# VinAIResearch/GeoFormer

Measured on AMD Instinct MI355X. Metric: scenes/sec forward (ScanNetV2 ~150k pts), higher is better.
Workload: dtype f32

## Files before the change

### geoformer_amd/csrc/decoder_attn.hip

```cpp
#include <stdlib.h>

#include "common.h"

#define DA_WAVES 16
#define DA_D 64

__device__ __forceinline__ float da_row_max(float v) {
    v = fmaxf(v, __int_as_float(__builtin_amdgcn_update_dpp(0, __float_as_int(v), 0xB1, 0xF, 0xF, true)));
    v = fmaxf(v, __int_as_float(__builtin_amdgcn_update_dpp(0, __float_as_int(v), 0x4E, 0xF, 0xF, true)));
    v = fmaxf(v, __int_as_float(__builtin_amdgcn_update_dpp(0, __float_as_int(v), 0x141, 0xF, 0xF, true)));
    v = fmaxf(v, __int_as_float(__builtin_amdgcn_update_dpp(0, __float_as_int(v), 0x140, 0xF, 0xF, true)));
    return v;
}
__device__ __forceinline__ float da_row_sum(float v) {
    v += __int_as_float(__builtin_amdgcn_update_dpp(0, __float_as_int(v), 0xB1, 0xF, 0xF, true));
    v += __int_as_float(__builtin_amdgcn_update_dpp(0, __float_as_int(v), 0x4E, 0xF, 0xF, true));
    v += __int_as_float(__builtin_amdgcn_update_dpp(0, __float_as_int(v), 0x141, 0xF, 0xF, true));
    v += __int_as_float(__builtin_amdgcn_update_dpp(0, __float_as_int(v), 0x140, 0xF, 0xF, true));
    return v;
}

template <int WAVES>
__global__ __launch_bounds__(WAVES * 64) void k_decoder_cross_attn(
    const float* __restrict__ geo_ctx, const float* __restrict__ max_geo, const float* __restrict__ qloc,
    const float* __restrict__ cloc, const float* __restrict__ lo, const float* __restrict__ hi,
    const float* __restrict__ gaussB, const float* __restrict__ Q1, const float* __restrict__ K1,
    const float* __restrict__ Kv, const float4* __restrict__ Wpack, int nq, int nc, float* __restrict__ out,
    float* __restrict__ stat_m, float* __restrict__ stat_l) {
    __shared__ float4 sW[3 * 16 * 64];
    __shared__ float4 sQ1[16];
    __shared__ float4 sB[3][2][4];
    __shared__ float sRed[3][WAVES][DA_D];
    const int qi = blockIdx.x, b = blockIdx.y;
    const int tid = threadIdx.x, lane = tid & 63, w = tid >> 6, g = lane >> 4, j = lane & 15;
    for (int t = tid; t < 3 * 16 * 64; t += WAVES * 64) sW[t] = Wpack[t];
    if (tid < 16) sQ1[tid] = *reinterpret_cast<const float4*>(Q1 + ((size_t)b * nq + qi) * DA_D + tid * 4);
    if (tid >= 64 && tid < 64 + 24) {
        const int e = tid - 64, axis = e >> 3, half = (e >> 2) & 1, gg = e & 3;
        sB[axis][half][gg] = *reinterpret_cast<const float4*>(gaussB + axis * 32 + half * 16 + 4 * gg);
    }
    geo_ctx += ((size_t)b * nq + qi) * nc;
    cloc += (size_t)b * nc * 3;
    K1 += (size_t)b * nc * DA_D;
    Kv += (size_t)b * nc * DA_D;
    const float mg = max_geo[(size_t)b * nq + qi];
    const float qx = qloc[((size_t)b * nq + qi) * 3 + 0], qy = qloc[((size_t)b * nq + qi) * 3 + 1],
                qz = qloc[((size_t)b * nq + qi) * 3 + 2];
    const float lx = lo[b * 3 + 0], ly = lo[b * 3 + 1], lz = lo[b * 3 + 2];
    const float sx = hi[b * 3 + 0] - lx, sy = hi[b * 3 + 1] - ly, sz = hi[b * 3 + 2] - lz;
    float sm[4][4], sl[4][4], sa[4][4];
#pragma unroll
    for (int rb = 0; rb < 4; rb++)
#pragma unroll
        for (int r = 0; r < 4; r++) {
            sm[rb][r] = -3.0e38f;
            sl[rb][r] = 0.f;
            sa[rb][r] = 0.f;
        }
    __syncthreads();

    const int ntiles = (nc + 15) >> 4;
    for (int t = w; t < ntiles; t += WAVES) {
        const int ctx = t * 16 + j;
        const bool valid = ctx < nc;
        const int cc = valid ? ctx : nc - 1;
        const float gd = geo_ctx[cc];
        float g0 = gd, g1 = gd, g2 = gd;
        if (gd < 0.f) {
            g0 = mg + fabsf(qx - cloc[cc * 3 + 0]);
            g1 = mg + fabsf(qy - cloc[cc * 3 + 1]);
            g2 = mg + fabsf(qz - cloc[cc * 3 + 2]);
        }
        const float t0 = ((g0 - lx) / sx) * 6.2831855f, t1 = ((g1 - ly) / sy) * 6.2831855f,
                    t2 = ((g2 - lz) / sz) * 6.2831855f;
        float R[4][4];
#pragma unroll
        for (int half = 0; half < 2; half++) {
            const float4 b0 = sB[0][half][g], b1 = sB[1][half][g], b2v = sB[2][half][g];
            const float p[4] = {fmaf(t2, b2v.x, fmaf(t1, b1.x, t0 * b0.x)), fmaf(t2, b2v.y, fmaf(t1, b1.y, t0 * b0.y)),
                                fmaf(t2, b2v.z, fmaf(t1, b1.z, t0 * b0.z)), fmaf(t2, b2v.w, fmaf(t1, b1.w, t0 * b0.w))};
#pragma unroll
            for (int e = 0; e < 4; e++) {
                float sn, cs;
                __sincosf(p[e], &sn, &cs);
                R[half][e] = sn;
// ... 240 lines not shown
                const float4 k1 = *reinterpret_cast<const float4*>(K1 + (size_t)cc[u] * DA_D + rb * 16 + 4 * g);
                H[u][rb][0] = fmaxf(acc[u][0] + q1.x - k1.x, 0.f);
                H[u][rb][1] = fmaxf(acc[u][1] + q1.y - k1.y, 0.f);
                H[u][rb][2] = fmaxf(acc[u][2] + q1.z - k1.z, 0.f);
                H[u][rb][3] = fmaxf(acc[u][3] + q1.w - k1.w, 0.f);
            }
            da_gemm_bf3_n<NT>(sW3, 2, rb, lane, RP, vv);
#pragma unroll
            for (int u = 0; u < NT; u++) V[u][rb] = vv[u];
            __builtin_amdgcn_sched_barrier(0);
        }
        DaPieces HP[NT];
#pragma unroll
        for (int u = 0; u < NT; u++) da_split_pack(H[u], HP[u]);
#pragma unroll
        for (int rb = 0; rb < 4; rb++) {
            f32x4 s[NT];
#pragma unroll
            for (int u = 0; u < NT; u++) s[u] = (f32x4){0.f, 0.f, 0.f, 0.f};
            da_gemm_bf3_n<NT>(sW3, 1, rb, lane, HP, s);
#pragma unroll
            for (int u = 0; u < NT; u++) {
                const float4 kv = *reinterpret_cast<const float4*>(Kv + (size_t)cc[u] * DA_D + rb * 16 + 4 * g);
                const float kvv[4] = {kv.x, kv.y, kv.z, kv.w};
                if (valid[u]) {
#pragma unroll
                    for (int r = 0; r < 4; r++) {
                        const float x = s[u][r] * kScale2;
                        const float val = V[u][rb][r] + kvv[r];
                        const float mn = fmaxf(sm[rb][r], x);
                        const float corr = __builtin_amdgcn_exp2f(sm[rb][r] - mn), p = __builtin_amdgcn_exp2f(x - mn);
                        sl[rb][r] = sl[rb][r] * corr + p;
                        sa[rb][r] = sa[rb][r] * corr + p * val;
                        sm[rb][r] = mn;
                    }
                }
            }
            __builtin_amdgcn_sched_barrier(0);
        }
    }
#pragma unroll
    for (int rb = 0; rb < 4; rb++)
#pragma unroll
        for (int r = 0; r < 4; r++) {
            const float m = da_row_max(sm[rb][r]);
            if (j == 0) sRed[0][w][rb * 16 + 4 * g + r] = m;
        }
    __syncthreads();
    if (tid < DA_D) {
        float m = sRed[0][0][tid];
#pragma unroll
        for (int u = 1; u < WAVES; u++) m = fmaxf(m, sRed[0][u][tid]);
        sRed[0][0][tid] = m;
    }
    __syncthreads();
#pragma unroll
    for (int rb = 0; rb < 4; rb++)
#pragma unroll
        for (int r = 0; r < 4; r++) {
            const int c = rb * 16 + 4 * g + r;
            const float f = __builtin_amdgcn_exp2f(sm[rb][r] - sRed[0][0][c]);
            const float l = da_row_sum(sl[rb][r] * f), a = da_row_sum(sa[rb][r] * f);
            if (j == 0) {
                sRed[1][w][c] = l;
                sRed[2][w][c] = a;
            }
        }
    __syncthreads();
    if (tid < DA_D) {
        float L = 0.f, A = 0.f;
#pragma unroll
        for (int u = 0; u < WAVES; u++) {
            L += sRed[1][u][tid];
            A += sRed[2][u][tid];
        }
        out[((size_t)b * nq + qi) * DA_D + tid] = A / L;
        if (stat_m) {
            stat_m[((size_t)b * nq + qi) * DA_D + tid] = sRed[0][0][tid] * 0.69314718055994531f;
            stat_l[((size_t)b * nq + qi) * DA_D + tid] = L;
        }
    }
}

extern "C" size_t gf_decoder_wpack_floats(void) { return (size_t)DA_WPACK_F32 + (size_t)DA_WPACK_BF3_U4 * 4; }

__global__ void k_decoder_pack(const float* __restrict__ W1, const float* __restrict__ W2, const float* __restrict__ Wv,
                               float* __restrict__ Wp) {
    const int t = blockIdx.x * blockDim.x + threadIdx.x;
    if (t >= 3 * 16 * 64 * 4) return;
    const int s = t & 3, lane = (t >> 2) & 63, kb = (t >> 8) & 3, rb = (t >> 10) & 3, m = t >> 12;
    const float* W = m == 0 ? W1 : (m == 1 ? W2 : Wv);
    Wp[t] = W[(rb * 16 + (lane & 15)) * DA_D + kb * 16 + 4 * (lane >> 4) + s];
}

__global__ void k_decoder_pack_bf3(const float* __restrict__ W1, const float* __restrict__ W2, const float* __restrict__ Wv,
                                   uint4* __restrict__ Wp3) {
    const int t = blockIdx.x * blockDim.x + threadIdx.x;
    if (t >= 3 * 4 * 2 * 64) return;
    const int lane = t & 63, h = (t >> 6) & 1, rb = (t >> 7) & 3, m = t >> 9;
    const float* W = m == 0 ? W1 : (m == 1 ? W2 : Wv);
    unsigned pc[3][8];
    for (int e = 0; e < 8; e++) {
        const int kb = 2 * h + (e >> 2), sidx = e & 3;
        da_split3(W[(rb * 16 + (lane & 15)) * DA_D + kb * 16 + 4 * (lane >> 4) + sidx], pc[0][e], pc[1][e], pc[2][e]);
    }
    for (int piece = 0; piece < 3; piece++) {
        uint4 v;
        v.x = (pc[piece][1] & 0xffff0000u) | (pc[piece][0] >> 16);
        v.y = (pc[piece][3] & 0xffff0000u) | (pc[piece][2] >> 16);
        v.z = (pc[piece][5] & 0xffff0000u) | (pc[piece][4] >> 16);
        v.w = (pc[piece][7] & 0xffff0000u) | (pc[piece][6] >> 16);
        Wp3[((size_t)(((m * 4 + rb) * 2 + h) * 3 + piece)) * 64 + lane] = v;
    }
}

extern "C" int gf_decoder_pack_weights(const float* W1, const float* W2, const float* Wv, float* Wpack, void* stream) {
    hipLaunchKernelGGL(k_decoder_pack, dim3(48), dim3(256), 0, (hipStream_t)stream, W1, W2, Wv, Wpack);
    hipLaunchKernelGGL(k_decoder_pack_bf3, dim3(6), dim3(256), 0, (hipStream_t)stream, W1, W2, Wv,
                       reinterpret_cast<uint4*>(Wpack + DA_WPACK_F32));
    GF_CHECK_LAUNCH("gf_decoder_pack_weights");
    return GF_OK;
}

static int g_da_bf3 = -1;
extern "C" int gf_dev_cross_attn_bf3(int on) {
    g_da_bf3 = on < 0 ? -1 : (on != 0);
    return GF_OK;
}

extern "C" int gf_decoder_cross_attn_cfg(const float* geo_ctx, const float* max_geo, const float* qloc, const float* cloc,
                                         const float* lo, const float* hi, const float* gaussB, const float* Q1,
                                         const float* K1, const float* Kv, const float* Wpack, const float* b2, int B,
                                         int nq, int nc, int d, float* out, float* stat_m, float* stat_l, int wg_waves,
                                         void* stream) {
    GF_CHECK_ARG(d == DA_D, "gf_decoder_cross_attn: implemented for dec_dim = 64 (got %d)", d);
    GF_CHECK_ARG(B >= 0 && nq >= 0 && nc >= 1, "gf_decoder_cross_attn: bad sizes");
    GF_CHECK_ARG((stat_m == nullptr) == (stat_l == nullptr), "gf_decoder_cross_attn: stat_m and stat_l come together");
    GF_CHECK_ARG(wg_waves == 16 || wg_waves == 8, "gf_decoder_cross_attn_cfg: %d waves per workgroup (16 or 8)", wg_waves);
    if (B == 0 || nq == 0) return GF_OK;
    (void)b2;
    if (wg_waves == 16 && g_da_bf3 != 0) {
        const size_t lds = (size_t)DA_WPACK_BF3_U4 * sizeof(uint4);
        gf_allow_lds((const void*)k_decoder_cross_attn_bf3<DA_BF3_WAVES, 1>, (int)lds);
        GF_LAUNCH_OP(GF_OP_CROSS_ATTN, (k_decoder_cross_attn_bf3<DA_BF3_WAVES, 1>), dim3(nq, B), dim3(DA_BF3_WAVES * 64), lds,
                     (hipStream_t)stream, geo_ctx, max_geo, qloc, cloc, lo, hi, gaussB, Q1, K1, Kv,
                     reinterpret_cast<const uint4*>(Wpack + DA_WPACK_F32), nq, nc, out, stat_m, stat_l);
        GF_CHECK_LAUNCH("gf_decoder_cross_attn");
        return GF_OK;
    }
    if (wg_waves == 16)
        GF_LAUNCH_OP(GF_OP_CROSS_ATTN, k_decoder_cross_attn<16>, dim3(nq, B), dim3(16 * 64), 0, (hipStream_t)stream, geo_ctx,
                     max_geo, qloc, cloc, lo, hi, gaussB, Q1, K1, Kv, reinterpret_cast<const float4*>(Wpack), nq, nc, out,
                     stat_m, stat_l);
    else
        GF_LAUNCH_OP(GF_OP_CROSS_ATTN, k_decoder_cross_attn<8>, dim3(nq, B), dim3(8 * 64), 0, (hipStream_t)stream, geo_ctx,
                     max_geo, qloc, cloc, lo, hi, gaussB, Q1, K1, Kv, reinterpret_cast<const float4*>(Wpack), nq, nc, out,
                     stat_m, stat_l);
    GF_CHECK_LAUNCH("gf_decoder_cross_attn");
    return GF_OK;
}

extern "C" int gf_decoder_cross_attn(const float* geo_ctx, const float* max_geo, const float* qloc, const float* cloc,
                                     const float* lo, const float* hi, const float* gaussB, const float* Q1,
                                     const float* K1, const float* Kv, const float* Wpack, const float* b2, int B,
                                     int nq, int nc, int d, float* out, float* stat_m, float* stat_l, void* stream) {
    return gf_decoder_cross_attn_cfg(geo_ctx, max_geo, qloc, cloc, lo, hi, gaussB, Q1, K1, Kv, Wpack, b2, B, nq, nc, d, out,
                                     stat_m, stat_l, 16, stream);
}


#define DAB_TS 68

__global__ void k_decoder_pack_w2t(const float* __restrict__ W2, float* __restrict__ Wp) {
    const int t = blockIdx.x * blockDim.x + threadIdx.x;
    if (t >= 16 * 64 * 4) return;
    const int s = t & 3, lane = (t >> 2) & 63, kb = (t >> 8) & 3, cb = (t >> 10) & 3;
    Wp[t] = W2[(kb * 16 + 4 * (lane >> 4) + s) * DA_D + cb * 16 + (lane & 15)];
}

__global__ __launch_bounds__(256, 1) void k_decoder_cross_attn_bwd(
    const float* __restrict__ geo_ctx, const float* __restrict__ max_geo, const float* __restrict__ qloc,
    const float* __restrict__ cloc, const float* __restrict__ lo, const float* __restrict__ hi,
    const float* __restrict__ gaussB, const float* __restrict__ Q1, const float* __restrict__ K1,
    const float* __restrict__ Kv, const float4* __restrict__ Wpack, const float4* __restrict__ W2Tpack,
    const float* __restrict__ outv, const float* __restrict__ stat_m, const float* __restrict__ stat_l,
    const float* __restrict__ gout, int B, int nq, int nc, int qsplit, float* __restrict__ dQ1p,
    float* __restrict__ dK1, float* __restrict__ dKv, float* __restrict__ dWp) {
    __shared__ float4 sW[3 * 16 * 64];
    __shared__ float4 sW2T[16 * 64];
    __shared__ float4 sB[3][2][4];
    __shared__ __attribute__((aligned(16))) float sT[4][16 * DAB_TS];
    __shared__ __attribute__((aligned(16))) float sV[4][4][DA_D];
    const int tid = threadIdx.x, lane = tid & 63, w = tid >> 6, g = lane >> 4, j = lane & 15;
    for (int t = tid; t < 3 * 16 * 64; t += 256) sW[t] = Wpack[t];
    for (int t = tid; t < 16 * 64; t += 256) sW2T[t] = W2Tpack[t];
    if (tid < 24) {
        const int axis = tid >> 3, half = (tid >> 2) & 1, gg = tid & 3;
        sB[axis][half][gg] = *reinterpret_cast<const float4*>(gaussB + axis * 32 + half * 16 + 4 * gg);
    }
    __syncthreads();
    const int ntiles = (nc + 15) >> 4;
    const int wave = blockIdx.x * 4 + w;
    const int items = B * ntiles * qsplit;
    if (wave >= items) return;
    const int part = wave % qsplit, bt = wave / qsplit;
    const int tile = bt % ntiles, b = bt / ntiles;
    const int qper = (nq + qsplit - 1) / qsplit;
    const int q0 = part * qper, q1 = min(nq, q0 + qper);
    float* T = sT[w];
    float* V = &sV[w][0][0];

    const int ctx = tile * 16 + j;
    const bool valid = ctx < nc;
    const int cc = valid ? ctx : nc - 1;
    const float* K1b = K1 + ((size_t)b * nc + cc) * DA_D;
    const float* Kvb = Kv + ((size_t)b * nc + cc) * DA_D;
    float4 k1[4], kv[4];
#pragma unroll
    for (int rb = 0; rb < 4; rb++) {
        k1[rb] = *reinterpret_cast<const float4*>(K1b + rb * 16 + 4 * g);
        kv[rb] = *reinterpret_cast<const float4*>(Kvb + rb * 16 + 4 * g);
    }
    const float cx = cloc[((size_t)b * nc + cc) * 3 + 0], cy = cloc[((size_t)b * nc + cc) * 3 + 1],
                cz = cloc[((size_t)b * nc + cc) * 3 + 2];
    const float lx = lo[b * 3 + 0], ly = lo[b * 3 + 1], lz = lo[b * 3 + 2];
    const float sx = hi[b * 3 + 0] - lx, sy = hi[b * 3 + 1] - ly, sz = hi[b * 3 + 2] - lz;

    f32x4 aW1[4][4], aW2[4][4], aWv[4][4];
    f32x4 aK1[4], aKv[4];
#pragma unroll
    for (int a = 0; a < 4; a++) {
        aK1[a] = (f32x4){0.f, 0.f, 0.f, 0.f};
        aKv[a] = (f32x4){0.f, 0.f, 0.f, 0.f};
#pragma unroll
        for (int c = 0; c < 4; c++) {
            aW1[a][c] = (f32x4){0.f, 0.f, 0.f, 0.f};
            aW2[a][c] = (f32x4){0.f, 0.f, 0.f, 0.f};
            aWv[a][c] = (f32x4){0.f, 0.f, 0.f, 0.f};
        }
    }
    auto transpose = [&](const f32x4 (&XA)[4], f32x4 (&XB)[4]) {
        asm volatile("s_waitcnt lgkmcnt(0)" ::: "memory");
#pragma unroll
        for (int rb = 0; rb < 4; rb++)
            *reinterpret_cast<float4*>(&T[j * DAB_TS + rb * 16 + 4 * g]) = make_float4(XA[rb][0], XA[rb][1], XA[rb][2], XA[rb][3]);
        asm volatile("s_waitcnt lgkmcnt(0)" ::: "memory");
#pragma unroll
        for (int cb = 0; cb < 4; cb++)
#pragma unroll
            for (int r = 0; r < 4; r++) XB[cb][r] = T[(4 * g + r) * DAB_TS + cb * 16 + j];
// ... 239 lines not shown
```

### geoformer_amd/csrc/decoder_layer.h

```cpp
#pragma once
#include "tile_gemm.h"

#define DL_D 64
#define DL_H 4
#define DL_DK 16
#define DL_THREADS 1024
#define DL_MAXFF 256

#define DL_LD 68
#define DL_LDH 260

template <typename Out>
__device__ __forceinline__ void dl_tile_layernorm_p(const float (*S)[DL_LD], int nvalid, float wl, float bl, int wave,
                                                    int nwaves, int lane, Out out);
template <typename Out>
__device__ __forceinline__ void dl_tile_layernorm(const float (*S)[DL_LD], int nvalid, const float* __restrict__ w,
                                                  const float* __restrict__ b, int wave, int nwaves, int lane,
                                                  Out out) {
    dl_tile_layernorm_p(S, nvalid, w[lane], b[lane], wave, nwaves, lane, out);
}
template <typename Out>
__device__ __forceinline__ void dl_tile_layernorm_p(const float (*S)[DL_LD], int nvalid, float wl, float bl, int wave,
                                                    int nwaves, int lane, Out out) {
    for (int r = wave; r < nvalid; r += nwaves) {
        const float v = S[r][lane];
        const float s = gf_wave_sum(v);
        const float mu = s / (float)DL_D;
        const float dv = v - mu;
        const float q = gf_wave_sum(dv * dv);
        const float rstd = 1.0f / sqrtf(q / (float)DL_D + 1e-5f);
        out(r, lane, dv * rstd * wl + bl);
    }
}
```

### geoformer_amd/csrc/decoder_layer.hip

```cpp
#include "decoder_layer.h"

struct DlPost {
    const float *omw, *omb, *n3w, *n3b, *l1w, *l1b, *l2w, *l2b, *fnw, *fnb;
};
struct DlPre {
    const float *n1w, *n1b, *ipw, *ipb, *opw, *opb, *n2w, *n2b, *w1w, *w1b;
};

#define DL_TILE_THREADS 256

#ifdef DL_TRACE
__device__ unsigned long long* g_dl_trace = nullptr;
extern "C" int gf_dev_dl_trace(void* p) {
    GF_TRY(hipMemcpyToSymbol(HIP_SYMBOL(g_dl_trace), &p, sizeof(p)));
    return GF_OK;
}
#define DL_STAMP(k) do { if (g_dl_trace && threadIdx.x == 0) g_dl_trace[((size_t)(blockIdx.y * gridDim.x + blockIdx.x)) * 32 + (k)] = __builtin_amdgcn_s_memtime(); } while (0)
#else
#define DL_STAMP(k) do { } while (0)
#endif

__global__ __launch_bounds__(DL_TILE_THREADS) void k_decoder_stage_a(const float* __restrict__ attn_out,
                                                                     const float* __restrict__ tgt_in,
                                                                     const float* __restrict__ query_pos, int T,
                                                                     int B, int ff, int has_post, int has_pre,
                                                                     DlPost po, DlPre pr, float* __restrict__ state,
                                                                     float* __restrict__ inter_out) {
    __shared__ float sX[16][DL_LD], sT[16][DL_LD], sQ[16][DL_LD], sH[16][DL_LDH];
    const int b = blockIdx.y, t0 = blockIdx.x * 16;
    const int nvalid = min(16, T - t0);
    const int lane = threadIdx.x & 63, wave = threadIdx.x >> 6, nw = DL_TILE_THREADS / 64;
    float* X = state + (size_t)b * T * (5 * DL_D);
    float* TGT2 = X + (size_t)T * DL_D;
    float* QKV = TGT2 + (size_t)T * DL_D;
    const int lds = B * DL_D;
    DL_STAMP(0);
    constexpr int NTF = DL_MAXFF / 16 / (DL_TILE_THREADS / 64);
    GfTileW<1, DL_D / 16> w_om;
    GfTileW<NTF, DL_D / 16> w_l1;
    GfTileW<1, DL_MAXFF / 16> w_l2;
    GfTileW<2, DL_D / 16> w_qk;
    GfTileW<1, DL_D / 16> w_v;
    float n3w = 0.f, n3b = 0.f, fnw = 0.f, fnb = 0.f, n1w = 0.f, n1b = 0.f;
    if (has_post) {
        gf_tile_w_load(w_om, po.omw, po.omb, DL_D, DL_D, wave, nw, lane);
        n3w = po.n3w[lane]; n3b = po.n3b[lane];
        gf_tile_w_load(w_l1, po.l1w, po.l1b, ff, DL_D, wave, nw, lane);
        gf_tile_w_load(w_l2, po.l2w, po.l2b, DL_D, ff, wave, nw, lane);
        fnw = po.fnw[lane]; fnb = po.fnb[lane];
    }
    if (has_pre) {
        n1w = pr.n1w[lane]; n1b = pr.n1b[lane];
        gf_tile_w_load(w_qk, pr.ipw, pr.ipb, 2 * DL_D, DL_D, wave, nw, lane);
        gf_tile_w_load(w_v, pr.ipw + 2 * DL_D * DL_D, pr.ipb + 2 * DL_D, DL_D, DL_D, wave, nw, lane);
    }
    if (has_post) {
        const float* tg = TGT2 + (size_t)t0 * DL_D;
        gf_tile_gemm_w<true>(attn_out + ((size_t)b * T + t0) * DL_D, DL_D, nvalid, DL_D, DL_D, wave, nw, lane, w_om,
                             [&](int r, int c, float v) { sX[r][c] = v; }, tg, DL_D);
        __syncthreads();
        DL_STAMP(1);
        dl_tile_layernorm_p(sX, nvalid, n3w, n3b, wave, nw, lane, [&](int r, int c, float v) { sT[r][c] = v; });
        __syncthreads();
        DL_STAMP(2);
        gf_tile_gemm_w<true>(&sT[0][0], DL_LD, nvalid, DL_D, ff, wave, nw, lane, w_l1,
                             [&](int r, int c, float v) { sH[r][c] = v; });
        __syncthreads();
        DL_STAMP(3);
        gf_tile_gemm_w<false>(&sH[0][0], DL_LDH, nvalid, ff, DL_D, wave, nw, lane, w_l2,
                              [&](int r, int c, float v) { sX[r][c] += v; });
        __syncthreads();
        DL_STAMP(4);
        float* io = inter_out + (size_t)t0 * lds + b * DL_D;
        dl_tile_layernorm_p(sX, nvalid, fnw, fnb, wave, nw, lane,
                            [&](int r, int c, float v) { io[(size_t)r * lds + c] = v; });
    } else {
        for (int i = threadIdx.x; i < nvalid * DL_D; i += DL_TILE_THREADS)
            sX[i >> 6][i & 63] = tgt_in[(size_t)(t0 + (i >> 6)) * lds + b * DL_D + (i & 63)];
        __syncthreads();
    }
    DL_STAMP(5);
    if (!has_pre) return;
    const float* qp = query_pos + (size_t)t0 * lds + b * DL_D;
    dl_tile_layernorm_p(sX, nvalid, n1w, n1b, wave, nw, lane, [&](int r, int c, float v) {
        sT[r][c] = v;
        sQ[r][c] = v + qp[(size_t)r * lds + c];
    });
    for (int i = threadIdx.x; i < nvalid * DL_D; i += DL_TILE_THREADS)
        X[(size_t)(t0 + (i >> 6)) * DL_D + (i & 63)] = sX[i >> 6][i & 63];
    __syncthreads();
    DL_STAMP(6);
    float* qkv = QKV + (size_t)t0 * (3 * DL_D);
    gf_tile_gemm_w<false>(&sQ[0][0], DL_LD, nvalid, DL_D, 2 * DL_D, wave, nw, lane, w_qk,
                          [&](int r, int c, float v) { qkv[(size_t)r * (3 * DL_D) + c] = v; });
    DL_STAMP(7);
    gf_tile_gemm_w<false>(&sT[0][0], DL_LD, nvalid, DL_D, DL_D, wave, nw, lane, w_v,
                          [&](int r, int c, float v) { qkv[(size_t)r * (3 * DL_D) + 2 * DL_D + c] = v; });
    DL_STAMP(8);
}

template <int QTN>
__device__ __forceinline__ void dl_attn_two_pass(const float* __restrict__ QKV, int T, int h, int j, int g, float4 bq,
                                                 f32x4& o, float& l) {
    float4 akt[QTN];
    float vt[QTN][4];
    const int last = T - 1;
#pragma unroll
    for (int kt = 0; kt < QTN; kt++) {
        const int krow = min(kt * 16 + j, last);
        akt[kt] = *reinterpret_cast<const float4*>(QKV + (size_t)krow * (3 * DL_D) + DL_D + h * DL_DK + 4 * g);
#pragma unroll
        for (int i = 0; i < 4; i++) {
            const int key = min(kt * 16 + 4 * g + i, last);
            vt[kt][i] = QKV[(size_t)key * (3 * DL_D) + 2 * DL_D + h * DL_DK + j];
        }
    }
    float sc[QTN][4];
    float mx = -INFINITY;
#pragma unroll
    for (int kt = 0; kt < QTN; kt++) {
        f32x4 s = {0.f, 0.f, 0.f, 0.f};
        s = gf_mfma4(akt[kt], bq, s);
#pragma unroll
        for (int i = 0; i < 4; i++) {
            sc[kt][i] = (kt * 16 + 4 * g + i) < T ? s[i] * 0.25f : -INFINITY;
            mx = fmaxf(mx, sc[kt][i]);
        }
    }
    mx = fmaxf(mx, gf_shfl_xor<16>(mx));
    mx = fmaxf(mx, gf_shfl_xor<32>(mx));
#pragma unroll
    for (int kt = 0; kt < QTN; kt++) {
#pragma unroll
        for (int i = 0; i < 4; i++) {
            const float pi = __builtin_amdgcn_exp2f((sc[kt][i] - mx) * 1.4426950408889634f);
            l += pi;
            o = __builtin_amdgcn_mfma_f32_16x16x4f32(vt[kt][i], pi, o, 0, 0, 0);
        }
    }
}

__global__ __launch_bounds__(DL_TILE_THREADS) void k_decoder_stage_b(int T, int B, DlPre pr,
                                                                     float* __restrict__ state,
                                                                     float* __restrict__ q1_out) {
    __shared__ float sO[16][DL_LD], sX[16][DL_LD], sT[16][DL_LD];
    const int b = blockIdx.y, t0 = blockIdx.x * 16;
    const int nvalid = min(16, T - t0);
    const int lane = threadIdx.x & 63, wave = threadIdx.x >> 6, nw = DL_TILE_THREADS / 64;
    const int j = lane & 15, g = lane >> 4;
    float* X = state + (size_t)b * T * (5 * DL_D);
    float* TGT2 = X + (size_t)T * DL_D;
    const float* QKV = TGT2 + (size_t)T * DL_D;
    DL_STAMP(16);
    GfTileW<1, DL_D / 16> w_op, w_w1;
    gf_tile_w_load(w_op, pr.opw, pr.opb, DL_D, DL_D, wave, nw, lane);
    gf_tile_w_load(w_w1, pr.w1w, pr.w1b, DL_D, DL_D, wave, nw, lane);
    const float n2w = pr.n2w[lane], n2b = pr.n2b[lane];
    {
        const int h = wave;
        const int QT = (T + 15) >> 4;
        const float4 z4 = make_float4(0.f, 0.f, 0.f, 0.f);
        const int qrow = t0 + j;
        float4 bq = z4;
        if (qrow < T) bq = *reinterpret_cast<const float4*>(QKV + (size_t)qrow * (3 * DL_D) + h * DL_DK + 4 * g);
        f32x4 o = {0.f, 0.f, 0.f, 0.f};
        float m = -INFINITY, l = 0.f;
        if (QT <= 16) {
            if (QT <= 8) dl_attn_two_pass<8>(QKV, T, h, j, g, bq, o, l);
            else dl_attn_two_pass<16>(QKV, T, h, j, g, bq, o, l);
        } else {
        float4 ak = z4;
        float v[4];
        {
            if (j < T) ak = *reinterpret_cast<const float4*>(QKV + (size_t)j * (3 * DL_D) + DL_D + h * DL_DK + 4 * g);
#pragma unroll
            for (int i = 0; i < 4; i++) {
                const int key = 4 * g + i;
                v[i] = key < T ? QKV[(size_t)key * (3 * DL_D) + 2 * DL_D + h * DL_DK + j] : 0.f;
            }
        }
        for (int kt = 0; kt < QT; kt++) {
            float4 ak_n = z4;
            float v_n[4] = {0.f, 0.f, 0.f, 0.f};
            if (kt + 1 < QT) {
                const int krow = (kt + 1) * 16 + j;
                if (krow < T)
                    ak_n = *reinterpret_cast<const float4*>(QKV + (size_t)krow * (3 * DL_D) + DL_D + h * DL_DK + 4 * g);
#pragma unroll
                for (int i = 0; i < 4; i++) {
                    const int key = (kt + 1) * 16 + 4 * g + i;
                    v_n[i] = key < T ? QKV[(size_t)key * (3 * DL_D) + 2 * DL_D + h * DL_DK + j] : 0.f;
                }
            }
            f32x4 s = {0.f, 0.f, 0.f, 0.f};
            s = gf_mfma4(ak, bq, s);
            float sc[4];
#pragma unroll
            for (int i = 0; i < 4; i++) sc[i] = (kt * 16 + 4 * g + i) < T ? s[i] * 0.25f : -INFINITY;
            float mx = fmaxf(fmaxf(sc[0], sc[1]), fmaxf(sc[2], sc[3]));
            mx = fmaxf(mx, gf_shfl_xor<16>(mx));
            mx = fmaxf(mx, gf_shfl_xor<32>(mx));
            const float mnew = fmaxf(m, mx);
            const float corr = expf(m - mnew);
            float p[4];
#pragma unroll
            for (int i = 0; i < 4; i++) p[i] = expf(sc[i] - mnew);
            l = l * corr + ((p[0] + p[1]) + (p[2] + p[3]));
            o *= corr;
            m = mnew;
#pragma unroll
            for (int i = 0; i < 4; i++) o = __builtin_amdgcn_mfma_f32_16x16x4f32(v[i], p[i], o, 0, 0, 0);
            ak = ak_n;
#pragma unroll
            for (int i = 0; i < 4; i++) v[i] = v_n[i];
        }
        }
        l += gf_shfl_xor<16>(l);
        l += gf_shfl_xor<32>(l);
#pragma unroll
        for (int i = 0; i < 4; i++) sO[j][h * DL_DK + 4 * g + i] = o[i] / l;
    }
    __syncthreads();
    DL_STAMP(17);
    const float* xg = X + (size_t)t0 * DL_D;
    gf_tile_gemm_w<false>(&sO[0][0], DL_LD, nvalid, DL_D, DL_D, wave, nw, lane, w_op,
                          [&](int r, int c, float v) { sX[r][c] = v; }, xg, DL_D);
    __syncthreads();
    DL_STAMP(18);
    float* xo = X + (size_t)t0 * DL_D;
    for (int i = threadIdx.x; i < nvalid * DL_D; i += DL_TILE_THREADS) xo[i] = sX[i >> 6][i & 63];
    float* tg = TGT2 + (size_t)t0 * DL_D;
    dl_tile_layernorm_p(sX, nvalid, n2w, n2b, wave, nw, lane, [&](int r, int c, float v) {
        sT[r][c] = v;
        tg[r * DL_D + c] = v;
    });
    __syncthreads();
    DL_STAMP(19);
    float* q1 = q1_out + ((size_t)b * T + t0) * DL_D;
    gf_tile_gemm_w<false>(&sT[0][0], DL_LD, nvalid, DL_D, DL_D, wave, nw, lane, w_w1,
                          [&](int r, int c, float v) { q1[r * DL_D + c] = v; });
    DL_STAMP(20);
}

extern "C" size_t gf_decoder_token_state_bytes(int nq, int B) {
    return (size_t)(nq > 0 ? nq : 0) * (B > 0 ? B : 0) * (5 * DL_D) * sizeof(float);
}

extern "C" int gf_decoder_token_stage(const float* attn_out, const float* tgt_in, const float* query_pos, int nq, int B,
                                      int d, int nhead, int ff, const float* const* post_params,
                                      const float* const* pre_params, void* state, float* inter_out, float* q1_out,
                                      void* stream) {
    GF_CHECK_ARG(d == DL_D && nhead == DL_H, "gf_decoder_token_stage: built for d_model=64, 4 heads (got %d, %d)", d,
                 nhead);
    GF_CHECK_ARG(ff > 0 && ff % 16 == 0 && ff <= DL_MAXFF, "gf_decoder_token_stage: dim_feedforward %d not in 16..%d",
                 ff, DL_MAXFF);
    GF_CHECK_ARG(nq >= 0 && B >= 0, "gf_decoder_token_stage: bad sizes");
    GF_CHECK_ARG(post_params || pre_params, "gf_decoder_token_stage: nothing to do");
    GF_CHECK_ARG(post_params ? (attn_out && inter_out) : (tgt_in != nullptr),
                 "gf_decoder_token_stage: post needs attn_out and inter_out, a first stage needs tgt_in");
    GF_CHECK_ARG(!pre_params || (query_pos && q1_out), "gf_decoder_token_stage: pre needs query_pos and q1_out");
    if (nq == 0 || B == 0) return GF_OK;
    DlPost po = {};
    DlPre pr = {};
    if (post_params) {
        for (int i = 0; i < 10; i++) GF_CHECK_ARG(post_params[i], "gf_decoder_token_stage: post_params[%d] is null", i);
        po = {post_params[0], post_params[1], post_params[2], post_params[3], post_params[4],
              post_params[5], post_params[6], post_params[7], post_params[8], post_params[9]};
    }
    if (pre_params) {
        for (int i = 0; i < 10; i++) GF_CHECK_ARG(pre_params[i], "gf_decoder_token_stage: pre_params[%d] is null", i);
        pr = {pre_params[0], pre_params[1], pre_params[2], pre_params[3], pre_params[4],
              pre_params[5], pre_params[6], pre_params[7], pre_params[8], pre_params[9]};
    }
    const dim3 grid((nq + 15) / 16, B);
    hipLaunchKernelGGL(k_decoder_stage_a, grid, dim3(DL_TILE_THREADS), 0, (hipStream_t)stream, attn_out, tgt_in,
                       query_pos, nq, B, ff, post_params ? 1 : 0, pre_params ? 1 : 0, po, pr, (float*)state, inter_out);
    if (pre_params)
        hipLaunchKernelGGL(k_decoder_stage_b, grid, dim3(DL_TILE_THREADS), 0, (hipStream_t)stream, nq, B, pr,
                           (float*)state, q1_out);
    GF_CHECK_LAUNCH("gf_decoder_token_stage");
    return GF_OK;
}
```

### geoformer_amd/csrc/mask_head.hip

```cpp
#include "common.h"

#ifndef MH_Q
#define MH_Q 2
#endif
#ifndef MH_MINB
#define MH_MINB 3
#endif

__device__ __forceinline__ float mh_xor32(float v, int lane) {
    const auto r = __builtin_amdgcn_permlane32_swap(__float_as_uint(v), __float_as_uint(v), false, false);
    return __uint_as_float(lane < 32 ? r[1] : r[0]);
}
__device__ __forceinline__ float mh_xor16(float v, int lane) {
    const auto r = __builtin_amdgcn_permlane16_swap(__float_as_uint(v), __float_as_uint(v), false, false);
    return __uint_as_float((lane & 16) ? r[0] : r[1]);
}

__device__ __forceinline__ float mh_relu(float x) { return __int_as_float(max(__float_as_int(x), 0)); }

typedef short bf16x4 __attribute__((ext_vector_type(4)));
typedef short mh_s8 __attribute__((ext_vector_type(8)));
typedef __bf16 mh_bf16x8 __attribute__((ext_vector_type(8)));
__device__ __forceinline__ f32x4 mh_mfma2(bf16x4 a1, bf16x4 a2, bf16x4 b1, bf16x4 b2, f32x4 acc) {
    const mh_s8 a = __builtin_shufflevector(a1, a2, 0, 1, 2, 3, 4, 5, 6, 7), b = __builtin_shufflevector(b1, b2, 0, 1, 2, 3, 4, 5, 6, 7);
// ... 81 lines not shown
    const size_t n16 = (size_t)N * 16;
    auto fetch = [&](int blk, Block& B) {
        const int p0 = TINY ? blk * 64 : min(blk * 64, N - 64);
#pragma unroll
        for (int t = 0; t < 4; t++) {
            const int pc = TINY ? min(p0 + 16 * t + j, N - 1) : p0 + 16 * t + j;
            if constexpr (SPLIT) {
                const size_t e = (size_t)pc * 16 + 4 * g;
                B.fh[t] = *reinterpret_cast<const bf16x4*>(fs + e);
                B.fm[t] = *reinterpret_cast<const bf16x4*>(fs + n16 + e);
                B.fl[t] = *reinterpret_cast<const bf16x4*>(fs + 2 * n16 + e);
            } else {
                B.f[t] = *reinterpret_cast<const float4*>(feat + (size_t)pc * 16 + 4 * g);
            }
            B.pc[t] = g < 3 ? coords[(size_t)pc * 3 + g] : 0.f;
#pragma unroll
            for (int u = 0; u < MH_Q; u++)
                B.gd[u][t] = USE_GEO ? geo[(size_t)qrow[u] * N + pc] : 0.f;
        }
    };
    auto compute = [&](const Block& cur, int blk) {
        const int p0 = TINY ? blk * 64 : min(blk * 64, N - 64);
#pragma unroll
        for (int t = 0; t < MH_Q; t++) {
            const int q = qg * MH_Q + t;
            float part[4];
#pragma unroll
            for (int tl = 0; tl < 4; tl++) {
                float rel = qc[t] - cur.pc[tl];
                if (USE_GEO) {
                    const float ms = __uint_as_float((__float_as_uint(rel) & 0x80000000u) | __float_as_uint(mq[t]));
                    rel = rel + ((cur.gd[t][tl] < 0.f && rel != 0.f) ? ms : 0.f);
                }
                f32x4 acc = {0.f, 0.f, 0.f, 0.f};
                acc = __builtin_amdgcn_mfma_f32_16x16x4f32(w5[t], rel, acc, 0, 0, 0);
                if constexpr (SPLIT) {
                    acc = mh_mfma2(wl[t], wh[t], cur.fh[tl], cur.fl[tl], acc);
                    acc = mh_mfma2(wm[t], wm[t], cur.fm[tl], cur.fh[tl], acc);
                    acc = mh_mfma2(wh[t], wh[t], cur.fm[tl], cur.fh[tl], acc);
                } else {
                    acc = __builtin_amdgcn_mfma_f32_16x16x4f32(wf[t][0], cur.f[tl].x, acc, 0, 0, 0);
                    acc = __builtin_amdgcn_mfma_f32_16x16x4f32(wf[t][1], cur.f[tl].y, acc, 0, 0, 0);
                    acc = __builtin_amdgcn_mfma_f32_16x16x4f32(wf[t][2], cur.f[tl].z, acc, 0, 0, 0);
                    acc = __builtin_amdgcn_mfma_f32_16x16x4f32(wf[t][3], cur.f[tl].w, acc, 0, 0, 0);
                }
                float s = 0.f;
#pragma unroll
                for (int r = 0; r < 4; r++) s = fmaf(ww[t][r], mh_relu(acc[r]), s);
                part[tl] = s;
            }
            {
                const bool hi = g >= 2;
                const float send0 = hi ? part[0] : part[2], send1 = hi ? part[1] : part[3];
                const float r0 = mh_xor32(send0, lane), r1 = mh_xor32(send1, lane);
                const float k0 = (hi ? part[2] : part[0]) + r0, k1 = (hi ? part[3] : part[1]) + r1;
                const bool odd = g & 1;
                const float send = odd ? k0 : k1;
                const float r = mh_xor16(send, lane);
                const float tot = (odd ? k1 : k0) + r + b2q[t];
                const int p = p0 + 16 * g + j;
                if (p < N && q < nq) out[(size_t)q * N + p] = tot;
            }
        }
    };
    Block bufA, bufB;
    if (blk0 < blk1) fetch(blk0, bufA);
    for (int blk = blk0; blk < blk1; blk += 2) {
        if (blk + 1 < blk1) fetch(blk + 1, bufB);
        compute(bufA, blk);
        if (blk + 1 < blk1) {
            if (blk + 2 < blk1) fetch(blk + 2, bufA);
            compute(bufB, blk + 1);
        }
    }
}

extern "C" int gf_mask_head_packed(const float* feat, const float* coords, const float* geo, const float* qxyz,
                                   const float* sqrt_max_geo, const float* w1, const float* b1, const float* w2,
                                   const float* b2, int ldp, int N, int nq, int C, float* out, void* stream);
extern "C" int gf_mask_head_episodes(const float* feat, const float* coords, const float* geo, const float* qxyz,
                                     const float* sqrt_max_geo, const float* w1, const float* b1, const float* w2,
                                     const float* b2, int ldp, int N, int nq, int E, int C, void* split_ws, float* out,
                                     void* stream);
extern "C" size_t gf_mask_head_split_bytes(int N) { return (size_t)(N > 0 ? N : 0) * 16 * 3 * sizeof(unsigned short); }
extern "C" int gf_mask_head(const float* feat, const float* coords, const float* geo, const float* qxyz,
                            const float* sqrt_max_geo, const float* w1, const float* b1, const float* w2,
                            const float* b2, int N, int nq, int C, float* out, void* stream) {
    return gf_mask_head_packed(feat, coords, geo, qxyz, sqrt_max_geo, w1, b1, w2, b2, 0, N, nq, C, out, stream);
}

extern "C" int gf_mask_head_packed(const float* feat, const float* coords, const float* geo, const float* qxyz,
                                   const float* sqrt_max_geo, const float* w1, const float* b1, const float* w2,
                                   const float* b2, int ldp, int N, int nq, int C, float* out, void* stream) {
    return gf_mask_head_episodes(feat, coords, geo, qxyz, sqrt_max_geo, w1, b1, w2, b2, ldp, N, nq, 1, C, nullptr, out, stream);
}

extern "C" int gf_mask_head_episodes(const float* feat, const float* coords, const float* geo, const float* qxyz,
                                     const float* sqrt_max_geo, const float* w1, const float* b1, const float* w2,
                                     const float* b2, int ldp, int N, int nq_scene, int E, int C, void* split_ws, float* out,
                                     void* stream) {
    GF_CHECK_ARG(ldp >= 0, "gf_mask_head: negative parameter stride");
    GF_CHECK_ARG(C == 16, "gf_mask_head: only the 16-channel mask head (m=16) is implemented, got C=%d", C);
    GF_CHECK_ARG(N >= 0 && nq_scene >= 0 && E >= 1, "gf_mask_head: bad sizes");
    GF_CHECK_ARG((long long)nq_scene * E < (1ll << 30), "gf_mask_head: %d episodes x %d queries", E, nq_scene);
    GF_CHECK_ARG((geo == nullptr) == (sqrt_max_geo == nullptr), "gf_mask_head: geo and sqrt_max_geo come together");
    if (N == 0 || nq_scene == 0) return GF_OK;
    const int qmod = nq_scene, nq = nq_scene * E;
    const int qgroups = (nq + MH_Q - 1) / MH_Q;
    const int nblocks = (N + 63) / 64;
    int chunks = (256 * 4 * 8 + qgroups - 1) / qgroups;
    if (chunks > nblocks) chunks = nblocks;
    if (chunks < 1) chunks = 1;
    const long long waves = (long long)qgroups * chunks;
    dim3 grid((unsigned)((waves + 3) / 4));
    hipStream_t st = (hipStream_t)stream;
    const unsigned short* fs = (const unsigned short*)split_ws;
    if (fs) {
        GF_CHECK_ARG(((uintptr_t)fs % 8) == 0, "gf_mask_head: split_ws must be 8-byte aligned");
        const int n16 = N * 16;
        hipLaunchKernelGGL(k_mh_split, dim3(gf_div_up(n16, 256)), dim3(256), 0, st, feat, n16, (unsigned short*)split_ws);
    }
#define MH_LAUNCH(GEO_, SPLIT_)                                                                                          \
    do {                                                                                                                 \
        if (N < 64)                                                                                                      \
            GF_LAUNCH_OP(GF_OP_MASK_HEAD, (k_mask_head<GEO_, SPLIT_, true>), grid, dim3(256), 0, st, feat, coords, geo, qxyz, \
                         sqrt_max_geo, w1, b1, w2, b2, ldp, N, nq, qmod, chunks, fs, out);                               \
        else                                                                                                             \
            GF_LAUNCH_OP(GF_OP_MASK_HEAD, (k_mask_head<GEO_, SPLIT_, false>), grid, dim3(256), 0, st, feat, coords, geo, qxyz, \
                         sqrt_max_geo, w1, b1, w2, b2, ldp, N, nq, qmod, chunks, fs, out);                               \
    } while (0)
    if (geo && fs) MH_LAUNCH(true, true);
    else if (geo) MH_LAUNCH(true, false);
    else if (fs) MH_LAUNCH(false, true);
    else MH_LAUNCH(false, false);
#undef MH_LAUNCH
    GF_CHECK_LAUNCH("gf_mask_head");
    return GF_OK;
}

#define MHB_Q 4

template <bool USE_GEO>
__global__ __launch_bounds__(256, 2) void k_mask_head_bwd_feat(const float* __restrict__ feat, const float* __restrict__ coords,
                                                               const float* __restrict__ geo, const float* __restrict__ qxyz,
                                                               const float* __restrict__ mx, const float* __restrict__ w1,
                                                               const float* __restrict__ b1, const float* __restrict__ w2,
                                                               const float* __restrict__ gout, int ldp, int N, int nq,
                                                               int qmod, int qsplit, float* __restrict__ dfeat) {
    const int ld_w1 = ldp ? ldp : 16 * 19, ld_v = ldp ? ldp : 16;
    const int lane = threadIdx.x & 63, g = lane >> 4, j = lane & 15;
    const int wave = (blockIdx.x * blockDim.x + threadIdx.x) >> 6;
    const int nblocks = (N + 63) >> 6;
    const int blk = wave / qsplit, part = wave - blk * qsplit;
    if (blk >= nblocks) return;
    const int p0 = blk * 64;
    const int qper = (nq + qsplit - 1) / qsplit;
    const int q0 = part * qper, q1 = min(nq, q0 + qper);
    float4 fA[4];
    float pcA[4];
    f32x4 accF[4];
#pragma unroll
    for (int t = 0; t < 4; t++) {
        const int pa = min(p0 + 16 * t + j, N - 1);
        fA[t] = *reinterpret_cast<const float4*>(feat + (size_t)pa * 16 + 4 * g);
        pcA[t] = coords[(size_t)pa * 3 + min(g, 2)];
        accF[t] = (f32x4){0.f, 0.f, 0.f, 0.f};
    }
    for (int q = q0; q < q1; q++) {
        const float* W = w1 + (size_t)q * ld_w1;
        float wf[4], wT[4], ww[4];
#pragma unroll
        for (int s = 0; s < 4; s++) {
            wf[s] = W[j * 19 + 3 + 4 * g + s];
            wT[s] = W[(4 * g + s) * 19 + 3 + j];
            ww[s] = w2[(size_t)q * ld_v + 4 * g + s];
        }
        const float w5 = g < 3 ? W[j * 19 + g] : b1[(size_t)q * ld_v + j];
        const int qs = q % qmod;
        const float qcA = g < 3 ? qxyz[qs * 3 + g] : 0.f;
        const float mq = USE_GEO ? mx[qs] : 0.f;
        float goA[4], gdA[4];
#pragma unroll
        for (int t = 0; t < 4; t++) {
            const int pa = p0 + 16 * t + j;
            goA[t] = pa < N ? gout[(size_t)q * N + pa] : 0.f;
            gdA[t] = USE_GEO ? geo[(size_t)qs * N + min(pa, N - 1)] : 0.f;
        }
#pragma unroll
        for (int t = 0; t < 4; t++) {
            float rel = qcA - pcA[t];
            if (USE_GEO) rel = rel + (gdA[t] < 0.f ? mq : 0.f) * (rel > 0.f ? 1.f : (rel < 0.f ? -1.f : 0.f));
            if (g == 3) rel = 1.0f;
            f32x4 acc = {0.f, 0.f, 0.f, 0.f};
            acc = __builtin_amdgcn_mfma_f32_16x16x4f32(w5, rel, acc, 0, 0, 0);
            acc = __builtin_amdgcn_mfma_f32_16x16x4f32(wf[0], fA[t].x, acc, 0, 0, 0);
            acc = __builtin_amdgcn_mfma_f32_16x16x4f32(wf[1], fA[t].y, acc, 0, 0, 0);
            acc = __builtin_amdgcn_mfma_f32_16x16x4f32(wf[2], fA[t].z, acc, 0, 0, 0);
            acc = __builtin_amdgcn_mfma_f32_16x16x4f32(wf[3], fA[t].w, acc, 0, 0, 0);
#pragma unroll
            for (int s = 0; s < 4; s++) {
                const float dh = acc[s] > 0.f ? goA[t] * ww[s] : 0.f;
                accF[t] = __builtin_amdgcn_mfma_f32_16x16x4f32(wT[s], dh, accF[t], 0, 0, 0);
            }
// ... 205 lines not shown
```

### geoformer_amd/csrc/proposal.hip

```cpp
#include "proposal_rows.h"

__global__ __launch_bounds__(PR_THREADS) void k_proposal_stats(const float* __restrict__ logits,
                                                               const float* __restrict__ cls_logits,
                                                               const float* __restrict__ sem_prob, int N, int ncls,
                                                               float logit_thresh, float score_thresh,
                                                               int npoint_thresh, int min_class,
                                                               int* __restrict__ cls_pred_out,
                                                               int* __restrict__ npoints_out,
                                                               float* __restrict__ scores_out,
                                                               int* __restrict__ final_out) {
    const int q = blockIdx.x;
    pr_stats_row(logits + (size_t)q * N, cls_logits + (size_t)q * ncls, sem_prob, (size_t)N, N, ncls, logit_thresh,
                 score_thresh, npoint_thresh, min_class, cls_pred_out + q, npoints_out + q, scores_out + q,
                 final_out + q);
}

__global__ __launch_bounds__(PR_THREADS) void k_proposal_stats_fs(const float* __restrict__ logits,
                                                                  const float* __restrict__ sim, int N,
                                                                  float logit_thresh, float score_thresh,
                                                                  int npoint_thresh, float sim_thresh,
                                                                  int* __restrict__ npoints_out,
                                                                  float* __restrict__ scores_out,
                                                                  int* __restrict__ final_out) {
    __shared__ int r_cnt[PR_THREADS / 64];
// ... 112 lines not shown
}

__global__ __launch_bounds__(256) void k_mask_intersections(const unsigned long long* __restrict__ bits, int n, int W2,
                                                            int32_t* __restrict__ inter) {
    const long long wave = ((long long)blockIdx.x * blockDim.x + threadIdx.x) >> 6;
    const int lane = threadIdx.x & 63;
    if (wave >= (long long)n * n) return;
    const int i = (int)(wave / n), j = (int)(wave - (long long)i * n);
    if (j < i) return;
    const unsigned long long *a = bits + (size_t)i * W2, *b = bits + (size_t)j * W2;
    int c = 0;
    for (int w = lane; w < W2; w += 64) c += __popcll(a[w] & b[w]);
    c = gf_wave_sum_i(c);
    if (lane == 0) {
        inter[(size_t)i * n + j] = c;
        inter[(size_t)j * n + i] = c;
    }
}

extern "C" size_t gf_mask_intersections_scratch_bytes(int n, int N) {
    return (size_t)(n > 0 ? n : 0) * ((size_t)(N > 0 ? N : 0) + 63) / 64 * sizeof(unsigned long long) + 64;
}

extern "C" int gf_mask_intersections(const int32_t* masks, int n, int N, void* scratch, int32_t* inter, void* stream) {
    GF_CHECK_ARG(n >= 0 && N >= 0, "gf_mask_intersections: bad sizes");
    if (n == 0) return GF_OK;
    hipStream_t st = (hipStream_t)stream;
    const int W2 = (N + 63) / 64;
    unsigned long long* bits = (unsigned long long*)scratch;
    if (W2 > 0) {
        const long long waves = (long long)n * W2;
        hipLaunchKernelGGL(k_mask_pack_bits, dim3((unsigned)((waves + 3) / 4)), dim3(256), 0, st, masks, n, N, W2, bits);
    }
    const long long pairs = (long long)n * n;
    hipLaunchKernelGGL(k_mask_intersections, dim3((unsigned)((pairs + 3) / 4)), dim3(256), 0, st, bits, n, W2, inter);
    GF_CHECK_LAUNCH("gf_mask_intersections");
    return GF_OK;
}

__global__ __launch_bounds__(256) void k_relpos_gather(const float* __restrict__ geo, const int32_t* __restrict__ inds,
                                                       int n, int nc, float* __restrict__ geo_ctx,
                                                       float* __restrict__ row_max) {
    __shared__ float s_m[4];
    const int q = blockIdx.x;
    const float* g = geo + (size_t)q * n;
    float m = -INFINITY;
    for (int j = threadIdx.x; j < nc; j += 256) {
        const float v = g[inds[j]];
        geo_ctx[(size_t)q * nc + j] = v;
        m = fmaxf(m, v);
    }
    m = gf_wave_max(m);
    if ((threadIdx.x & 63) == 0) s_m[threadIdx.x >> 6] = m;
    __syncthreads();
    if (threadIdx.x == 0) row_max[q] = fmaxf(fmaxf(s_m[0], s_m[1]), fmaxf(s_m[2], s_m[3]));
}

__global__ __launch_bounds__(1024) void k_relpos_fix(float* __restrict__ row_max, int nq) {
    __shared__ float s_m[16];
    float m = -INFINITY;
    for (int q = threadIdx.x; q < nq; q += 1024) m = fmaxf(m, row_max[q]);
    m = gf_wave_max(m);
    if ((threadIdx.x & 63) == 0) s_m[threadIdx.x >> 6] = m;
    __syncthreads();
    float all = s_m[0];
#pragma unroll
    for (int w = 1; w < 16; w++) all = fmaxf(all, s_m[w]);
    for (int q = threadIdx.x; q < nq; q += 1024)
        if (row_max[q] < 0.f) row_max[q] = all;
}

extern "C" int gf_relpos_prepare(const float* geo, const int32_t* inds, int nq, int n, int nc, float* geo_ctx,
                                 float* max_geo, void* stream) {
    GF_CHECK_ARG(geo && inds && geo_ctx && max_geo, "gf_relpos_prepare: null argument");
    GF_CHECK_ARG(nq >= 0 && n >= 1 && nc >= 1, "gf_relpos_prepare: bad sizes");
    if (nq == 0) return GF_OK;
    hipStream_t st = (hipStream_t)stream;
    hipLaunchKernelGGL(k_relpos_gather, dim3(nq), dim3(256), 0, st, geo, inds, n, nc, geo_ctx, max_geo);
    hipLaunchKernelGGL(k_relpos_fix, dim3(1), dim3(1024), 0, st, max_geo, nq);
    GF_CHECK_LAUNCH("gf_relpos_prepare");
    return GF_OK;
}

__global__ __launch_bounds__(1024) void k_proposal_select(const int32_t* __restrict__ final_, const int32_t* __restrict__ cls_pred,
                                                          const float* __restrict__ scores, int nq,
                                                          int32_t* __restrict__ sel, long long* __restrict__ cls_out,
                                                          float* __restrict__ scores_out, int32_t* __restrict__ count) {
    pr_select_rows(final_, cls_pred, scores, nq, sel, cls_out, scores_out, count);
}

extern "C" int gf_proposal_select(const int32_t* final_, const int32_t* cls_pred, const float* scores, int nq,
                                  int32_t* sel, long long* cls_out, float* scores_out, int32_t* d_count, void* stream) {
    GF_CHECK_ARG(final_ && cls_pred && scores && sel && cls_out && scores_out && d_count && nq >= 0,
                 "gf_proposal_select: bad arguments");
    hipLaunchKernelGGL(k_proposal_select, dim3(1), dim3(1024), 0, (hipStream_t)stream, final_, cls_pred, scores, nq, sel,
                       cls_out, scores_out, d_count);
    GF_CHECK_LAUNCH("gf_proposal_select");
    return GF_OK;
}
```

### geoformer_amd/model/geoformer.py

```python
from __future__ import annotations

import functools
import os

import numpy as np
import torch
import torch.nn as nn
from torch.nn import functional as F

from .. import _lib, pointops, spconv, unet_exec, unet_train
from . import config as _config
from .backbone import ResidualBlock, UBlock, conv1d_bn_relu, random_downsample
from .layers import (BatchNorm1d, BigLinear, GenericMLP, LazyRelPos, PointwiseConv1d, PositionEmbeddingCoordsSine, RelPosSpec,
                     TransformerDecoder,
                     TransformerDecoderLayer, scene_counts)
from .set_abstraction import PointnetSAModuleVotesSeparate


class _Voxelization(torch.autograd.Function):

    @staticmethod
    def forward(ctx, feats, map_rule, mode=4):
        ctx.rule, ctx.mode, ctx.N = map_rule, mode, feats.shape[0]
        return pointops.voxelize_fp(feats.contiguous(), map_rule, mode)
# ... 651 lines not shown
                    grid_done = torch.cuda.Event()
                    grid_done.record(aux)
                grid = (grid, grid_done)
            if multi:
                for t in (xyz_b, idx, first, sampling_indices):
                    if t is not None:
                        t.record_stream(main)
            if early is not None and b == 0:
                main.wait_event(early_done)
            staged[b] = [xyz_b, None, idx, grid, sampling_indices]
            if not epilogue:
                continue
            self._side_epilogue(b, batch_size, g, xyz_b, src, pc_dims, main, side, aux, picks_ready)
        for sb in scene_streams:
            main.wait_stream(sb)
        with grad_ctx():
            for b, st in enumerate(staged):
                feat_b = output_feats_[offs[b]:offs[b + 1]]
                if st[4] is not None:
                    feat_b = pointops.take_rows_unique(feat_b, st[4])
                st[1] = feat_b.unsqueeze(0).transpose(1, 2).contiguous()
        staged = [tuple(st[:4]) for st in staged]
        self.__dict__.setdefault("_gf_pending_side", {})[_stream_key(locs_float_.device)] = geo_ready
        self.__dict__.setdefault("_gf_stretch_events", {})[_stream_key(locs_float_.device)] = fps_done_evs + [
            ev for ev in geo_ready if ev is not None]
        cat = lambda ts: ts[0] if len(ts) == 1 else torch.cat(ts)
        with grad_ctx():
            fused = []
            for xyz_b, feat_b, idx, grid in staged:
                if grid is not None:
                    main.wait_event(grid[1])
                fused.append(self.set_aggregator.fused_forward(xyz_b, feat_b, idx, grid=None if grid is None else grid[0]))
            if all(f is not None for f in fused):
                context_locs, pre_enc_inds = cat([f[0] for f in fused]), cat([st[2] for st in staged])
                context_feats = cat([f[1] for f in fused]).transpose(1, 2)
                res = ((context_locs, context_feats, pre_enc_inds), geo)
                return res + (early_out,) if early is not None else res
            locs, gfeat, gxyz, inds = [], [], [], []
            for xyz_b, feat_b, idx, _ in staged:
                l, gf, gx, idx = self.set_aggregator.group_points(xyz_b, feat_b, inds=idx)
                locs.append(l); gfeat.append(gf); gxyz.append(gx); inds.append(idx)
            context_locs, pre_enc_inds = cat(locs), cat(inds)
            context_feats = self.set_aggregator.mlp(cat(gfeat), cat(gxyz)).transpose(1, 2)
        res = ((context_locs, context_feats, pre_enc_inds), geo)
        return res + (early_out,) if early is not None else res

    def _side_epilogue(self, b, batch_size, g, xyz_b, src, pc_dims, main, side, aux, first_ready):
        early = self._early()
        if b == 0:
            early.clear()
        with torch.cuda.stream(side):
            mx = torch.max(g, dim=1)[0]
            mx = torch.sqrt(torch.where(mx < 0, torch.max(mx), mx)).contiguous()
            mx.record_stream(main)
            ev = torch.cuda.Event()
            ev.record(side)
            early[("mx", b)] = (g, mx, ev)
        if batch_size == 1 and pc_dims is not None and self.cfg.dec_dim == 64:
            aux.wait_event(first_ready)
            with torch.cuda.stream(aux):
                qpr = self._pointwise_chain("qproj", [self.query_projection], xyz_b)
                if qpr is not None:
                    xyz_b.record_stream(aux)
                    q_locs = xyz_b[:, src.long()]
                    qpe = self.pos_embedding(q_locs, input_range=pc_dims).float()
                    qpos = pointops.pointwise_mlp(qpe[0].t().contiguous(), qpr)
                    qpos.record_stream(main)
                    src.record_stream(aux)
                    ev = torch.cuda.Event()
                    ev.record(aux)
                    early["qpos"] = (q_locs, qpos, ev)

    def _early(self):
        if not torch.cuda.is_available():
            return {}
        return self.__dict__.setdefault("_gf_early", {}).setdefault(_stream_key(), {})

    def _join_side_stream(self):
        pend = self.__dict__.get("_gf_pending_side")
        if pend and torch.cuda.is_available():
            for ev in pend.pop(_stream_key(), None) or ():
                torch.cuda.current_stream().wait_event(ev)

    def relative_position_embedding(self, context_locs, query_locs, pc_dims, geo_dists, pre_enc_inds):
        B = context_locs.shape[0]
        self._join_side_stream()
        if context_locs.is_cuda and self.cfg.dec_dim == 64 and (not torch.is_grad_enabled()
                                                                 or os.environ.get("GF_FUSED_BWD", "1") != "0"):
            if B == 1 and pre_enc_inds.dtype == torch.int32:
                g1, m1 = pointops.relpos_prepare(geo_dists[0].contiguous(), pre_enc_inds[0].contiguous())
                geo, max_geo = g1.unsqueeze(0), m1.unsqueeze(0)
            elif B > 1 and pre_enc_inds.stride(0) == 0 and all(g is geo_dists[0] for g in geo_dists):
                g1 = geo_dists[0][:, pre_enc_inds[0].long()]
                m1 = torch.max(g1, dim=1)[0]
                m1 = torch.where(m1 < 0, torch.max(m1), m1)
                geo, max_geo = g1.unsqueeze(0).expand(B, -1, -1).contiguous(), m1.unsqueeze(0).expand(B, -1).contiguous()
            else:
                geo = torch.stack([geo_dists[b][:, pre_enc_inds[b].long()] for b in range(B)], dim=0).contiguous()
                max_geo = torch.max(geo, dim=2)[0]
                max_geo = torch.where(max_geo < 0, torch.max(max_geo), max_geo).contiguous()
            return RelPosSpec(geo, max_geo, query_locs.contiguous(), context_locs.contiguous(),
                              pc_dims[0].float().contiguous(), pc_dims[1].float().contiguous(),
                              self.pos_embedding.gauss_B.contiguous())
        rel = torch.abs(query_locs[:, :, None, :] - context_locs[:, None, :, :])
        nq, nc = rel.shape[1], rel.shape[2]
        geo = torch.stack([geo_dists[b][:, pre_enc_inds[b].long()] for b in range(B)], dim=0)
        max_geo = torch.max(geo, dim=2)[0]
        max_all = torch.max(max_geo)
        max_geo = torch.where(max_geo < 0, max_all, max_geo)
        geo3 = geo[:, :, :, None].repeat(1, 1, 1, 3)
        geo3 = torch.where(geo3 < 0, max_geo[:, :, None, None] + rel, geo3)
        emb = self.pos_embedding(geo3.reshape(B, nq * nc, -1), input_range=pc_dims).reshape(B, -1, nq, nc)
        return emb.permute(2, 3, 0, 1)

    def forward_decoder(self, context_locs, context_feats, query_locs, pc_dims, geo_dists, pre_enc_inds):
        nq = self.cfg.n_query_points
        if context_locs.shape[0] == 1 and context_locs.is_cuda and not torch.is_grad_enabled():
            e2d = self._pointwise_chain("e2d", [self.encoder_to_decoder_projection], context_feats)
            qpr = self._pointwise_chain("qproj", [self.query_projection], context_feats)
            if e2d is not None and qpr is not None:
                ctx = pointops.pointwise_mlp(context_feats[0].contiguous(), e2d)
                rel = LazyRelPos(lambda: self.relative_position_embedding(context_locs, query_locs, pc_dims, geo_dists,
                                                                          pre_enc_inds))
                hit = self._early().pop("qpos", None)
                if hit is not None and hit[0].shape == query_locs.shape:
                    torch.cuda.current_stream().wait_event(hit[2])
                    qpos = hit[1]
                else:
                    qpe = self.pos_embedding(query_locs, input_range=pc_dims).float()
                    qpos = pointops.pointwise_mlp(qpe[0].t().contiguous(), qpr)
                memory = ctx.unsqueeze(1)
                return self.decoder(tgt=memory[:nq], memory=memory, pos=None, query_pos=qpos.unsqueeze(1),
                                    relative_pos=rel)
        context_embedding_pos = self.pos_embedding(context_locs, input_range=pc_dims)
        context_feats = self.encoder_to_decoder_projection(context_feats.permute(0, 2, 1))
        query_embedding_pos = self.query_projection(self.pos_embedding(query_locs, input_range=pc_dims).float())
        dec_inputs = context_feats[:, :, :nq].permute(2, 0, 1)
        relative_embedding_pos = self.relative_position_embedding(context_locs, query_locs, pc_dims, geo_dists,
                                                                  pre_enc_inds)
        return self.decoder(tgt=dec_inputs, memory=context_feats.permute(2, 0, 1),
                            pos=context_embedding_pos.permute(2, 0, 1), query_pos=query_embedding_pos.permute(2, 0, 1),
                            relative_pos=relative_embedding_pos)

    def parse_dynamic_params(self, params, out_channels):
        n = params.size(0)
        w1, w2, b1, b2 = torch.split_with_sizes(params, self.weight_nums + self.bias_nums, dim=1)
        return ([w1.reshape(n * out_channels, -1, 1), w2.reshape(n, -1, 1)],
                [b1.reshape(n * out_channels), b2.reshape(n)])

    def mask_heads_forward(self, geo_dist, mask_features, weights, biases, num_insts, coords_, fps_sampling_coords,
                           use_geo=True):
        n_mask = mask_features.size(0)
        if (mask_features.is_cuda and self.output_dim == 16 and not torch.is_grad_enabled()):
            mx = None
            if use_geo:
                early = self._early()
                hit = next((early.pop(k) for k in list(early) if k[0] == "mx" and early[k][0] is geo_dist), None)
                if hit is not None:
                    torch.cuda.current_stream().wait_event(hit[2])
                    mx = hit[1]
                else:
                    mx = torch.max(geo_dist, dim=1)[0]
                    mx = torch.sqrt(torch.where(mx < 0, torch.max(mx), mx)).contiguous()
            od = self.output_dim
            logits = pointops.mask_head(
                mask_features.reshape(n_mask, od).contiguous(), coords_.contiguous(),
                geo_dist.contiguous() if use_geo else None, fps_sampling_coords.reshape(-1, 3).contiguous(), mx,
                weights[0].reshape(num_insts, od, od + 3).contiguous(), biases[0].reshape(num_insts, od).contiguous(),
                weights[1].reshape(num_insts, od).contiguous(), biases[1].reshape(num_insts).contiguous())
            return logits.reshape(1, num_insts, n_mask)
        rel = fps_sampling_coords.reshape(-1, 1, 3) - coords_.reshape(1, -1, 3)
        if use_geo:
            mx = torch.max(geo_dist, dim=1)[0]
            mx = torch.sqrt(torch.where(mx < 0, torch.max(mx), mx))
            rel = torch.where((geo_dist < 0).unsqueeze(-1), rel + mx[:, None, None] * torch.sign(rel), rel)
        w1, w2 = weights[0].reshape(num_insts, self.output_dim, -1), weights[1].reshape(num_insts, 1, -1)
        b1, b2 = biases[0].reshape(num_insts, self.output_dim, 1), biases[1].reshape(num_insts, 1, 1)
        feat = mask_features.reshape(n_mask, -1)
        h = torch.matmul(w1[:, :, :3], rel.permute(0, 2, 1)) + torch.matmul(w1[:, :, 3:], feat.t().unsqueeze(0)) + b1
        x = torch.matmul(w2, F.relu(h)) + b2
        return x.reshape(1, num_insts, n_mask)

    def _mask_head_packed(self, geo_dist, mask_features, params, num_insts, coords_, fps_sampling_coords):
        n_mask = mask_features.size(0)
        early = self._early()
        hit = next((early.pop(k) for k in list(early) if k[0] == "mx" and early[k][0] is geo_dist), None)
        if hit is not None:
            torch.cuda.current_stream().wait_event(hit[2])
            mx = hit[1]
        else:
            mx = torch.max(geo_dist, dim=1)[0]
            mx = torch.sqrt(torch.where(mx < 0, torch.max(mx), mx)).contiguous()
        logits = pointops.mask_head_packed(mask_features.reshape(n_mask, self.output_dim).contiguous(),
                                           coords_.contiguous(), geo_dist.contiguous(),
                                           fps_sampling_coords.reshape(-1, 3).contiguous(), mx, params.contiguous())
        return logits.reshape(1, num_insts, n_mask)

    def get_mask_prediction(self, geo_dists, param_kernels, mask_features, locs_float_, fps_sampling_locs,
                            batch_offsets_):
        num_layers, n_queries, batch = param_kernels.shape[:3]
        offs = _offsets_list(batch_offsets_)
        outputs = []
        fused_train = (mask_features.is_cuda and torch.is_grad_enabled() and self.output_dim == 16 and self.use_coords
                       and os.environ.get("GF_FUSED_BWD", "1") != "0")
        per_scene, train_ctrl = {}, {}
        if fused_train:
            for b in range(batch):
                s, e = offs[b], offs[b + 1]
                if e - s == 0:
                    continue
                g = geo_dists[b].contiguous()
                mx = torch.max(g, dim=1)[0]
                mx = torch.sqrt(torch.where(mx < 0, torch.max(mx), mx)).contiguous()
                per_scene[b] = (mask_features[s:e].reshape(e - s, self.output_dim).contiguous(),
                                locs_float_[s:e].contiguous(), g, fps_sampling_locs[b].reshape(-1, 3).contiguous(), mx)
        for l, pk in enumerate(param_kernels.unbind(0) if fused_train else param_kernels):
            pk2 = pk.transpose(0, 1).flatten(0, 1)
            sem_chain = self._pointwise_chain("detr_sem_head", [self.detr_sem_head], pk2)
            tow_chain = self._pointwise_chain("before_embedding_tower", [self.before_embedding_tower], pk2)
            packed = False
            if sem_chain is not None and tow_chain is not None:
                rows = pk2.contiguous()
                packed = self.output_dim == 16 and self.use_coords
                cls_done = None
                if packed and rows.is_cuda and not torch.is_grad_enabled() and batch == 1 and not pointops.co_resident():
                    main = torch.cuda.current_stream(rows.device)
                    aux = _SIDE_STREAMS.get((rows.device, main.cuda_stream, "aux"))
                    if aux is not None:
                        rows_ready = torch.cuda.Event()
                        rows_ready.record(main)
                        aux.wait_event(rows_ready)
                        with torch.cuda.stream(aux):
                            cls_logits = pointops.pointwise_mlp(rows, sem_chain).reshape(batch, n_queries, -1)
                            cls_done = torch.cuda.Event()
                            cls_done.record(aux)
                        rows.record_stream(aux)
                        cls_logits.record_stream(main)
                if cls_done is None:
                    cls_logits = pointops.pointwise_mlp(rows, sem_chain).reshape(batch, n_queries, -1)
                emb = pointops.pointwise_mlp(rows, tow_chain)
                controllers = F.linear(emb, self.controller.weight[:, :, 0], self.controller.bias)
            else:
                cls_logits = self.detr_sem_head(pk.permute(1, 2, 0)).transpose(1, 2)
                controllers = self.controller(self.before_embedding_tower(pk2.unsqueeze(2))).squeeze(2)
            controllers = controllers.reshape(batch, n_queries, -1)
            ctrl = controllers.unbind(0) if fused_train else controllers
            mask_logits_list = []
            for b in range(batch):
                s, e = offs[b], offs[b + 1]
                if e - s == 0:
                    mask_logits_list.append(None)
                    continue
                if packed and mask_features.is_cuda and not torch.is_grad_enabled():
                    ml = self._mask_head_packed(geo_dists[b], mask_features[s:e], controllers[b], n_queries,
                                                locs_float_[s:e], fps_sampling_locs[b])
                elif fused_train:
                    train_ctrl.setdefault(b, []).append(ctrl[b])
                    mask_logits_list.append(None)
                    continue
                else:
                    weights, biases = self.parse_dynamic_params(controllers[b], self.output_dim)
                    ml = self.mask_heads_forward(geo_dists[b], mask_features[s:e], weights, biases, n_queries,
                                                 locs_float_[s:e], fps_sampling_locs[b], use_geo=self.use_coords)
                mask_logits_list.append(ml.squeeze(0))
            if packed and cls_done is not None:
                torch.cuda.current_stream(cls_logits.device).wait_event(cls_done)
            outputs.append({"cls_logits": cls_logits, "mask_logits": mask_logits_list})
        for b, ctrls in train_ctrl.items():
            mf_b, locs_b, g, fps_b, mx = per_scene[b]
            logits = pointops.mask_head_train_episodes(mf_b, torch.stack(ctrls), locs_b, g, fps_b, mx)
            for l, ml in enumerate(logits.unbind(0)):
                outputs[l]["mask_logits"][b] = ml
        return outputs

    def generate_proposal(self, mask_logits, cls_logits, fg_idxs, batch_offsets, batch_offsets_,
                          semantic_scores_=None, logit_thresh=0.5, score_thresh=0.5, npoint_thresh=100, sem_prob=None,
                          defer=False, knn_flags=(), segments=None):
        b = 0
# ... 106 lines not shown

    def forward_split(self, batch_input, epoch, training=True, defer_proposals=False):
        return SplitForward(self._forward_steps(batch_input, epoch, training, defer_proposals, True))

    def _forward_steps(self, batch_input, epoch, training, defer_proposals, split, all_scenes=False):
        cfg = self.cfg
        outputs = {}
        batch_idxs = batch_input["locs"][:, 0].int()
        locs_float = batch_input["locs_float"]
        batch_offsets = batch_input["offsets"]
        batch_size = len(batch_offsets) - 1
        assert batch_size > 0
        pc_dims = [batch_input["pc_maxs"], batch_input["pc_mins"]]
        segments = _segments_arg(batch_input.get("segments"), locs_float.shape[0])
        if training or torch.is_grad_enabled():
            segments = None

        fused_fg = (locs_float.is_cuda and not torch.is_grad_enabled() and epoch > self.prepare_epochs
                    and locs_float.dtype == torch.float32)
        output_feats, semantic_scores, semantic_preds = self.forward_backbone(batch_input, batch_size,
                                                                              want_preds=not fused_fg)
        outputs["semantic_scores"] = semantic_scores
        if epoch <= self.prepare_epochs:
            return outputs
        same_fold = cfg.train_fold == cfg.cvfold
        fg_pending = None
        if fused_fg:
            feats_src, feat_rows = output_feats if isinstance(output_feats, tuple) else (output_feats.contiguous(), None)
            fg_pending = pointops.select_foreground(
                semantic_scores.contiguous(), 4 if same_fold else 3, not same_fold, locs_float.contiguous(),
                batch_idxs.contiguous(), feats_src, feat_rows, deferred=True)
        if split:
            backbone_done = torch.cuda.Event() if locs_float.is_cuda else None
            if backbone_done is not None:
                backbone_done.record()
            yield backbone_done
        if fused_fg:
            presampled = None
            from_count = (batch_size == 1 and not training and cfg.n_downsampling
                          and os.environ.get("GF_OVERLAP", "1") != "0")
            if batch_size == 1 and locs_float.is_cuda and cfg.n_downsampling and epoch > self.prepare_epochs:
                pointops.legacy_prefetch(int(1.4 * locs_float.shape[0]) + 4096)
                if from_count:
                    nq_, npoint_sa_, split_ = self._sampling_split()
                    draw_bufs = pointops.draw_sample_buffers(int(cfg.n_downsampling), int(locs_float.shape[0]),
                                                             locs_float.device, fps_m=nq_ if split_ else npoint_sa_)
                    draw_bufs["before"] = fg_pending.done
            n_fg = fg_pending.wait()
            if from_count and n_fg > 0:
                presampled = self._sample_from_count(n_fg, fg_pending.bufs[1], draw_bufs)
            fg_idxs, locs_float_, batch_idxs_, output_feats_, semantic_scores_ = fg_pending.views()
        else:
            fg = semantic_preds >= 4 if same_fold else semantic_preds == 3
            fg_idxs = torch.nonzero(fg).view(-1)
        agree = self.rank_agreement if (training and torch.is_grad_enabled()) else None
        if len(fg_idxs) == 0:
            if agree is not None:
                agree(False, locs_float.device)
            outputs["mask_predictions"] = None
            if all_scenes:
                empty = [([], [], []) for _ in range(batch_size)]
                outputs["proposal_scores_per_scene"] = PendingBatchProposals(batch_size, value=empty) \
                    if defer_proposals else empty
            return outputs
        if not fused_fg:
            batch_idxs_ = batch_idxs[fg_idxs]
            locs_float_ = locs_float[fg_idxs]
            output_feats_ = pointops.take_rows_unique(output_feats, fg_idxs)
            semantic_scores_ = semantic_scores[fg_idxs]
        batch_offsets_ = get_batch_offsets(batch_idxs_, batch_size, host_only=fused_fg and not training)
        offs_ = _offsets_list(batch_offsets_)
        nonempty = min(offs_[b + 1] - offs_[b] for b in range(batch_size)) > 0
        n_scenes, scene_ids = batch_size, list(range(batch_size))
        if all_scenes and not nonempty:
            scene_ids = [b for b in range(batch_size) if offs_[b + 1] > offs_[b]]
            offs_ = [offs_[b] for b in scene_ids] + [offs_[-1]]
            batch_offsets_ = torch.tensor(offs_, dtype=torch.int32, device=batch_offsets_.device)
            pc_dims = [pc_dims[0][scene_ids], pc_dims[1][scene_ids]]
            batch_size, nonempty = len(scene_ids), True
        if agree is not None and not agree(nonempty, locs_float.device):
            outputs["mask_predictions"] = None
            return outputs

        def sampling_independent(graphs_only=None):
            if graphs_only is True:
                return knn_graphs(locs_float_, batch_offsets_, batch_size, neighbor=64, radius=0.05)
            chain = self._pointwise_chain("mask_tower", [self.mask_tower], output_feats_)
            if chain is not None:
                mf = pointops.pointwise_mlp(output_feats_.contiguous(), chain).unsqueeze(2)
            else:
                mf = self._mask_tower_rows(output_feats_)
                if mf is None:
                    mf = self.mask_tower(output_feats_.unsqueeze(2).permute(2, 1, 0)).permute(2, 1, 0)
            sp = None
            if not training:
                sp = F.softmax(semantic_scores_, dim=1)
                if sp.is_cuda:
                    sp = (sp, sp.t().contiguous())
            if graphs_only is False:
                return mf, sp
            gr = None
            if locs_float_.is_cuda and nonempty:
                gr = knn_graphs(locs_float_, batch_offsets_, batch_size, neighbor=64, radius=0.05)
            return mf, sp, gr

        max_step = 128 if self.training else 256
        geo_dists = None
        overlap = locs_float_.is_cuda and nonempty and os.environ.get("GF_OVERLAP", "1") != "0"
        if overlap and fused_fg and not training:
            contexts, geo_dists, (mask_features_, sem_prob, graphs) = self._aggregate_geodesic_overlapped(
                locs_float_, output_feats_, batch_offsets_, batch_size, None, max_step, pc_dims, epilogue=True,
                early=sampling_independent, presampled=presampled if fused_fg else None,
                presampled_before=draw_bufs["before"] if (fused_fg and presampled is not None) else None)
        else:
            mask_features_, sem_prob, graphs = sampling_independent()
            if graphs is not None and overlap:
                contexts, geo_dists = self._aggregate_geodesic_overlapped(locs_float_, output_feats_, batch_offsets_,
                                                                          batch_size, graphs, max_step, pc_dims,
                                                                          epilogue=not torch.is_grad_enabled())
            else:
                contexts = self.forward_aggregator(locs_float_, output_feats_, batch_offsets_, batch_size)
        if contexts is None:
            outputs["mask_predictions"] = None
            return outputs
        context_locs, context_feats, pre_enc_inds = contexts
        query_locs = context_locs[:, :cfg.n_query_points, :]

        if geo_dists is None:
            geo_dists = cal_geodesic(pre_enc_inds, locs_float_, batch_offsets_, max_step=max_step, neighbor=64,
                                     radius=0.05, n_queries=cfg.n_query_points, graphs=graphs)
        if split:
            stretch = []
            if locs_float.is_cuda:
                stretch = list(self.__dict__.get("_gf_stretch_events", {}).pop(_stream_key(locs_float.device), ()))
                if not stretch:
                    ev = torch.cuda.Event()
                    ev.record()
                    stretch = [ev]
            yield stretch
        dec_outputs = self.forward_decoder(context_locs, context_feats, query_locs, pc_dims, geo_dists, pre_enc_inds)
        self._join_side_stream()

        if training:
            idxs_sub, idxs_sub_raw = random_downsample(batch_offsets_, batch_size, n_subsample=30000,
                                                         host_offsets=_offsets_list(batch_offsets_))
            geo_sub = [geo_dists[b][:, idxs_sub_raw[b]] for b in range(batch_size)]
            del geo_dists
            batch_idxs_sub = batch_idxs_[idxs_sub]
            offsets_sub = get_batch_offsets(batch_idxs_sub, batch_size)
            outputs["fg_idxs"] = fg_idxs[idxs_sub]
            outputs["num_insts"] = cfg.n_query_points * batch_size
            outputs["batch_idxs"] = batch_idxs_sub
            outputs["n_fg_total"] = int(offs_[-1])
            trunc = knn_truncated(graphs)
            if trunc is not None:
                outputs["knn_truncated"] = trunc
            outputs["mask_predictions"] = self.get_mask_prediction(geo_sub, dec_outputs,
                                                                   pointops.take_rows_unique(mask_features_, idxs_sub),
                                                                   locs_float_[idxs_sub], query_locs, offsets_sub)
        else:
            dec_outputs = dec_outputs[-1:, ...]
            outputs["fg_idxs"] = fg_idxs
            outputs["num_insts"] = cfg.n_query_points * batch_size
            outputs["batch_idxs"] = batch_idxs_
            preds = self.get_mask_prediction(geo_dists, dec_outputs, mask_features_, locs_float_, query_locs,
                                             batch_offsets_)
            outputs["mask_predictions"] = preds
            if all_scenes:
                outputs["proposal_scores_per_scene"] = self.generate_proposals_batched(
                    preds[-1]["mask_logits"], preds[-1]["cls_logits"], fg_idxs, batch_offsets, offs_, scene_ids,
                    n_scenes, sem_prob, logit_thresh=0.5, score_thresh=cfg.TEST_SCORE_THRESH,
                    npoint_thresh=cfg.TEST_NPOINT_THRESH, defer=defer_proposals,
                    knn_flags=[f for f in (knn_truncated(graphs),) if f is not None], segments=segments)
            else:
                outputs["proposal_scores"] = self.generate_proposal(
                    preds[-1]["mask_logits"], preds[-1]["cls_logits"], fg_idxs, batch_offsets, batch_offsets_,
                    semantic_scores_=semantic_scores_, logit_thresh=0.5, score_thresh=cfg.TEST_SCORE_THRESH,
                    npoint_thresh=cfg.TEST_NPOINT_THRESH, sem_prob=sem_prob, defer=defer_proposals,
                    knn_flags=[f for f in (knn_truncated(graphs),) if f is not None], segments=segments)
        if locs_float.is_cuda:
            self._early().clear()
        return outputs
```

### geoformer_amd/model/layers.py

```python
from __future__ import annotations

import copy
import math
import os

import numpy as np
import torch
import torch.nn as nn
import torch.nn.functional as F

from .. import pointops

_FUSED_BN = os.environ.get("GF_FUSED_BN", "1") != "0"


def _bn_train(mod, x, dims):
    if _FUSED_BN and isinstance(mod, _HostCounter) and pointops.bn_train_cl_supported(mod, x):
        y = pointops.bn_train_cl(mod, x)
        mod._nbt_pending = getattr(mod, "_nbt_pending", 0) + 1
        return y
    shape = [1, -1] + [1] * (x.dim() - 2)
    var, mean = torch.var_mean(x, dims, unbiased=False)
    if mod.track_running_stats:
        with torch.no_grad():
# ... 282 lines not shown
        self.norm_1, self.norm_2 = Norm(d_model), Norm(d_model)
        self.attn_1 = _MHA(heads, d_model)
        self.ff = _FF(d_model, d_ff=d_ff)
        self.dropout_1, self.dropout_2 = nn.Dropout(dropout), nn.Dropout(dropout)

    def forward(self, x, mask=None):
        x2 = self.norm_1(x)
        x = x + self.dropout_1(self.attn_1(x2, x2, x2, mask))
        x2 = self.norm_2(x)
        return x + self.dropout_2(self.ff(x2))


def scene_counts(batch_ids, batch_size):
    ids = batch_ids.view(-1, 1)
    return (ids == torch.arange(batch_size, device=batch_ids.device, dtype=batch_ids.dtype)).sum(0)


class BackboneTransformer(nn.Module):

    def __init__(self, d_model, N, heads, d_ff):
        super().__init__()
        self.d_model, self.N = d_model, N
        self.layers = nn.ModuleList([copy.deepcopy(_EncLayer(d_model, heads, d_ff)) for _ in range(N)])
        self.norm = Norm(d_model)
        self.position_linear = nn.Linear(3, d_model)

    def forward(self, xyz, features, batch_ids, batch_size=None):
        out = torch.zeros_like(features)
        if batch_size == 1 and features.shape[0] > 0:
            bounds = [0, features.shape[0]]
        else:
            nb = batch_size if batch_size is not None else int(batch_ids.max().item()) + 1
            counts = scene_counts(batch_ids, nb)
            ends = torch.cumsum(counts, 0)
            bounds = [0] + ends.tolist()
            if nb > 1 and features.is_cuda and features.shape[0] > 0:
                return self._forward_padded(xyz, features, batch_ids, bounds, ends - counts)
        nb = len(bounds) - 1
        for b in range(nb):
            s, e = bounds[b], bounds[b + 1]
            if e == s:
                continue
            rows = slice(s, e)
            pts = xyz[s:e].view(-1, 3)
            rel = (pts.unsqueeze(1) - pts.unsqueeze(0)).float().mean(dim=1)
            x = (features[s:e].view(-1, self.d_model) + self.position_linear(rel)).unsqueeze(0)
            for layer in self.layers:
                x = layer(x, mask=None)
            out[rows] = self.norm(x).squeeze(0)
        return out

    def _forward_padded(self, xyz, features, batch_ids, bounds, starts):
        nb, d = len(bounds) - 1, self.d_model
        M = features.shape[0]
        lens = [bounds[b + 1] - bounds[b] for b in range(nb)]
        L = max(lens)
        rels = []
        for b in range(nb):
            pts = xyz[bounds[b]:bounds[b + 1]].view(-1, 3)
            if pts.shape[0]:
                rels.append((pts.unsqueeze(1) - pts.unsqueeze(0)).float().mean(dim=1))
        x_all = features.view(-1, d) + self.position_linear(torch.cat(rels))
        bid = batch_ids.long()
        slot = torch.arange(M, device=features.device) - starts[bid] + bid * L
        x = x_all.new_zeros(nb * L, d).index_copy(0, slot, x_all).view(nb, L, d)
        mask = torch.zeros(nb * L, device=features.device, dtype=torch.long).index_fill_(0, slot, 1).view(nb, 1, L)
        for layer in self.layers:
            x = layer(x, mask=mask)
        return self.norm(x).view(nb * L, d)[slot]


class RelPosSpec:

    def __init__(self, geo_ctx, max_geo, query_locs, context_locs, lo, hi, gauss_B):
        self.geo_ctx, self.max_geo, self.query_locs, self.context_locs = geo_ctx, max_geo, query_locs, context_locs
        self.lo, self.hi, self.gauss_B = lo, hi, gauss_B


class LazyRelPos:

    def __init__(self, fn):
        self.fn, self.value = fn, None

    def get(self):
        if self.value is None:
            self.value = self.fn()
        return self.value


class TransformerDecoderLayer(nn.Module):
    def __init__(self, d_model, nhead=4, dim_feedforward=256, dropout=0.1, dropout_attn=None, activation="relu",
                 normalize_before=True, use_rel=False, norm_fn_name="ln"):
        super().__init__()
        if not use_rel or not normalize_before or norm_fn_name != "ln":
            raise NotImplementedError("GeoFormer uses the pre-norm relative-position layer (geoformer.py:122-129)")
        self.self_attn = nn.MultiheadAttention(d_model, nhead, dropout=dropout)
        self.norm1, self.norm2, self.norm3 = nn.LayerNorm(d_model), nn.LayerNorm(d_model), nn.LayerNorm(d_model)
        self.dropout1 = nn.Dropout(dropout, inplace=True)
        self.dropout2 = nn.Dropout(dropout, inplace=True)
        self.dropout3 = nn.Dropout(dropout, inplace=True)
        self.linear1 = nn.Linear(d_model, dim_feedforward)
        self.dropout = nn.Dropout(dropout, inplace=False)
        self.linear2 = nn.Linear(dim_feedforward, d_model)
        self.activation = {"relu": nn.ReLU, "gelu": nn.GELU}[activation]()
        self.nhead, self.use_rel, self.normalize_before = nhead, use_rel, normalize_before
        self.attn_mlp = nn.Sequential(BigLinear(d_model, d_model), nn.ReLU(), BigLinear(d_model, d_model))
        self.v_mlp = nn.Sequential(BigLinear(d_model, d_model))
        self.out_mlp = nn.Sequential(nn.Linear(d_model, d_model), nn.ReLU())

    def cross_attention(self, tgt2, memory, relative_pos):
        if isinstance(relative_pos, RelPosSpec):
            return self._cross_attention_fused(tgt2, memory, relative_pos)
        sim = self.attn_mlp(tgt2[:, None] - memory[None] + relative_pos)
        if sim.is_cuda and sim.dtype == torch.float32:
            from .. import pointops

            attn = pointops.softmax_dim1(sim, 1.0 / float(np.sqrt(sim.shape[-1])))
        else:
            attn = F.softmax(sim / np.sqrt(sim.shape[-1]), dim=1)
        v2 = self.v_mlp(memory[None] + relative_pos)
        return (attn * v2).sum(dim=1)

    def _cross_attention_fused(self, tgt2, memory, rp):
        from .. import pointops

        w1, w2, wv = self.attn_mlp[0], self.attn_mlp[2], self.v_mlp[0]
        key = (w1.weight._version, w2.weight._version, wv.weight._version, w1.weight.data_ptr())
        if getattr(self, "_wpack_key", None) != key:
            self._wpack = pointops.decoder_pack_weights(w1.weight.detach().contiguous(), w2.weight.detach().contiguous(),
                                                        wv.weight.detach().contiguous())
            self._wpack_key = key
        if torch.is_grad_enabled():
            Q1 = w1(tgt2.clone()).permute(1, 0, 2)
            K1 = _SplitKLinearFn.apply(memory, w1.weight, None).permute(1, 0, 2)
            Kv = wv(memory).permute(1, 0, 2)
            out = pointops.decoder_cross_attn_train(rp.geo_ctx, rp.max_geo, rp.query_locs, rp.context_locs, rp.lo, rp.hi,
                                                    rp.gauss_B, Q1, K1, Kv, w1.weight, w2.weight, wv.weight)
            return out.permute(1, 0, 2)
        Q1 = w1(tgt2).permute(1, 0, 2).contiguous()
        K1 = F.linear(memory, w1.weight).permute(1, 0, 2).contiguous()
        Kv = wv(memory).permute(1, 0, 2).contiguous()
        out = pointops.decoder_cross_attn(rp.geo_ctx, rp.max_geo, rp.query_locs, rp.context_locs, rp.lo, rp.hi,
                                          rp.gauss_B, Q1, K1, Kv, self._wpack, w2.bias.detach().contiguous())
        return out.permute(1, 0, 2)

    def forward(self, tgt, memory, tgt_mask=None, memory_mask=None, tgt_key_padding_mask=None,
                memory_key_padding_mask=None, pos=None, query_pos=None, relative_pos=None,
                return_attn_weights=False):
        tgt2 = self.norm1(tgt)
        q = k = tgt2 if query_pos is None else tgt2 + query_pos
        tgt2 = self.self_attn(q, k, value=tgt2, attn_mask=tgt_mask, key_padding_mask=tgt_key_padding_mask)[0]
        tgt = tgt + self.dropout1(tgt2)
        tgt2 = self.norm2(tgt)
        tgt = self.out_mlp(self.cross_attention(tgt2, memory, relative_pos))
        tgt = tgt + self.dropout2(tgt2)
        tgt2 = self.norm3(tgt)
        tgt2 = self.linear2(self.dropout(self.activation(self.linear1(tgt2))))
        tgt = tgt + self.dropout3(tgt2)
        return tgt, None


def _decoder_fused_cache(dec):
    from .. import pointops

    params = dec.__dict__.get("_gf_fused_params")
    if params is None:
        params = dec.__dict__["_gf_fused_params"] = list(dec.parameters())
    key = (params[0].data_ptr(), sum([p._version for p in params]))
    hit = dec.__dict__.get("_gf_fused")
    if hit is not None and hit["key"] == key:
        return hit
    with torch.no_grad():
        tables = [pointops.decoder_stage_tables(l, dec.norm) for l in dec.layers]
        wt = torch.stack([w for l in dec.layers for w in (l.attn_mlp[0].weight.t(), l.v_mlp[0].weight.t())]).contiguous()
        bs = torch.stack([b for l in dec.layers
                          for b in (torch.zeros_like(l.v_mlp[0].bias), l.v_mlp[0].bias)]).unsqueeze(1).contiguous()
        packs = [pointops.decoder_pack_weights(l.attn_mlp[0].weight.detach().contiguous(),
                                               l.attn_mlp[2].weight.detach().contiguous(),
                                               l.v_mlp[0].weight.detach().contiguous()) for l in dec.layers]
        b2 = [l.attn_mlp[2].bias.detach().contiguous() for l in dec.layers]
    hit = {"key": key, "tables": tables, "wt": wt, "bs": bs, "packs": packs, "b2": b2}
    dec.__dict__["_gf_fused"] = hit
    return hit


class TransformerDecoder(nn.Module):
    def __init__(self, decoder_layer, num_layers, norm_fn_name="ln", return_intermediate=False,
                 weight_init_name="xavier_uniform"):
        super().__init__()
        self.layers = nn.ModuleList([copy.deepcopy(decoder_layer) for _ in range(num_layers)])
        self.num_layers = num_layers
        self.norm = nn.LayerNorm(self.layers[0].linear2.out_features) if norm_fn_name == "ln" else None
        self.return_intermediate = return_intermediate
        for p in self.parameters():
            if p.dim() > 1:
                nn.init.xavier_uniform_(p)

    def _forward_fused(self, tgt, memory, query_pos, rp):
        from .. import pointops

        c = _decoder_fused_cache(self)
        nq, B, d = tgt.shape
        nc = memory.shape[0]
        L = len(self.layers)
        ff = self.layers[0].linear1.out_features
        mem = memory.permute(1, 0, 2).reshape(1, B * nc, d)
        kk = torch.baddbmm(c["bs"], mem.expand(2 * L, B * nc, d), c["wt"])
        state = pointops.decoder_token_state(nq, B, tgt.device)
        inter = torch.empty((L, nq, B, d), dtype=torch.float32, device=tgt.device)
        q1 = torch.empty((B, nq, d), dtype=torch.float32, device=tgt.device)
        tgt_c, qp = tgt.contiguous(), query_pos.contiguous()
        pointops.decoder_token_stage(None, tgt_c, qp, nq, B, 4, ff, None, c["tables"][0][1], state, None, q1)
        if isinstance(rp, LazyRelPos):
            rp = rp.get()
        for l in range(L):
            attn = pointops.decoder_cross_attn(rp.geo_ctx, rp.max_geo, rp.query_locs, rp.context_locs, rp.lo, rp.hi,
                                               rp.gauss_B, q1, kk[2 * l].view(B, nc, d), kk[2 * l + 1].view(B, nc, d),
                                               c["packs"][l], c["b2"][l])
            pre = c["tables"][l + 1][1] if l + 1 < L else None
            pointops.decoder_token_stage(attn, None, qp, nq, B, 4, ff, c["tables"][l][0], pre, state, inter[l],
                                         q1 if pre is not None else None)
        return inter

    def _train_fused_dropout(self):
        ps = set()
        for l in self.layers:
            ps |= {float(l.self_attn.dropout), float(l.dropout1.p), float(l.dropout2.p), float(l.dropout3.p),
                   float(l.dropout.p)}
            if not isinstance(l.activation, nn.ReLU) or not isinstance(l.norm1, nn.LayerNorm):
                return None
        if len(ps) != 1:
            return None
        return ps.pop() if self.layers[0].self_attn.training else 0.0

    def _forward_train_fused(self, tgt, memory, query_pos, rp, p):
        from .. import pointops

        x = tgt.permute(1, 0, 2).contiguous()
        qp = query_pos.permute(1, 0, 2).contiguous()
        seed = int(torch.randint(0, 2 ** 31 - 1, (1,)).item())
        inter = []
        d = memory.shape[-1]
        wk = torch.cat([w for layer in self.layers for w in (layer.attn_mlp[0].weight, layer.v_mlp[0].weight)], 0)
        bk = torch.cat([b for layer in self.layers for b in (torch.zeros_like(layer.v_mlp[0].bias), layer.v_mlp[0].bias)])
        kk = _SplitKLinearFn.apply(memory, wk, bk).split(d, dim=-1)
        for l, layer in enumerate(self.layers):
            pre, post = pointops.decoder_stage_tensors(layer, self.norm)
            w1, w2, wv = layer.attn_mlp[0], layer.attn_mlp[2], layer.v_mlp[0]
            t2n, q1 = pointops.decoder_pre_train(x, qp, l, p, seed, pre)
            K1 = kk[2 * l].permute(1, 0, 2)
            Kv = kk[2 * l + 1].permute(1, 0, 2)
            ca = pointops.decoder_cross_attn_train(rp.geo_ctx, rp.max_geo, rp.query_locs, rp.context_locs, rp.lo, rp.hi,
                                                   rp.gauss_B, q1, K1, Kv, w1.weight, w2.weight, wv.weight)
            x, it = pointops.decoder_post_train(ca, t2n, l, p, seed, post)
            inter.append(it)
        return torch.stack(inter).permute(0, 2, 1, 3)

    def forward(self, tgt, memory, tgt_mask=None, memory_mask=None, tgt_key_padding_mask=None,
                memory_key_padding_mask=None, pos=None, query_pos=None, relative_pos=None, transpose_swap=False,
                return_attn_weights=False):
        if isinstance(relative_pos, LazyRelPos) and (torch.is_grad_enabled() or self.layers[0].self_attn.training):
            relative_pos = relative_pos.get()
        shapes_ok = (isinstance(relative_pos, (RelPosSpec, LazyRelPos)) and tgt_mask is None and tgt_key_padding_mask is None
                     and query_pos is not None and self.norm is not None and self.return_intermediate
                     and tgt.shape[-1] == 64 and self.layers[0].nhead == 4
                     and self.layers[0].linear1.out_features % 16 == 0 and self.layers[0].linear1.out_features <= 256)
        if shapes_ok and not self.layers[0].self_attn.training and not torch.is_grad_enabled():
            return self._forward_fused(tgt, memory, query_pos, relative_pos)
        if isinstance(relative_pos, LazyRelPos):
            relative_pos = relative_pos.get()
        if (shapes_ok and torch.is_grad_enabled() and tgt.is_cuda and tgt.dtype == torch.float32
                and os.environ.get("GF_FUSED_DECODER_TRAIN", "1") != "0"):
            p = self._train_fused_dropout()
            if p is not None:
                return self._forward_train_fused(tgt, memory, query_pos, relative_pos, p)
        output, inter = tgt, []
        for layer in self.layers:
            output, _ = layer(output, memory, tgt_mask=tgt_mask, memory_mask=memory_mask,
                              tgt_key_padding_mask=tgt_key_padding_mask,
                              memory_key_padding_mask=memory_key_padding_mask, pos=pos, query_pos=query_pos,
                              relative_pos=relative_pos)
            if self.return_intermediate:
                inter.append(self.norm(output))
        if self.norm is not None:
            output = self.norm(output)
            if self.return_intermediate:
                inter[-1] = output
        return torch.stack(inter) if self.return_intermediate else output
```

### geoformer_amd/pointops.py

```python
from __future__ import annotations

import contextlib
import os
import threading

import numpy as np
import torch

from . import _lib
from ._lib import check, ptr, stream_ptr


def _f32c(t, name):
    if not (t.is_cuda and t.dtype == torch.float32 and t.is_contiguous()):
        raise RuntimeError(f"{name}: expected a contiguous float32 tensor on the GPU")
    return t


def _i32c(t, name):
    if not (t.is_cuda and t.dtype == torch.int32 and t.is_contiguous()):
        raise RuntimeError(f"{name}: expected a contiguous int32 tensor on the GPU")
    return t


# ... 291 lines not shown
    if st[0] != "MT19937" or not (1 <= k <= n <= 0x7fffffff):
        return np.random.choice(n, k, replace=False)
    key = np.ascontiguousarray(st[1], dtype=np.uint32).copy()
    pos = ctypes.c_int32(int(st[2]))
    if out is None or out.dtype != np.int64 or out.size < k or not out.flags.c_contiguous:
        out = np.empty(k, dtype=np.int64)
    check(_lib.load().gf_host_legacy_choice(key.ctypes.data, ctypes.addressof(pos), n, k, out.ctypes.data),
          "gf_host_legacy_choice")
    np.random.set_state((st[0], key, int(pos.value), st[3], st[4]))
    return out[:k]


def knn_radius(xyz, k, radius, sqrt_out=True, check_overflow=False, return_flag=False):
    _f32c(xyz, "xyz")
    n = xyz.shape[0]
    lib = _lib.load()
    dev = xyz.device
    D = torch.empty((n, k), dtype=torch.float32, device=dev)
    I = torch.empty((n, k), dtype=torch.int32, device=dev)
    deg = torch.empty(n, dtype=torch.int32, device=dev)
    scratch = torch.empty(lib.gf_knn_scratch_bytes(n) // 4 + 16, dtype=torch.int32, device=dev)
    check(lib.gf_knn_radius(ptr(xyz), n, k, float(radius), int(sqrt_out), ptr(D), ptr(I), ptr(deg), ptr(scratch),
                            stream_ptr()), "gf_knn_radius")
    if check_overflow:
        off = (lib.gf_knn_error_flag(ptr(scratch), n) - scratch.data_ptr()) // 4
        if int(scratch[off].item()) != 0:
            raise _lib.GeoFormerHipError("gf_knn_radius: a point has more in-radius neighbours than the kernel's "
                                         "candidate list holds (rows truncated)")
    if return_flag:
        off = (lib.gf_knn_error_flag(ptr(scratch), n) - scratch.data_ptr()) // 4
        return D, I, deg, scratch[off:off + 1]
    return D, I, deg


_SCRATCH = {}


def scratch(name, numel, dtype, device):
    dev = torch.device(device)
    key = (dev.index if dev.index is not None else torch.cuda.current_device(), torch.cuda.current_stream(dev).cuda_stream,
           name, dtype)
    t = _SCRATCH.get(key)
    if t is None or t.numel() < numel:
        _SCRATCH[key] = None
        t = _SCRATCH[key] = torch.empty(int(numel * 1.25) + 64, dtype=dtype, device=dev)
    return t[:numel]


def release_scratch(device=None):
    if device is not None:
        dev = torch.device(device)
        idx = dev.index if dev.index is not None else torch.cuda.current_device()
    for key in list(_SCRATCH):
        if device is None or key[0] == idx:
            del _SCRATCH[key]


def scratch_bytes():
    return sum(t.numel() * t.element_size() for t in _SCRATCH.values() if t is not None)


def geodesic_bfs(D, I, deg, src, radius, max_step, wg_threads=1024):
    _f32c(D, "D"); _i32c(I, "I"); _i32c(src, "src")
    n, K = D.shape
    nq = src.shape[0]
    dev = D.device
    geo = torch.empty((nq, n), dtype=torch.float32, device=dev)
    lib = _lib.load()
    keys = scratch("bfs_keys", nq * n, torch.int64, dev)
    qwords = int(lib.gf_geodesic_bfs_queue_words(n))
    queues = scratch("bfs_queues", nq * qwords, torch.int32, dev)
    check(lib.gf_geodesic_bfs_cfg(ptr(D), ptr(I), ptr(deg), n, K, ptr(src), nq, float(radius), int(max_step),
                                          ptr(geo), ptr(keys), ptr(queues), qwords, int(wg_threads), stream_ptr()),
          "gf_geodesic_bfs")
    return geo


def _mask_head_split_ws(N, device, split):
    if not split:
        return None
    return scratch("mask_head_split", _lib.load().gf_mask_head_split_bytes(N) // 8 + 1, torch.int64, device)


def mask_head(feat, coords, geo, qxyz, sqrt_max_geo, w1, b1, w2, b2, split=True):
    for t, name in ((feat, "feat"), (coords, "coords"), (qxyz, "qxyz"), (w1, "w1"), (b1, "b1"), (w2, "w2"), (b2, "b2")):
        _f32c(t, name)
    N, C = feat.shape
    nq = qxyz.shape[0]
    out = torch.empty((nq, N), dtype=torch.float32, device=feat.device)
    check(_lib.load().gf_mask_head_episodes(ptr(feat), ptr(coords), ptr(geo), ptr(qxyz), ptr(sqrt_max_geo), ptr(w1), ptr(b1),
                                            ptr(w2), ptr(b2), 0, N, nq, 1, C, ptr(_mask_head_split_ws(N, feat.device, split)),
                                            ptr(out), stream_ptr()), "gf_mask_head")
    return out


def mask_head_packed(feat, coords, geo, qxyz, sqrt_max_geo, params, split=True):
    return mask_head_episodes(feat, coords, geo, qxyz, sqrt_max_geo, params.unsqueeze(0), split=split)[0]


def mask_head_episodes(feat, coords, geo, qxyz, sqrt_max_geo, params, split=True):
    for t, name in ((feat, "feat"), (coords, "coords"), (qxyz, "qxyz"), (params, "params")):
        _f32c(t, name)
    N, C = feat.shape
    E, nq, ld = params.shape
    if ld != C * (C + 3) + C + C + 1 or qxyz.shape[0] != nq:
        raise RuntimeError(f"mask_head_episodes: params {tuple(params.shape)} for {qxyz.shape[0]} queries, C={C}")
    base = params.data_ptr()
    o_w2, o_b1, o_b2 = C * (C + 3), C * (C + 3) + C, C * (C + 3) + 2 * C
    out = torch.empty((E, nq, N), dtype=torch.float32, device=feat.device)
    check(_lib.load().gf_mask_head_episodes(ptr(feat), ptr(coords), ptr(geo), ptr(qxyz), ptr(sqrt_max_geo), base,
                                            base + 4 * o_b1, base + 4 * o_w2, base + 4 * o_b2, ld, N, nq, E, C,
                                            ptr(_mask_head_split_ws(N, feat.device, split)), ptr(out), stream_ptr()),
          "gf_mask_head_episodes")
    return out


class _MaskHeadFn(torch.autograd.Function):

    @staticmethod
    def forward(ctx, feat, params, coords, geo, qxyz, sqrt_max_geo):
        ctx.save_for_backward(feat, params, coords, geo, qxyz, sqrt_max_geo)
        return mask_head_packed(feat, coords, geo, qxyz, sqrt_max_geo, params)

    @staticmethod
    def backward(ctx, gout):
        feat, params, coords, geo, qxyz, mx = ctx.saved_tensors
        N, C = feat.shape
        nq, ld = params.shape
        lib = _lib.load()
        dparams = torch.empty_like(params)
        dfeat = torch.zeros_like(feat)
        scratch = torch.empty(lib.gf_mask_head_bwd_scratch_floats(N, nq), dtype=torch.float32, device=feat.device)
        base = params.data_ptr()
        o_w2, o_b1 = C * (C + 3), C * (C + 3) + C
        check(lib.gf_mask_head_bwd(ptr(feat), ptr(coords), ptr(geo), ptr(qxyz), ptr(mx), base, base + 4 * o_b1,
                                   base + 4 * o_w2, ptr(gout.contiguous()), ld, N, nq, C, ptr(dparams), ptr(dfeat),
                                   ptr(scratch), stream_ptr()), "gf_mask_head_bwd")
        return dfeat, dparams, None, None, None, None


class _MaskHeadEpisodesFn(torch.autograd.Function):

    @staticmethod
    def forward(ctx, feat, params, coords, geo, qxyz, sqrt_max_geo):
        ctx.save_for_backward(feat, params, coords, geo, qxyz, sqrt_max_geo)
        return mask_head_episodes(feat, coords, geo, qxyz, sqrt_max_geo, params)

    @staticmethod
    def backward(ctx, gout):
        feat, params, coords, geo, qxyz, mx = ctx.saved_tensors
        N, C = feat.shape
        E, nq, ld = params.shape
        lib = _lib.load()
        dparams = torch.empty_like(params)
        dfeat = torch.zeros_like(feat)
        scratch = torch.empty(lib.gf_mask_head_bwd_scratch_floats(N, E * nq), dtype=torch.float32, device=feat.device)
        base = params.data_ptr()
        o_w2, o_b1 = C * (C + 3), C * (C + 3) + C
        check(lib.gf_mask_head_bwd_episodes(ptr(feat), ptr(coords), ptr(geo), ptr(qxyz), ptr(mx), base, base + 4 * o_b1,
                                            base + 4 * o_w2, ptr(gout.contiguous()), ld, N, nq, E, C, ptr(dparams),
                                            ptr(dfeat), ptr(scratch), stream_ptr()), "gf_mask_head_bwd_episodes")
        return dfeat, dparams, None, None, None, None


def mask_head_train_episodes(feat, params, coords, geo, qxyz, sqrt_max_geo):
    for t, name in ((feat, "feat"), (coords, "coords"), (qxyz, "qxyz"), (params, "params")):
        _f32c(t, name)
    return _MaskHeadEpisodesFn.apply(feat, params, coords, geo, qxyz, sqrt_max_geo)


def mask_head_train(feat, params, coords, geo, qxyz, sqrt_max_geo):
    for t, name in ((feat, "feat"), (coords, "coords"), (qxyz, "qxyz"), (params, "params")):
        _f32c(t, name)
    return _MaskHeadFn.apply(feat, params, coords, geo, qxyz, sqrt_max_geo)


class PointwiseChain:

    def __init__(self, modules):
        import ctypes

        layers = []
        for m in modules:
            name = type(m).__name__
            if isinstance(m, (torch.nn.Linear, torch.nn.Conv1d, torch.nn.Conv2d)):
                W = m.weight.detach()
                W = W.reshape(W.shape[0], W.shape[1]).float().contiguous()
                bias = m.bias.detach().float() if m.bias is not None else torch.zeros(W.shape[0], device=W.device)
                layers.append([W, torch.ones_like(bias), bias.clone(), 0])
            elif isinstance(m, torch.nn.modules.batchnorm._BatchNorm):
                if m.training:
                    raise RuntimeError("PointwiseChain folds eval-mode BatchNorm only")
                s = (m.weight / torch.sqrt(m.running_var + m.eps)).detach().float()
                layers[-1][2] = (layers[-1][2] - m.running_mean.detach()) * s + m.bias.detach()
                layers[-1][1] = layers[-1][1] * s
            elif isinstance(m, torch.nn.ReLU):
# ... 128 lines not shown
        lib = _lib.load()
        B, T, _ = x.shape
        x, qpos = _f32c(x.contiguous(), "x"), _f32c(qpos.contiguous(), "qpos")
        params = [_f32c(t.detach().contiguous(), "decoder parameter") for t in params]
        t2n, q1 = torch.empty_like(x), torch.empty_like(x)
        save = torch.empty(lib.gf_decoder_pre_train_save_bytes(T, B) // 4, dtype=torch.float32, device=x.device)
        check(lib.gf_decoder_pre_train_fwd(ptr(x), ptr(qpos), T, B, _ptr_table(params), float(p), int(seed), int(layer),
                                           ptr(save), ptr(t2n), ptr(q1), stream_ptr()), "gf_decoder_pre_train_fwd")
        ctx.save_for_backward(x, qpos, t2n, save, *params)
        ctx.cfg = (int(layer), float(p), int(seed))
        ctx.set_materialize_grads(False)
        return t2n, q1

    @staticmethod
    def backward(ctx, d_t2n, d_q1):
        lib = _lib.load()
        x, qpos, t2n, save, *params = ctx.saved_tensors
        layer, p, seed = ctx.cfg
        B, T, _ = x.shape
        if d_t2n is None and d_q1 is None:
            return (None,) * (5 + len(params))
        d_t2n = None if d_t2n is None else _f32c(d_t2n.contiguous(), "d_t2n")
        d_q1 = None if d_q1 is None else _f32c(d_q1.contiguous(), "d_q1")
        work = torch.empty(lib.gf_decoder_pre_train_work_bytes(T, B) // 4, dtype=torch.float32, device=x.device)
        grads = torch.empty(lib.gf_decoder_pre_grad_floats(), dtype=torch.float32, device=x.device)
        dx, dqpos = torch.empty_like(x), torch.empty_like(x)
        check(lib.gf_decoder_pre_train_bwd(ptr(x), ptr(qpos), ptr(t2n), ptr(d_t2n), ptr(d_q1), T, B, _ptr_table(params), p,
                                           seed, layer, ptr(save), ptr(work), ptr(dx), ptr(dqpos), ptr(grads),
                                           stream_ptr()), "gf_decoder_pre_train_bwd")
        return (dx, dqpos, None, None, None) + tuple(_split_grads(grads, params))


class _DecoderPostTrainFn(torch.autograd.Function):

    @staticmethod
    def forward(ctx, ca, t2n, layer, p, seed, *params):
        lib = _lib.load()
        B, T, _ = ca.shape
        ca, t2n = _f32c(ca.contiguous(), "ca"), _f32c(t2n.contiguous(), "t2n")
        params = [_f32c(t.detach().contiguous(), "decoder parameter") for t in params]
        ff = params[4].shape[0]
        x3, inter = torch.empty_like(ca), torch.empty_like(ca)
        save = torch.empty(lib.gf_decoder_post_train_save_bytes(T, B, ff) // 4, dtype=torch.float32, device=ca.device)
        check(lib.gf_decoder_post_train_fwd(ptr(ca), ptr(t2n), T, B, ff, _ptr_table(params), float(p), int(seed), int(layer),
                                            ptr(save), ptr(x3), ptr(inter), stream_ptr()), "gf_decoder_post_train_fwd")
        ctx.save_for_backward(ca, x3, save, *params)
        ctx.cfg = (int(layer), float(p), int(seed), ff)
        ctx.set_materialize_grads(False)
        return x3, inter

    @staticmethod
    def backward(ctx, d_x3, d_inter):
        lib = _lib.load()
        ca, x3, save, *params = ctx.saved_tensors
        layer, p, seed, ff = ctx.cfg
        B, T, _ = ca.shape
        if d_x3 is None and d_inter is None:
            return (None,) * (5 + len(params))
        d_x3 = None if d_x3 is None else _f32c(d_x3.contiguous(), "d_x3")
        d_inter = None if d_inter is None else _f32c(d_inter.contiguous(), "d_inter")
        work = torch.empty(lib.gf_decoder_post_train_work_bytes(T, B, ff) // 4, dtype=torch.float32, device=ca.device)
        grads = torch.empty(lib.gf_decoder_post_grad_floats(ff), dtype=torch.float32, device=ca.device)
        d_ca, d_t2n = torch.empty_like(ca), torch.empty_like(ca)
        check(lib.gf_decoder_post_train_bwd(ptr(ca), ptr(x3), ptr(d_x3), ptr(d_inter), T, B, ff, _ptr_table(params), p, seed,
                                            layer, ptr(save), ptr(work), ptr(d_ca), ptr(d_t2n), ptr(grads), stream_ptr()),
              "gf_decoder_post_train_bwd")
        return (d_ca, d_t2n, None, None, None) + tuple(_split_grads(grads, params))


def decoder_pre_train(x, qpos, layer_index, p, seed, pre_params):
    return _DecoderPreTrainFn.apply(x, qpos, layer_index, p, seed, *pre_params)


def decoder_post_train(ca, t2n, layer_index, p, seed, post_params):
    return _DecoderPostTrainFn.apply(ca, t2n, layer_index, p, seed, *post_params)


def decoder_token_stage(attn_out, tgt_in, query_pos, nq, B, nhead, ff, post, pre, state, inter_out, q1_out):
    check(_lib.load().gf_decoder_token_stage(ptr(attn_out), ptr(tgt_in), ptr(query_pos), nq, B, 64, nhead, ff, post,
                                             pre, ptr(state), ptr(inter_out), ptr(q1_out), stream_ptr()),
          "gf_decoder_token_stage")


def decoder_token_state(nq, B, device):
    return torch.empty(_lib.load().gf_decoder_token_state_bytes(nq, B) // 4, dtype=torch.float32, device=device)


def proposal_stats(mask_logits, cls_logits, sem_prob, logit_thresh, score_thresh, npoint_thresh, min_class=4,
                   class_major=False):
    _f32c(mask_logits, "mask_logits"), _f32c(cls_logits, "cls_logits")
    nq, N = mask_logits.shape
    ncls = cls_logits.shape[1]
    if sem_prob.shape != ((ncls, N) if class_major else (N, ncls)):
        raise RuntimeError(f"sem_prob must be [{N},{ncls}] ([{ncls},{N}] class-major), got {tuple(sem_prob.shape)}")
    sem_prob = _f32c(sem_prob if class_major else sem_prob.t().contiguous(), "sem_prob")
    ints = torch.empty((3, nq), dtype=torch.int32, device=mask_logits.device)
    scores = torch.empty(nq, dtype=torch.float32, device=mask_logits.device)
    check(_lib.load().gf_proposal_stats(ptr(mask_logits), ptr(cls_logits), ptr(sem_prob), nq, N, ncls,
                                        float(logit_thresh), float(score_thresh), int(npoint_thresh), int(min_class),
                                        ptr(ints[0]), ptr(ints[1]), ptr(scores), ptr(ints[2]), stream_ptr()),
          "gf_proposal_stats")
    return ints[0], ints[1], scores, ints[2]


def proposal_stats_fs(mask_logits, sim, logit_thresh, score_thresh, npoint_thresh, sim_thresh):
    _f32c(mask_logits, "mask_logits"), _f32c(sim, "sim")
    nq, N = mask_logits.shape
    if sim.shape != (nq,):
        raise RuntimeError(f"sim must be [{nq}], got {tuple(sim.shape)}")
    ints = torch.empty((2, nq), dtype=torch.int32, device=mask_logits.device)
    scores = torch.empty(nq, dtype=torch.float32, device=mask_logits.device)
    check(_lib.load().gf_proposal_stats_fs(ptr(mask_logits), ptr(sim), nq, N, float(logit_thresh), float(score_thresh),
                                           int(npoint_thresh), float(sim_thresh), ptr(ints[0]), ptr(scores),
                                           ptr(ints[1]), stream_ptr()), "gf_proposal_stats_fs")
    return ints[0], scores, ints[1]


def proposal_select(final, cls_pred, scores):
    _i32c(final, "final"); _i32c(cls_pred, "cls_pred"); _f32c(scores, "scores")
    nq = final.shape[0]
    dev = final.device
    sel = torch.empty(nq, dtype=torch.int32, device=dev)
    cls = torch.empty(nq, dtype=torch.int64, device=dev)
    sc = torch.empty(nq, dtype=torch.float32, device=dev)
    cnt = torch.empty(1, dtype=torch.int32, device=dev)
    check(_lib.load().gf_proposal_select(ptr(final), ptr(cls_pred), ptr(scores), nq, ptr(sel), ptr(cls), ptr(sc), ptr(cnt),
                                         stream_ptr()), "gf_proposal_select")
    return sel, cls, sc, cnt


def proposal_scatter(mask_logits, sel, fg_idxs, logit_thresh, num_points):
    _f32c(mask_logits, "mask_logits"), _i32c(sel, "sel")
    if not (fg_idxs.is_cuda and fg_idxs.dtype == torch.int64 and fg_idxs.is_contiguous()):
        raise RuntimeError("fg_idxs: expected a contiguous int64 tensor on the GPU")
    out = torch.zeros((sel.shape[0], num_points), dtype=torch.int32, device=mask_logits.device)
    check(_lib.load().gf_proposal_scatter(ptr(mask_logits), ptr(sel), sel.shape[0], mask_logits.shape[1],
                                          ptr(fg_idxs), float(logit_thresh), int(num_points), ptr(out), stream_ptr()),
          "gf_proposal_scatter")
    return out


def relpos_prepare(geo, inds):
    _f32c(geo, "geo"); _i32c(inds, "inds")
    nq, n = geo.shape
    nc = inds.shape[0]
    geo_ctx = torch.empty((nq, nc), dtype=torch.float32, device=geo.device)
    max_geo = torch.empty(nq, dtype=torch.float32, device=geo.device)
    check(_lib.load().gf_relpos_prepare(ptr(geo), ptr(inds), nq, n, nc, ptr(geo_ctx), ptr(max_geo), stream_ptr()),
          "gf_relpos_prepare")
    return geo_ctx, max_geo


def mask_intersections(masks):
    _i32c(masks, "masks")
    n, N = masks.shape
    lib = _lib.load()
    scratch = torch.empty(lib.gf_mask_intersections_scratch_bytes(n, N) // 8 + 1, dtype=torch.int64,
                          device=masks.device)
    inter = torch.empty((n, n), dtype=torch.int32, device=masks.device)
    check(lib.gf_mask_intersections(ptr(masks), n, N, ptr(scratch), ptr(inter), stream_ptr()), "gf_mask_intersections")
    return inter


def overlap_layout(n, max_gt, extra_words=0):
    o_id = 2
    o_cnt = o_id + 2 * max_gt
    o_inter = o_cnt + max_gt
    o_extra = (o_inter + n * (max_gt + 1) + 1) // 2 * 2
    return {"id": o_id, "count": o_cnt, "inter": o_inter, "extra": o_extra, "total": o_extra + extra_words}


def instance_overlaps_packed(masks, gt_ids, class_ids, rows=None, max_gt=256, extra_words=0):
    _i32c(masks, "masks")
    if masks.dim() != 2:
        raise RuntimeError("masks: expected [n_rows, N]")
    if not (gt_ids.is_cuda and gt_ids.dtype == torch.int64 and gt_ids.is_contiguous() and gt_ids.dim() == 1):
        raise RuntimeError("gt_ids: expected a contiguous int64 vector on the GPU")
    _i32c(class_ids, "class_ids")
    n_rows, N = masks.shape
    if gt_ids.shape[0] != N:
        raise RuntimeError(f"gt_ids has {gt_ids.shape[0]} points, the masks {N}")
    if rows is not None:
        _i32c(rows, "rows")
    n = n_rows if rows is None else rows.shape[0]
    C = class_ids.shape[0]
    lay = overlap_layout(n, max_gt, extra_words)
    buf = torch.empty(lay["total"], dtype=torch.int32, device=masks.device)
    lib = _lib.load()
    scratch = torch.empty(lib.gf_instance_overlaps_scratch_bytes(N, C) // 4 + 1, dtype=torch.int32, device=masks.device)
    base = buf.data_ptr()
    check(lib.gf_instance_overlaps(ptr(masks), n_rows, N, ptr(rows), n, ptr(gt_ids), ptr(class_ids), C, max_gt,
                                   ptr(scratch), base, base + 4 * lay["id"], base + 4 * lay["count"],
                                   base + 4 * lay["inter"], stream_ptr()), "gf_instance_overlaps")
    return buf, lay


def instance_overlaps(masks, gt_ids, class_ids, rows=None, max_gt=256):
    while True:
        buf, lay = instance_overlaps_packed(masks, gt_ids, class_ids, rows, max_gt)
        G = int(buf[0])
        if G <= max_gt:
            break
        max_gt = G
    n = masks.shape[0] if rows is None else rows.shape[0]
    gt_id = buf[lay["id"]:lay["id"] + 2 * G].view(torch.int64)
    gt_count = buf[lay["count"]:lay["count"] + G]
    inter = buf[lay["inter"]:lay["inter"] + n * (G + 1)].view(n, G + 1)
    return gt_id, gt_count, inter


def semantic_confusion_limits():
    lib = _lib.load()
    return lib.gf_semantic_confusion_max_classes(), lib.gf_semantic_confusion_run_points()


def semantic_confusion(scores, labels, offsets, conf, *, lut=None, ignore_label=-100, map_ignore=-1, map_other=-1,
                       want_preds=True, offsets_host=None):
    _f32c(scores, "scores")
    if scores.dim() != 2:
        raise RuntimeError("scores: expected [N, C]")
    N, C = scores.shape
    S = 0
    if labels is not None:
        if not (labels.is_cuda and labels.dtype == torch.int64 and labels.is_contiguous() and labels.shape == (N,)):
            raise RuntimeError(f"labels: expected a contiguous int64 [{N}] tensor on the GPU")
        _i32c(offsets, "offsets")
        S = offsets.shape[0] - 1
        if not (conf.is_cuda and conf.dtype == torch.int64 and conf.is_contiguous() and conf.shape == (S, C + 1, C)):
            raise RuntimeError(f"conf: expected a contiguous int64 [{S}, {C + 1}, {C}] tensor on the GPU")
        if offsets_host is not None and not (offsets_host.device.type == "cpu" and offsets_host.dtype == torch.int32
                                             and offsets_host.is_contiguous() and offsets_host.shape == (S + 1,)):
            raise RuntimeError(f"offsets_host: expected a contiguous int32 [{S + 1}] host tensor")
# ... 682 lines not shown
```

### include/geoformer_hip.h

```cpp
#ifndef GEOFORMER_HIP_H
#define GEOFORMER_HIP_H

#include <stddef.h>
#include <stdint.h>

#ifdef __cplusplus
extern "C" {
#endif

#define GF_ABI_VERSION 7

typedef enum {
    GF_OK = 0,
    GF_ERR_INVALID_ARG = -1,
    GF_ERR_LAUNCH = -2,
    GF_ERR_UNSUPPORTED = -3,
    GF_ERR_CALLBACK = -4,
} gf_status;

int gf_abi_version(void);
const char* gf_last_error(void);

size_t gf_fg_scratch_bytes(int N);
int gf_fg_select(const float* scores, int N, int C, int cls, int mode, const float* locs, const int32_t* batch_idxs,
// ... 142 lines not shown
                             float* dgamma, float* dbeta, float* scratch, void* stream);

size_t gf_bn_train_cl_scratch_floats(int B, int C, long long L);
int gf_bn_relu_train_cl_fwd(const float* x, int B, int C, long long L, const float* gamma, const float* beta, float eps,
                            float momentum, int relu, float* running_mean, float* running_var, float* y,
                            float* save_mean, float* save_invstd, float* scratch, void* stream);
int gf_bn_relu_train_cl_bwd(const float* x, const float* y, const float* dy, int B, int C, long long L,
                            const float* gamma, const float* save_mean, const float* save_invstd, int relu, float* dx,
                            float* dgamma, float* dbeta, float* scratch, void* stream);


size_t gf_voxelize_idx_scratch_bytes(int N);
int gf_voxelize_idx_count(const long long* coords, int N, int ncol, int mode, void* scratch, int32_t* input_map,
                          int32_t* d_M_maxActive, void* stream);
int gf_voxelize_idx_fill(const long long* coords, int N, int ncol, int mode, void* scratch, const int32_t* input_map,
                         int M, int maxActive, long long* out_coords, int32_t* out_map, void* stream);

#define GF_FEEDER_MAX_COPIES 16
typedef struct {
    int slot, n_copies;
    const void* src[GF_FEEDER_MAX_COPIES];
    void* pinned[GF_FEEDER_MAX_COPIES];
    void* dev[GF_FEEDER_MAX_COPIES];
    size_t bytes[GF_FEEDER_MAX_COPIES];
    const long long* coords_dev;
    int N, ncol, mode, pad_;
    void* scratch;
    int32_t* input_map;
    int32_t* head_dev;
    int32_t* head_host;
    void* stream;
} GfFeederJob;
void* gf_feeder_create(int device);
int gf_feeder_submit(void* feeder, const GfFeederJob* job);
int gf_feeder_wait_issued(void* feeder, int slot);
int gf_feeder_wait_copied(void* feeder, int slot);
int gf_feeder_wait_head(void* feeder, int slot);
int gf_feeder_destroy(void* feeder);

int gf_voxelize_fp(const float* feats, const int32_t* rules, int M, int maxActive, int C, int average, float* out,
                   void* stream);
int gf_voxelize_bp(const float* d_out, const int32_t* rules, int M, int maxActive, int C, int average, float* d_feats,
                   void* stream);


int gf_gather_points(const float* points, const int32_t* idx, int b, int c, int n, int m, float* out, void* stream);
int gf_gather_points_grad(const float* grad_out, const int32_t* idx, int b, int c, int n, int m, float* grad_points,
                          void* stream);
int gf_group_points(const float* points, const int32_t* idx, int b, int c, int n, int npoints, int nsample, float* out,
                    void* stream);
int gf_group_points_grad(const float* grad_out, const int32_t* idx, int b, int c, int n, int npoints, int nsample,
                         float* grad_points, void* stream);
int gf_ball_query(const float* new_xyz, const float* xyz, int b, int n, int m, float radius, int nsample, int32_t* idx,
                  void* stream);
size_t gf_fps_scratch_bytes(int b);
int gf_furthest_point_sampling(const float* xyz, int b, int n, int m, int32_t* idxs, void* scratch, void* stream);
const int32_t* gf_fps_error_flag(void* scratch, int b);
int gf_furthest_point_sampling_resume(const float* xyz, int b, int n, int m, int m_known, int32_t* idxs,
                                      void* scratch, void* stream);


size_t gf_knn_scratch_bytes(int n);
int gf_knn_radius(const float* xyz, int n, int k, float radius, int sqrt_out, float* D, int32_t* I, int32_t* deg,
                  void* scratch, void* stream);
const int32_t* gf_knn_error_flag(void* scratch, int n);

size_t gf_geodesic_bfs_queue_words(int n);
int gf_geodesic_bfs(const float* D, const int32_t* I, const int32_t* deg, int n, int K, const int32_t* src, int nq,
                    float radius, int max_step, float* geo, void* keys_ws, void* queue_ws, void* stream);
int gf_geodesic_bfs_cfg(const float* D, const int32_t* I, const int32_t* deg, int n, int K, const int32_t* src, int nq,
                        float radius, int max_step, float* geo, void* keys_ws, void* queue_ws, size_t queue_words,
                        int wg_threads, void* stream);

int gf_mask_head(const float* feat, const float* coords, const float* geo, const float* qxyz,
                 const float* sqrt_max_geo, const float* w1, const float* b1, const float* w2, const float* b2, int N,
                 int nq, int C, float* out, void* stream);
int gf_mask_head_packed(const float* feat, const float* coords, const float* geo, const float* qxyz,
                        const float* sqrt_max_geo, const float* w1, const float* b1, const float* w2, const float* b2,
                        int ldp, int N, int nq, int C, float* out, void* stream);
size_t gf_mask_head_split_bytes(int N);
int gf_mask_head_episodes(const float* feat, const float* coords, const float* geo, const float* qxyz,
                          const float* sqrt_max_geo, const float* w1, const float* b1, const float* w2, const float* b2,
                          int ldp, int N, int nq, int E, int C, void* split_ws, float* out, void* stream);

size_t gf_mask_head_bwd_scratch_floats(int N, int nq);
int gf_mask_head_bwd(const float* feat, const float* coords, const float* geo, const float* qxyz,
                     const float* sqrt_max_geo, const float* w1, const float* b1, const float* w2, const float* gout,
                     int ldp, int N, int nq, int C, float* dparams, float* dfeat, float* scratch, void* stream);
int gf_mask_head_bwd_episodes(const float* feat, const float* coords, const float* geo, const float* qxyz,
                              const float* sqrt_max_geo, const float* w1, const float* b1, const float* w2,
                              const float* gout, int ldp, int N, int nq, int E, int C, float* dparams, float* dfeat,
                              float* scratch, void* stream);


int gf_pointwise_mlp(const float* x, int N, int n_layers, const float* const* W, const float* const* scale,
                     const float* const* shift, const int* channels, const int* relu, float* out, void* stream);
int gf_pointwise_mlp_rows(const float* x, const int32_t* rows, int N, int n_layers, const float* const* W,
                          const float* const* scale, const float* const* shift, const int* channels, const int* relu,
                          float* out, void* stream);

int gf_group_mlp_max(const float* grouped, int B, int npoint, int nsample, int n_layers, const float* const* W,
                     const float* const* scale, const float* const* shift, const int* channels, const int* relu,
                     float* out, void* stream);

int gf_ball_query_centres(const float* xyz, const int32_t* centre_idx, int b, int n, int m, float radius, int nsample,
                          float* new_xyz, int32_t* idx, void* stream);
int gf_point_grid_build(const float* xyz, int n, float radius, void* scratch, void* stream);
int gf_ball_query_grid(const float* xyz, int n, const int32_t* centre_idx, const float* centres, int m, float radius,
                       int nsample, void* scratch, int grid_ready, float* new_xyz, int32_t* idx, void* stream);
int gf_sa_group_mlp_max(const float* xyz, const float* feats, const int32_t* inds, int B, int n, int C, int npoint,
                        float radius, int nsample, int use_xyz, int normalize_xyz, int n_layers,
                        const float* const* W, const float* const* scale, const float* const* shift,
                        const int* channels, const int* relu, float* new_xyz, int32_t* idx, float* out, void* scratch,
                        int grid_ready, void* stream);

int gf_softmax_dim1_fwd(const float* x, int n0, int n1, int inner, float scale, float* y, void* stream);
int gf_softmax_dim1_bwd(const float* y, const float* gy, int n0, int n1, int inner, float scale, float* gx,
                        void* stream);


size_t gf_decoder_token_state_bytes(int nq, int B);
int gf_decoder_token_stage(const float* attn_out, const float* tgt_in, const float* query_pos, int nq, int B, int d,
                           int nhead, int ff, const float* const* post_params, const float* const* pre_params,
                           void* state, float* inter_out, float* q1_out, void* stream);

size_t gf_decoder_pre_train_save_bytes(int T, int B);
size_t gf_decoder_pre_train_work_bytes(int T, int B);
long long gf_decoder_pre_grad_floats(void);
int gf_decoder_pre_train_fwd(const float* x, const float* qpos, int T, int B, const float* const* params, float p,
                             unsigned seed, int layer, void* save, float* t2n, float* q1, void* stream);
int gf_decoder_pre_train_bwd(const float* x, const float* qpos, const float* t2n, const float* d_t2n, const float* d_q1,
                             int T, int B, const float* const* params, float p, unsigned seed, int layer, void* save,
                             void* work, float* dx, float* dqpos, float* grads, void* stream);
size_t gf_decoder_post_train_save_bytes(int T, int B, int ff);
size_t gf_decoder_post_train_work_bytes(int T, int B, int ff);
long long gf_decoder_post_grad_floats(int ff);
int gf_decoder_post_train_fwd(const float* ca, const float* t2n, int T, int B, int ff, const float* const* params,
                              float p, unsigned seed, int layer, void* save, float* x3, float* inter, void* stream);
int gf_decoder_post_train_bwd(const float* ca, const float* x3, const float* d_x3, const float* d_inter, int T, int B,
                              int ff, const float* const* params, float p, unsigned seed, int layer, void* save,
                              void* work, float* d_ca, float* d_t2n, float* grads, void* stream);


int gf_proposal_stats(const float* mask_logits, const float* cls_logits, const float* sem_prob, int nq, int N,
                      int ncls, float logit_thresh, float score_thresh, int npoint_thresh, int min_class,
                      int* cls_pred, int* npoints, float* scores, int* final_mask, void* stream);

int gf_proposal_stats_fs(const float* mask_logits, const float* sim, int nq, int N, float logit_thresh,
                         float score_thresh, int npoint_thresh, float sim_thresh, int* npoints, float* scores,
                         int* final_mask, void* stream);

int gf_proposal_scatter(const float* mask_logits, const int* sel, int n_sel, int N, const long long* fg_idxs,
                        float logit_thresh, int num_points, int* proposals, void* stream);

int gf_relpos_prepare(const float* geo, const int32_t* inds, int nq, int n, int nc, float* geo_ctx, float* max_geo,
                      void* stream);

int gf_proposal_select(const int32_t* final_, const int32_t* cls_pred, const float* scores, int nq, int32_t* sel,
                       long long* cls_out, float* scores_out, int32_t* d_count, void* stream);

size_t gf_mask_intersections_scratch_bytes(int n, int N);
int gf_mask_intersections(const int32_t* masks, int n, int N, void* scratch, int32_t* inter, void* stream);

#define GF_PROP_SCENE_FIELDS 6
int gf_proposal_stats_batched(const long long* table, int S, int nq, const float* cls_logits, const float* sem_prob,
                              long long sem_stride, int ncls, float logit_thresh, float score_thresh, int npoint_thresh,
                              int min_class, int* cls_pred, int* npoints, float* scores, int* final_mask, void* stream);
int gf_proposal_select_batched(const int32_t* final_, const int32_t* cls_pred, const float* scores, int S, int nq,
                               int32_t* sel, long long* cls_out, float* scores_out, int32_t* counts, void* stream);
int gf_proposal_scatter_batched(const long long* table, int S, int nq, const int32_t* sel, const int32_t* counts,
                                int total_rows, int max_N, const long long* fg_idxs, float logit_thresh, int* packed,
                                void* stream);

#define GF_NMS_SCENE_FIELDS 8
#define GF_NMS_MAX_N 1024
int gf_mask_intersections_batched(const long long* table, int S, long long max_waves, long long max_pairs, void* bits,
                                  int32_t* inter, void* stream);
int gf_matrix_nms_batched(const long long* table, int S, const int32_t* inter, int kernel, float sigma,
                          float final_score_thresh, int32_t* picks, int32_t* pick_counts, void* stream);
int gf_greedy_nms_batched(const long long* table, int S, const int32_t* inter, float threshold, int32_t* picks,
                          int32_t* pick_counts, void* stream);
int gf_greedy_nms_ious(const float* ious, const float* scores, int n, float threshold, int32_t* picks,
                       int32_t* pick_count, void* stream);

#define GF_LBL_SCENE_FIELDS 12
#define GF_LBL_CHUNK 4096
#define GF_LBL_OWN_SPLIT 4
#define GF_LBL_TABLE_INTS 5
#define GF_LBL_TABLE_FLOATS 10
int gf_label_map_batched(const long long* table, int S, long long max_points, int max_picks, float min_score,
                         void* bits, float* part_f, int32_t* part_cnt, int32_t* own_part, int32_t* owner, int32_t* ids,
                         int32_t* tab_i, float* tab_f, void* stream);

size_t gf_instance_overlaps_scratch_bytes(int N, int C);
int gf_instance_overlaps(const int32_t* masks, int n_rows, int N, const int32_t* rows, int n, const long long* gt_ids,
                         const int32_t* class_ids, int C, int max_gt, void* scratch, int32_t* d_G, long long* gt_id,
                         int32_t* gt_count, int32_t* inter, void* stream);

int gf_semantic_confusion_max_classes(void);
int gf_semantic_confusion_run_points(void);
int gf_semantic_confusion(const float* scores, const long long* labels, const int32_t* offsets,
                          const int32_t* offsets_host, int S, int N, int C, const int32_t* lut, int L,
                          long long ignore_label, int map_ignore, int map_other, int32_t* preds, long long* conf,
                          void* stream);

int gf_panoptic_max_rows(void);
int gf_panoptic_run_points(void);
size_t gf_panoptic_overlaps_scratch_bytes(int S, int N, int C);
int gf_panoptic_overlaps(const int32_t* owner, const int32_t* ids, const int32_t* sem, const long long* gt_ids,
                         const int32_t* offsets, const int32_t* offsets_host, int S, int N, const int32_t* class_ids,
                         const int32_t* is_stuff, int C, const int32_t* stuff_of_sem, int L, int n_stuff, int P,
                         int max_gt, void* scratch, int32_t* pan, int32_t* d_G, long long* gt_id, int32_t* inter,
                         void* stream);

int gf_segment_pool_scene_fields(void);
int gf_segment_pool_chunk_points(void);
size_t gf_segment_pool_scratch_bytes(int S, long long n_fg, int nq);
int gf_segment_pool_batched(const long long* table, const long long* table_host, int S, int nq,
                            const long long* keys_sorted, const int32_t* order, long long n_fg, long long max_N,
                            void* scratch, void* stream);

size_t gf_point_normals_scratch_bytes(int n);
int gf_point_normals(const float* xyz, const int32_t* I, const int32_t* deg, int n, int k, float* out, void* stream);
size_t gf_smooth_components_scratch_bytes(int n);
int gf_smooth_components(const float* xyz, const float* normals4, const int32_t* I, const int32_t* deg, int n, int k,
                         float cos_thresh, float offset, float flatness, int min_points, int32_t* ids_out,
                         void* scratch, void* stream);


size_t gf_backbone_transformer_scratch_bytes(int M);
int gf_backbone_transformer_num_params(int n_layers);
int gf_backbone_transformer(const float* feats, const int* coords, const int* scene_offsets, int n_scenes, int M,
                            int c, int n_layers, const float* const* params, void* scratch, float* out,
                            void* stream);

size_t gf_backbone_transformer_train_save_bytes(int M, int n_layers);
size_t gf_backbone_transformer_train_work_bytes(int M, int n_layers, int n_scenes);
long long gf_backbone_transformer_grad_floats(int c, int n_layers);
int gf_backbone_transformer_train_fwd(const float* feats, const int* coords, int n_scenes, int M, int c, int n_layers,
                                      const float* const* params, float p, unsigned seed, void* save, float* out,
                                      void* stream);
int gf_backbone_transformer_train_bwd(const float* feats, const float* dout, int n_scenes, int M, int c, int n_layers,
                                      const float* const* params, float p, unsigned seed, void* save, void* work,
                                      float* dfeats, float* grads, void* stream);


size_t gf_decoder_wpack_floats(void);
int gf_decoder_pack_weights(const float* W1, const float* W2, const float* Wv, float* Wpack, void* stream);

int gf_decoder_cross_attn(const float* geo_ctx, const float* max_geo, const float* qloc, const float* cloc,
                          const float* lo, const float* hi, const float* gaussB, const float* Q1, const float* K1,
                          const float* Kv, const float* Wpack, const float* b2, int B, int nq, int nc, int d, float* out,
                          float* stat_m, float* stat_l, void* stream);
int gf_decoder_cross_attn_cfg(const float* geo_ctx, const float* max_geo, const float* qloc, const float* cloc,
                              const float* lo, const float* hi, const float* gaussB, const float* Q1, const float* K1,
                              const float* Kv, const float* Wpack, const float* b2, int B, int nq, int nc, int d,
                              float* out, float* stat_m, float* stat_l, int wg_waves, void* stream);

size_t gf_decoder_cross_attn_bwd_scratch_floats(int B, int nq, int nc);
int gf_decoder_cross_attn_bwd(const float* geo_ctx, const float* max_geo, const float* qloc, const float* cloc,
                              const float* lo, const float* hi, const float* gaussB, const float* Q1, const float* K1,
                              const float* Kv, const float* Wpack, const float* W2, const float* out, const float* stat_m,
                              const float* stat_l, const float* gout, int B, int nq, int nc, int d, float* dQ1, float* dK1,
                              float* dKv, float* dW, float* scratch, void* stream);


int gf_sec_op(int kind, const float* inp, const int32_t* offsets, int nProposal, int C, float* out, void* stream);
int gf_roipool_fp(const float* feats, const int32_t* offsets, int nProposal, int C, float* out, int32_t* maxidx,
                  void* stream);
int gf_roipool_bp(const float* d_out, const int32_t* maxidx, int nProposal, int C, float* d_feats, void* stream);
int gf_get_iou(const int32_t* proposals_idx, const int32_t* proposals_offset, const long long* instance_labels,
               const int32_t* instance_pointnum, int nInstance, int nProposal, float* iou, void* stream);
size_t gf_ballquery_batch_p_scratch_bytes(int n);
int gf_ballquery_batch_p(const float* xyz, const int32_t* batch_idxs, const int32_t* batch_offsets, int n, int meanActive,
                         float radius, int32_t* idx, int32_t* start_len, int32_t* d_cumsum, void* scratch, void* stream);
int gf_bfs_cluster_host(const int32_t* h_semantic_label, const int32_t* h_ball_query_idxs, const int32_t* h_start_len,
                        int N, int threshold, int32_t* h_cluster_idxs, int32_t* h_cluster_offsets, int32_t* h_nCluster,
                        int32_t* h_sumNPoint);
int gf_three_nn(const float* unknown, const float* known, int b, int n, int m, float* dist2, int32_t* idx, void* stream);
int gf_three_interpolate(const float* points, const int32_t* idx, const float* weight, int b, int c, int m, int n,
                         float* out, void* stream);
int gf_three_interpolate_grad(const float* grad_out, const int32_t* idx, const float* weight, int b, int c, int n, int m,
                              float* grad_points, void* stream);

#define GF_AUG_REC 320
#define GF_AUG_MAX_INST 4096
#define GF_AUG_MAX_CROP 64
#define GF_AUG_LUT 128
#define GF_AUG_STAT 10
#define GF_AUG_HEAD 16
enum {
    GF_AUG_R_M = 0, GF_AUG_R_SHIFT = 9, GF_AUG_R_FLIP = 12, GF_AUG_R_THETA = 13, GF_AUG_R_AMAX0 = 14,
    GF_AUG_R_AMAX1 = 17, GF_AUG_R_MIN = 20, GF_AUG_R_MAX = 23, GF_AUG_R_CHOSEN = 26, GF_AUG_R_ERR = 27,
    GF_AUG_R_CAP0 = 28, GF_AUG_R_BASE0 = 29, GF_AUG_R_CAP1 = 30, GF_AUG_R_BASE1 = 31, GF_AUG_R_PCMIN = 32,
    GF_AUG_R_PCMAX = 35, GF_AUG_R_NINST = 38, GF_AUG_R_IBASE = 39, GF_AUG_R_COUNTS = 64, GF_AUG_R_CROPU = 128,
    GF_AUG_R_PBASE = 40, GF_AUG_R_CLASS = 41, GF_AUG_R_SUPID = 42,
    GF_AUG_R_BMIN = 43, GF_AUG_R_BMAX = 46, GF_AUG_R_BCNT = 49, GF_AUG_R_BLMAX = 50
};
enum { GF_AUG_H_N = 0, GF_AUG_H_NINST = 1, GF_AUG_H_ERR = 2, GF_AUG_H_LMAX = 3, GF_AUG_H_SHAPE = 6 };
enum { GF_AUG_ERR_CELLS = 1, GF_AUG_ERR_INST = 2, GF_AUG_ERR_NOINST = 4 };
typedef struct {
    int B, n_raw, max_inst, pad_;
    const double* raw;
    const long long* raw_off;
    long long* rec;
    double* xyz_middle;
    double* xyz;
    float* noise[2];
    float* work[2];
    long long cells[2];
    int32_t* flags;
    int32_t* lab;
    int32_t* inst;
    int32_t* start;
    int32_t* cursor;
    int32_t* block_sums;
    int32_t* block_off;
    int32_t* sidx;
    uint32_t* bitmap;
    int32_t* inst_map;
    long long* inst_stats;
    long long* locs;
    float* locs_float;
    double* feats;
    long long* labels;
    long long* instance_labels;
    float* instance_infos;
    int32_t* instance_pointnum;
    int32_t* offsets;
    float* pc_mins;
    float* pc_maxs;
    int32_t* head;
} GfAugBatch;
int gf_aug_scan_blocks(int n_raw);
int gf_aug_draw(const GfAugBatch* b, unsigned long long seed, long long batch_index, int K, void* stream);
int gf_aug_transform(const GfAugBatch* b, int s0, int ns, double scale, int max_scene_points, void* stream);
int gf_aug_elastic(const GfAugBatch* b, int s0, int ns, int pass, int gran, double mag, int fill,
                   unsigned long long seed, long long batch_index, int max_scene_points, long long max_cells,
                   void* stream);
int gf_aug_crop(const GfAugBatch* b, int s0, int ns, int full_scale, int K, long long max_npoint, int max_scene_points,
// ... 17 lines not shown
```

### include/geoformer_hip_dev.h

```cpp
#ifndef GEOFORMER_HIP_DEV_H
#define GEOFORMER_HIP_DEV_H

#include "geoformer_hip.h"

#ifdef __cplusplus
extern "C" {
#endif

int gf_dev_conv_fwd_timed(const float* in, const float* Wp, const int32_t* nbr, const uint32_t* gmask,
                          const int32_t* steps, int K, int M_in, int M_out, int ld, int Cin, int Cout, const float* in_scale, const float* in_shift,
                          const float* residual, const float* out_scale, const float* out_shift, float* out, void* ev_start,
                          void* ev_stop, void* stream);

int gf_dev_conv_knobs(int split, int wide, int pair, int ldsw, int block);

int gf_dev_conv_knobs_g16(int use, int ldsw, int gpw, int pipe);

int gf_dev_conv_knob_flat(int use, int max_items);

int gf_dev_conv_knob_lw(int use, int min_groups);

int gf_dev_conv_plan(const float* in, const float* Wp, const int32_t* nbr, const uint32_t* gmask, const int32_t* steps,
                     const int32_t* flat, int K, int M_in, int M_out, int ld, int Cin, int Cout, const float* in_scale,
                     const float* in_shift, const float* residual, const float* out_scale, const float* out_shift, float* out,
                     float* out_act, int* desc);

int gf_dev_conv_chunks(int n);
int gf_dev_conv_g16p_wpb(int wpb);

int gf_dev_unet_probe(int mode);
unsigned long long gf_dev_host_wait_ns(int reset);
int gf_dev_unet_probe_read(int max_records, int* meta, float* us);
int gf_dev_unet_probe_read2(int max_records, int* meta, float* us, float* us_kernel);
int gf_dev_conv_kernel_events(void* start, void* stop);
int gf_dev_conv_kernel_events_taken(void);

int gf_dev_op_kernel_events(int op, void* start, void* stop);
int gf_dev_op_kernel_events_taken(int op);
void* gf_dev_event_create(void);
int gf_dev_event_destroy(void* event);
int gf_dev_event_elapsed_us(void* start, void* stop, float* us);

int gf_dev_cross_attn_bf3(int on);

int gf_dev_bfs_qcap_max(int qcap);

int gf_dev_panoptic_lds_bins(int bins);

int gf_dev_fps_plan(int n, int* G, int* P, int* inst, int* bs_log2, int* per_launch);

#ifdef __cplusplus
}
#endif
#endif
```

Measured before the change: 225.1.

## Fuse decoder self-attn, cross-attn and FFN into one per-query kernel

Adds a fused decoder-layer kernel that runs the previous layer's self-attention projection, the geometric cross-attention context loop with bf16x3 MFMA, the output projection, LayerNorm and FFN, and the next layer's QKV projection in a single workgroup per query. It also adds a hoisted mask-head split workspace and a raw row-max relpos gather, so max_geo can be reduced inside the kernel. The aim is to remove many small kernel launches and intermediate global-memory round trips in the decoder. In exchange the workgroup holds 1024 threads with large LDS and register use, and the small per-query GEMV stages may leave the GPU underused.

```diff
diff --git a/geoformer_amd/csrc/decoder_attn.hip b/geoformer_amd/csrc/decoder_attn.hip
--- a/geoformer_amd/csrc/decoder_attn.hip
+++ b/geoformer_amd/csrc/decoder_attn.hip
@@ -1,6 +1,7 @@
 #include <stdlib.h>
 
 #include "common.h"
+#include "decoder_layer.h"
 
 #define DA_WAVES 16
 #define DA_D 64
@@ -407,6 +408,387 @@
     }
 }
 
+template <int WAVES, int NT>
+__device__ __forceinline__ void da_bf3_ctx_loop(const uint4* sW3, const float4* sQ1,
+                                                const float4 (*sB)[2][4], const float* __restrict__ geo_ctx,
+                                                const float* __restrict__ cloc, const float* __restrict__ K1,
+                                                const float* __restrict__ Kv, int nc, float mg, float qx, float qy, float qz,
+                                                float lx, float ly, float lz, float ix, float iy, float iz, int w, int lane,
+                                                float (&sm)[4][4], float (&sl)[4][4], float (&sa)[4][4]) {
+    const int g = lane >> 4, j = lane & 15;
+    constexpr float kScale2 = 0.125f * 1.44269504088896341f;
+    const int ntiles = (nc + 15) >> 4;
+    for (int t0 = w * NT; t0 < ntiles; t0 += WAVES * NT) {
+        bool valid[NT];
+        int cc[NT];
+        DaPieces RP[NT];
+#pragma unroll
+        for (int u = 0; u < NT; u++) {
+            const int ctx = (t0 + u) * 16 + j;
+            valid[u] = ctx < nc;
+            cc[u] = valid[u] ? ctx : nc - 1;
+            const float gd = geo_ctx[cc[u]];
+            float g0 = gd, g1 = gd, g2 = gd;
+            if (gd < 0.f) {
+                g0 = mg + fabsf(qx - cloc[cc[u] * 3 + 0]);
+                g1 = mg + fabsf(qy - cloc[cc[u] * 3 + 1]);
+                g2 = mg + fabsf(qz - cloc[cc[u] * 3 + 2]);
+            }
+            const float t0f = (g0 - lx) * ix, t1f = (g1 - ly) * iy, t2f = (g2 - lz) * iz;
+            float R[4][4];
+#pragma unroll
+            for (int half = 0; half < 2; half++) {
+                const float4 b0 = sB[0][half][g], b1 = sB[1][half][g], b2v = sB[2][half][g];
+                const float p[4] = {fmaf(t2f, b2v.x, fmaf(t1f, b1.x, t0f * b0.x)), fmaf(t2f, b2v.y, fmaf(t1f, b1.y, t0f * b0.y)),
+                                    fmaf(t2f, b2v.z, fmaf(t1f, b1.z, t0f * b0.z)), fmaf(t2f, b2v.w, fmaf(t1f, b1.w, t0f * b0.w))};
+#pragma unroll
+                for (int e = 0; e < 4; e++) {
+                    R[half][e] = __builtin_amdgcn_sinf(p[e]);
+                    R[2 + half][e] = __builtin_amdgcn_cosf(p[e]);
+                }
+            }
+            da_split_pack(R, RP[u]);
+        }
+        float H[NT][4][4];
+        f32x4 V[NT][4];
+#pragma unroll
+        for (int rb = 0; rb < 4; rb++) {
+            f32x4 acc[NT], vv[NT];
+#pragma unroll
+            for (int u = 0; u < NT; u++) {
+                acc[u] = (f32x4){0.f, 0.f, 0.f, 0.f};
+                vv[u] = (f32x4){0.f, 0.f, 0.f, 0.f};
+            }
+            da_gemm_bf3_n<NT>(sW3, 0, rb, lane, RP, acc);
+            const float4 q1 = sQ1[rb * 4 + g];
+#pragma unroll
+            for (int u = 0; u < NT; u++) {
+                const float4 k1 = *reinterpret_cast<const float4*>(K1 + (size_t)cc[u] * DA_D + rb * 16 + 4 * g);
+                H[u][rb][0] = fmaxf(acc[u][0] + q1.x - k1.x, 0.f);
+                H[u][rb][1] = fmaxf(acc[u][1] + q1.y - k1.y, 0.f);
+                H[u][rb][2] = fmaxf(acc[u][2] + q1.z - k1.z, 0.f);
+                H[u][rb][3] = fmaxf(acc[u][3] + q1.w - k1.w, 0.f);
+            }
+            da_gemm_bf3_n<NT>(sW3, 2, rb, lane, RP, vv);
+#pragma unroll
+            for (int u = 0; u < NT; u++) V[u][rb] = vv[u];
+            __builtin_amdgcn_sched_barrier(0);
+        }
+        DaPieces HP[NT];
+#pragma unroll
+        for (int u = 0; u < NT; u++) da_split_pack(H[u], HP[u]);
+#pragma unroll
+        for (int rb = 0; rb < 4; rb++) {
+            f32x4 s[NT];
+#pragma unroll
+            for (int u = 0; u < NT; u++) s[u] = (f32x4){0.f, 0.f, 0.f, 0.f};
+            da_gemm_bf3_n<NT>(sW3, 1, rb, lane, HP, s);
+#pragma unroll
+            for (int u = 0; u < NT; u++) {
+                const float4 kv = *reinterpret_cast<const float4*>(Kv + (size_t)cc[u] * DA_D + rb * 16 + 4 * g);
+                const float kvv[4] = {kv.x, kv.y, kv.z, kv.w};
+                if (valid[u]) {
+#pragma unroll
+                    for (int r = 0; r < 4; r++) {
+                        const float x = s[u][r] * kScale2;
+                        const float val = V[u][rb][r] + kvv[r];
+                        const float mn = fmaxf(sm[rb][r], x);
+                        const float corr = __builtin_amdgcn_exp2f(sm[rb][r] - mn), p = __builtin_amdgcn_exp2f(x - mn);
+                        sl[rb][r] = sl[rb][r] * corr + p;
+                        sa[rb][r] = sa[rb][r] * corr + p * val;
+                        sm[rb][r] = mn;
+                    }
+                }
+            }
+            __builtin_amdgcn_sched_barrier(0);
+        }
+    }
+}
+
+template <int WAVES>
+__device__ __forceinline__ void da_bf3_merge(float (*sRed)[WAVES][DA_D], const float (&sm)[4][4], const float (&sl)[4][4],
+                                             const float (&sa)[4][4], int tid, float& A, float& L) {
+    const int lane = tid & 63, w = tid >> 6, g = lane >> 4, j = lane & 15;
+#pragma unroll
+    for (int rb = 0; rb < 4; rb++)
+#pragma unroll
+        for (int r = 0; r < 4; r++) {
+            const float m = da_row_max(sm[rb][r]);
+            if (j == 0) sRed[0][w][rb * 16 + 4 * g + r] = m;
+        }
+    __syncthreads();
+    if (tid < DA_D) {
+        float m = sRed[0][0][tid];
+#pragma unroll
+        for (int u = 1; u < WAVES; u++) m = fmaxf(m, sRed[0][u][tid]);
+        sRed[0][0][tid] = m;
+    }
+    __syncthreads();
+#pragma unroll
+    for (int rb = 0; rb < 4; rb++)
+#pragma unroll
+        for (int r = 0; r < 4; r++) {
+            const int c = rb * 16 + 4 * g + r;
+            const float f = __builtin_amdgcn_exp2f(sm[rb][r] - sRed[0][0][c]);
+            const float l = da_row_sum(sl[rb][r] * f), a = da_row_sum(sa[rb][r] * f);
+            if (j == 0) {
+                sRed[1][w][c] = l;
+                sRed[2][w][c] = a;
+            }
+        }
+    __syncthreads();
+    L = 0.f, A = 0.f;
+    if (tid < DA_D) {
+#pragma unroll
+        for (int u = 0; u < WAVES; u++) {
+            L += sRed[1][u][tid];
+            A += sRed[2][u][tid];
+        }
+    }
+}
+
+__device__ __forceinline__ float da_dot4(float4 w, float4 x) { return fmaf(w.w, x.w, fmaf(w.z, x.z, fmaf(w.y, x.y, w.x * x.x))); }
+__device__ __forceinline__ float da_vec_layernorm(const float* S, int lane, float wl, float bl) {
+    const float v = S[lane];
+    const float mu = gf_wave_sum(v) / (float)DL_D;
+    const float dv = v - mu;
+    const float q = gf_wave_sum(dv * dv);
+    const float rstd = 1.0f / sqrtf(q / (float)DL_D + 1e-5f);
+    return dv * rstd * wl + bl;
+}
+
+#ifdef DL_TRACE
+__device__ unsigned long long* g_da_trace = nullptr;
+extern "C" int gf_dev_da_trace(void* p) {
+    GF_TRY(hipMemcpyToSymbol(HIP_SYMBOL(g_da_trace), &p, sizeof(p)));
+    return GF_OK;
+}
+#define DA_STAMP(k) do { if (g_da_trace && threadIdx.x == 0) g_da_trace[((size_t)(blockIdx.y * gridDim.x + blockIdx.x)) * 16 + (k)] = __builtin_amdgcn_s_memtime(); } while (0)
+#else
+#define DA_STAMP(k) do { } while (0)
+#endif
+
+template <int WAVES>
+__global__ __launch_bounds__(WAVES * 64) void k_decoder_layer_fused(
+    const float* __restrict__ geo_ctx, const float* __restrict__ max_geo, const float* __restrict__ qloc,
+    const float* __restrict__ cloc, const float* __restrict__ lo, const float* __restrict__ hi,
+    const float* __restrict__ gaussB, float* __restrict__ Q1, const float* __restrict__ K1, const float* __restrict__ Kv,
+    const uint4* __restrict__ Wp3, int nq, int nc, const float* __restrict__ query_pos, int B, int ff, int has_pro,
+    int has_pre, DlPre pro, DlPost po, DlPre pre, float* __restrict__ state, float* __restrict__ qkv_alt, int qkv_in,
+    float* __restrict__ inter_out) {
+    static_assert(WAVES == 16, "k_decoder_layer_fused: 1 024 threads = 64 outputs x 16 input parts");
+    extern __shared__ __attribute__((aligned(16))) unsigned char da_smem[];
+    uint4* sW3 = reinterpret_cast<uint4*>(da_smem);
+    __shared__ float4 sQ1[16];
+    __shared__ float4 sB[3][2][4];
+    __shared__ float sRed[3][WAVES][DA_D];
+    __shared__ __attribute__((aligned(16))) float sO[DL_D], sX[DL_D], sT[DL_D], sQ[DL_D], sT2[DL_D], sH[DL_MAXFF];
+    const int qi = blockIdx.x, b = blockIdx.y;
+    const int tid = threadIdx.x, lane = tid & 63, w = tid >> 6, g = lane >> 4, j = lane & 15;
+    const int o16 = tid >> 4;
+    DA_STAMP(0);
+    for (int t = tid; t < DA_WPACK_BF3_U4; t += WAVES * 64) sW3[t] = Wp3[t];
+    if (tid >= 64 && tid < 64 + 24) {
+        const int e = tid - 64, axis = e >> 3, half = (e >> 2) & 1, gg = e & 3;
+        sB[axis][half][gg] = *reinterpret_cast<const float4*>(gaussB + axis * 32 + half * 16 + 4 * gg);
+    }
+    float* X = state + (size_t)b * nq * (DL_STATE_ROWS * DL_D);
+    const float* TGT2 = X + (size_t)nq * DL_D;
+    float* qkv0 = X + (size_t)nq * (2 * DL_D);
+    float* qkv1 = qkv_alt + (size_t)b * nq * (3 * DL_D);
+    const float* QKVi = qkv_in ? qkv1 : qkv0;
+    float* QKVo = qkv_in ? qkv0 : qkv1;
+    const size_t qrow = (size_t)b * nq + qi;
+    float mg = max_geo[qrow];
+    if (mg < 0.f) {
+        float m = -INFINITY;
+        for (int t = tid; t < nq; t += WAVES * 64) m = fmaxf(m, max_geo[(size_t)b * nq + t]);
+        m = gf_wave_max(m);
+        if (lane == 0) sRed[0][0][w] = m;
+        __syncthreads();
+        mg = sRed[0][0][0];
+#pragma unroll
+        for (int u = 1; u < WAVES; u++) mg = fmaxf(mg, sRed[0][0][u]);
+        __syncthreads();
+    }
+    if (has_pro) {
+        const float4 w_op = reinterpret_cast<const float4*>(pro.opw)[tid], w_w1 = reinterpret_cast<const float4*>(pro.w1w)[tid];
+        const float b_op = pro.opb[o16], b_w1 = pro.w1b[o16], xres = X[(size_t)qi * DL_D + o16];
+        const float n2w = pro.n2w[lane], n2b = pro.n2b[lane];
+        const float* qp_ = QKVi + (size_t)qi * (3 * DL_D) + g * DL_DK;
+        const float4 q0 = *reinterpret_cast<const float4*>(qp_), q1v = *reinterpret_cast<const float4*>(qp_ + 4),
+                     q2 = *reinterpret_cast<const float4*>(qp_ + 8), q3 = *reinterpret_cast<const float4*>(qp_ + 12);
+        auto score = [&](int key) {
+            const float* kp = QKVi + (size_t)min(key, nq - 1) * (3 * DL_D) + DL_D + g * DL_DK;
+            const float4 k0 = *reinterpret_cast<const float4*>(kp), k1v = *reinterpret_cast<const float4*>(kp + 4),
+                         k2 = *reinterpret_cast<const float4*>(kp + 8), k3 = *reinterpret_cast<const float4*>(kp + 12);
+            const float s = (da_dot4(k0, q0) + da_dot4(k1v, q1v)) + (da_dot4(k2, q2) + da_dot4(k3, q3));
+            return key < nq ? s * 0.25f : -INFINITY;
+        };
+        const bool one_trip = nq <= WAVES * 16;
+        float s_keep = -INFINITY, mx = -INFINITY;
+#pragma unroll 1
+        for (int k0 = w * 16; k0 < nq; k0 += WAVES * 16) {
+            s_keep = score(k0 + j);
+            mx = fmaxf(mx, s_keep);
+        }
+        mx = da_row_max(mx);
+        if (j == 0) sRed[0][0][w * DL_H + g] = mx;
+        __syncthreads();
+        mx = sRed[0][0][g];
+#pragma unroll
+        for (int u = 1; u < WAVES; u++) mx = fmaxf(mx, sRed[0][0][u * DL_H + g]);
+        float oacc[DL_DK], l = 0.f;
+#pragma unroll
+        for (int c = 0; c < DL_DK; c++) oacc[c] = 0.f;
+#pragma unroll 1
+        for (int k0 = w * 16; k0 < nq; k0 += WAVES * 16) {
+            const int key = k0 + j;
+            const float sc = one_trip ? s_keep : score(key);
+            const float pi = __builtin_amdgcn_exp2f((sc - mx) * 1.4426950408889634f);
+            const float* vp = QKVi + (size_t)min(key, nq - 1) * (3 * DL_D) + 2 * DL_D + g * DL_DK;
+            l += pi;
+#pragma unroll
+            for (int c4 = 0; c4 < 4; c4++) {
+                const float4 v = *reinterpret_cast<const float4*>(vp + 4 * c4);
+                oacc[4 * c4 + 0] = fmaf(pi, v.x, oacc[4 * c4 + 0]);
+                oacc[4 * c4 + 1] = fmaf(pi, v.y, oacc[4 * c4 + 1]);
+                oacc[4 * c4 + 2] = fmaf(pi, v.z, oacc[4 * c4 + 2]);
+                oacc[4 * c4 + 3] = fmaf(pi, v.w, oacc[4 * c4 + 3]);
+            }
+        }
+        l = da_row_sum(l);
+        if (j == 0) sRed[2][w][g] = l;
+#pragma unroll
+        for (int c = 0; c < DL_DK; c++) {
+            const float a = da_row_sum(oacc[c]);
+            if (j == 0) sRed[1][w][g * DL_DK + c] = a;
+        }
+        __syncthreads();
+        if (tid < DL_D) {
+            float a = 0.f, ls = 0.f;
+#pragma unroll
+            for (int u = 0; u < WAVES; u++) {
+                a += sRed[1][u][tid];
+                ls += sRed[2][u][tid >> 4];
+            }
+            sO[tid] = a / ls;
+        }
+        __syncthreads();
+        DA_STAMP(1);
+        {
+            const float acc = da_row_sum(da_dot4(w_op, reinterpret_cast<const float4*>(sO)[j]));
+            if (j == 0) sX[o16] = (acc + b_op) + xres;
+        }
+        __syncthreads();
+        if (w == 0) sT2[lane] = da_vec_layernorm(sX, lane, n2w, n2b);
+        __syncthreads();
+        {
+            const float acc = da_row_sum(da_dot4(w_w1, reinterpret_cast<const float4*>(sT2)[j]));
+            if (j == 0) {
+                reinterpret_cast<float*>(sQ1)[o16] = acc + b_w1;
+                Q1[qrow * DA_D + o16] = acc + b_w1;
+            }
+        }
+        DA_STAMP(2);
+    } else {
+        if (tid < 16) sQ1[tid] = *reinterpret_cast<const float4*>(Q1 + qrow * DA_D + tid * 4);
+        if (tid >= 128 && tid < 128 + DL_D) sT2[tid - 128] = TGT2[(size_t)qi * DL_D + (tid - 128)];
+    }
+    geo_ctx += qrow * nc;
+    cloc += (size_t)b * nc * 3;
+    K1 += (size_t)b * nc * DA_D;
+    Kv += (size_t)b * nc * DA_D;
+    const float qx = qloc[qrow * 3 + 0], qy = qloc[qrow * 3 + 1], qz = qloc[qrow * 3 + 2];
+    const float lx = lo[b * 3 + 0], ly = lo[b * 3 + 1], lz = lo[b * 3 + 2];
+    const float ix = 1.0f / (hi[b * 3 + 0] - lx), iy = 1.0f / (hi[b * 3 + 1] - ly), iz = 1.0f / (hi[b * 3 + 2] - lz);
+    float sm[4][4], sl[4][4], sa[4][4];
+#pragma unroll
+    for (int rb = 0; rb < 4; rb++)
+#pragma unroll
+        for (int r = 0; r < 4; r++) {
+            sm[rb][r] = -3.0e38f;
+            sl[rb][r] = 0.f;
+            sa[rb][r] = 0.f;
+        }
+    __syncthreads();
+    DA_STAMP(3);
+
+    da_bf3_ctx_loop<WAVES, 1>(sW3, sQ1, sB, geo_ctx, cloc, K1, Kv, nc, mg, qx, qy, qz, lx, ly, lz, ix, iy, iz, w, lane, sm, sl, sa);
+    DA_STAMP(4);
+    const size_t tok = ((size_t)qi * B + b) * DL_D;
+    const float4 w_om = reinterpret_cast<const float4*>(po.omw)[tid];
+    const float4 z4 = make_float4(0.f, 0.f, 0.f, 0.f);
+    const bool l1_on = o16 < ff, l2_on = 4 * j < ff;
+    const float4 w_l1 = l1_on ? reinterpret_cast<const float4*>(po.l1w)[tid] : z4;
+    const float4 w_l2 = l2_on ? *reinterpret_cast<const float4*>(po.l2w + (size_t)o16 * ff + 4 * j) : z4;
+    const float b_om = po.omb[o16], b_l1 = l1_on ? po.l1b[o16] : 0.f, b_l2 = po.l2b[o16];
+    const float n3w = po.n3w[lane], n3b = po.n3b[lane], fnw = po.fnw[lane], fnb = po.fnb[lane];
+    float4 w_ip[3];
+    float b_ip[3], n1w = 0.f, n1b = 0.f, qpv = 0.f;
+#pragma unroll
+    for (int i = 0; i < 3; i++) {
+        w_ip[i] = z4;
+        b_ip[i] = 0.f;
+    }
+    if (has_pre) {
+#pragma unroll
+        for (int i = 0; i < 3; i++) {
+            w_ip[i] = reinterpret_cast<const float4*>(pre.ipw)[i * (WAVES * 64) + tid];
+            b_ip[i] = pre.ipb[i * DL_D + o16];
+        }
+        n1w = pre.n1w[lane], n1b = pre.n1b[lane];
+        qpv = query_pos[tok + lane];
+    }
+    float A, L;
+    da_bf3_merge<WAVES>(sRed, sm, sl, sa, tid, A, L);
+    if (tid < DA_D) sO[tid] = A / L;
+    __syncthreads();
+    DA_STAMP(5);
+    {
+        const float acc = da_row_sum(da_dot4(w_om, reinterpret_cast<const float4*>(sO)[j]));
+        if (j == 0) sX[o16] = fmaxf(acc + b_om, 0.f) + sT2[o16];
+    }
+    __syncthreads();
+    if (w == 0) sT[lane] = da_vec_layernorm(sX, lane, n3w, n3b);
+    __syncthreads();
+    {
+        const float4 x = reinterpret_cast<const float4*>(sT)[j];
+        const float acc = da_row_sum(da_dot4(w_l1, x));
+        if (j == 0 && l1_on) sH[o16] = fmaxf(acc + b_l1, 0.f);
+        for (int o = DL_D + o16; o < ff; o += DL_D) {
+            const float a2 = da_row_sum(da_dot4(*reinterpret_cast<const float4*>(po.l1w + (size_t)o * DL_D + 4 * j), x));
+            if (j == 0) sH[o] = fmaxf(a2 + po.l1b[o], 0.f);
+        }
+    }
+    __syncthreads();
+    {
+        float part = l2_on ? da_dot4(w_l2, reinterpret_cast<const float4*>(sH)[j]) : 0.f;
+        for (int k = DL_D + 4 * j; k < ff; k += DL_D)
+            part += da_dot4(*reinterpret_cast<const float4*>(po.l2w + (size_t)o16 * ff + k), *reinterpret_cast<const float4*>(sH + k));
+        const float acc = da_row_sum(part);
+        if (j == 0) sX[o16] += acc + b_l2;
+    }
+    __syncthreads();
+    DA_STAMP(6);
+    if (w == 0) inter_out[tok + lane] = da_vec_layernorm(sX, lane, fnw, fnb);
+    if (!has_pre) return;
+    if (w == 1) {
+        const float v = da_vec_layernorm(sX, lane, n1w, n1b);
+        sT[lane] = v;
+        sQ[lane] = v + qpv;
+    }
+    if (w == 2) X[(size_t)qi * DL_D + lane] = sX[lane];
+    __syncthreads();
+#pragma unroll
+    for (int i = 0; i < 3; i++) {
+        const float4 x = reinterpret_cast<const float4*>(i < 2 ? sQ : sT)[j];
+        const float acc = da_row_sum(da_dot4(w_ip[i], x));
+        if (j == 0) QKVo[(size_t)qi * (3 * DL_D) + i * DL_D + o16] = acc + b_ip[i];
+    }
+    DA_STAMP(7);
+}
+
 extern "C" size_t gf_decoder_wpack_floats(void) { return (size_t)DA_WPACK_F32 + (size_t)DA_WPACK_BF3_U4 * 4; }
 
 __global__ void k_decoder_pack(const float* __restrict__ W1, const float* __restrict__ W2, const float* __restrict__ Wv,
@@ -491,6 +873,65 @@
                                      int nq, int nc, int d, float* out, float* stat_m, float* stat_l, void* stream) {
     return gf_decoder_cross_attn_cfg(geo_ctx, max_geo, qloc, cloc, lo, hi, gaussB, Q1, K1, Kv, Wpack, b2, B, nq, nc, d, out,
                                      stat_m, stat_l, 16, stream);
+}
+
+static int g_da_fused = -1;
+extern "C" int gf_dev_decoder_fused(int on) {
+    g_da_fused = on < 0 ? -1 : (on != 0);
+    return GF_OK;
+}
+extern "C" int gf_decoder_layer_fused_ok(int wg_waves) {
+    int on = g_da_fused;
+    if (on < 0) {
+        const char* e = getenv("GF_DECODER_FUSED");
+        on = !(e && e[0] == '0' && !e[1]);
+    }
+    return on && wg_waves == 16 && g_da_bf3 != 0;
+}
+
+extern "C" size_t gf_decoder_layer_fused_qkv_bytes(int nq, int B) {
+    return (size_t)(nq > 0 ? nq : 0) * (B > 0 ? B : 0) * (3 * DL_D) * sizeof(float);
+}
+
+extern "C" int gf_decoder_layer_fused(const float* geo_ctx, const float* max_geo, const float* qloc, const float* cloc,
+                                      const float* lo, const float* hi, const float* gaussB, float* Q1, const float* K1,
+                                      const float* Kv, const float* Wpack, int B, int nq, int nc, int d, int nhead, int ff,
+                                      const float* query_pos, const float* const* pro_params,
+                                      const float* const* post_params, const float* const* pre_params, void* state,
+                                      void* qkv_alt, int qkv_in, float* inter_out, void* stream) {
+    GF_CHECK_ARG(d == DA_D && nhead == DL_H, "gf_decoder_layer_fused: built for d_model=64, 4 heads (got %d, %d)", d, nhead);
+    GF_CHECK_ARG(ff > 0 && ff % 16 == 0 && ff <= DL_MAXFF, "gf_decoder_layer_fused: dim_feedforward %d not in 16..%d", ff,
+                 DL_MAXFF);
+    GF_CHECK_ARG(B >= 0 && nq >= 0 && nc >= 1, "gf_decoder_layer_fused: bad sizes");
+    GF_CHECK_ARG(geo_ctx && max_geo && qloc && cloc && lo && hi && gaussB && Q1 && K1 && Kv && Wpack && state && qkv_alt && inter_out,
+                 "gf_decoder_layer_fused: null argument");
+    GF_CHECK_ARG(post_params, "gf_decoder_layer_fused: the layer's post table is required");
+    GF_CHECK_ARG(!pre_params || query_pos, "gf_decoder_layer_fused: pre needs query_pos");
+    GF_CHECK_ARG(qkv_in == 0 || qkv_in == 1, "gf_decoder_layer_fused: qkv_in is 0 or 1");
+    GF_CHECK_ARG(gf_decoder_layer_fused_ok(16), "gf_decoder_layer_fused: switched off (gf_dev_decoder_fused / gf_dev_cross_attn_bf3)");
+    if (B == 0 || nq == 0) return GF_OK;
+    DlPre pro = {}, pre = {};
+    DlPost po = {};
+    for (int i = 0; i < 10; i++) {
+        GF_CHECK_ARG(post_params[i] && (!pro_params || pro_params[i]) && (!pre_params || pre_params[i]),
+                     "gf_decoder_layer_fused: parameter %d of a table is null", i);
+    }
+    po = {post_params[0], post_params[1], post_params[2], post_params[3], post_params[4],
+          post_params[5], post_params[6], post_params[7], post_params[8], post_params[9]};
+    if (pro_params)
+        pro = {pro_params[0], pro_params[1], pro_params[2], pro_params[3], pro_params[4],
+               pro_params[5], pro_params[6], pro_params[7], pro_params[8], pro_params[9]};
+    if (pre_params)
+        pre = {pre_params[0], pre_params[1], pre_params[2], pre_params[3], pre_params[4],
+               pre_params[5], pre_params[6], pre_params[7], pre_params[8], pre_params[9]};
+    const size_t lds = (size_t)DA_WPACK_BF3_U4 * sizeof(uint4);
+    gf_allow_lds((const void*)k_decoder_layer_fused<DA_BF3_WAVES>, (int)lds);
+    GF_LAUNCH_OP(GF_OP_CROSS_ATTN, (k_decoder_layer_fused<DA_BF3_WAVES>), dim3(nq, B), dim3(DA_BF3_WAVES * 64), lds,
+                 (hipStream_t)stream, geo_ctx, max_geo, qloc, cloc, lo, hi, gaussB, Q1, K1, Kv,
+                 reinterpret_cast<const uint4*>(Wpack + DA_WPACK_F32), nq, nc, query_pos, B, ff, pro_params ? 1 : 0,
+                 pre_params ? 1 : 0, pro, po, pre, (float*)state, (float*)qkv_alt, qkv_in, inter_out);
+    GF_CHECK_LAUNCH("gf_decoder_layer_fused");
+    return GF_OK;
 }
 
 
diff --git a/geoformer_amd/csrc/decoder_layer.h b/geoformer_amd/csrc/decoder_layer.h
--- a/geoformer_amd/csrc/decoder_layer.h
+++ b/geoformer_amd/csrc/decoder_layer.h
@@ -6,6 +6,15 @@
 #define DL_DK 16
 #define DL_THREADS 1024
 #define DL_MAXFF 256
+
+#define DL_STATE_ROWS 5
+
+struct DlPost {
+    const float *omw, *omb, *n3w, *n3b, *l1w, *l1b, *l2w, *l2b, *fnw, *fnb;
+};
+struct DlPre {
+    const float *n1w, *n1b, *ipw, *ipb, *opw, *opb, *n2w, *n2b, *w1w, *w1b;
+};
 
 #define DL_LD 68
 #define DL_LDH 260
diff --git a/geoformer_amd/csrc/decoder_layer.hip b/geoformer_amd/csrc/decoder_layer.hip
--- a/geoformer_amd/csrc/decoder_layer.hip
+++ b/geoformer_amd/csrc/decoder_layer.hip
@@ -1,11 +1,4 @@
 #include "decoder_layer.h"
-
-struct DlPost {
-    const float *omw, *omb, *n3w, *n3b, *l1w, *l1b, *l2w, *l2b, *fnw, *fnb;
-};
-struct DlPre {
-    const float *n1w, *n1b, *ipw, *ipb, *opw, *opb, *n2w, *n2b, *w1w, *w1b;
-};
 
 #define DL_TILE_THREADS 256
 
@@ -30,7 +23,7 @@
     const int b = blockIdx.y, t0 = blockIdx.x * 16;
     const int nvalid = min(16, T - t0);
     const int lane = threadIdx.x & 63, wave = threadIdx.x >> 6, nw = DL_TILE_THREADS / 64;
-    float* X = state + (size_t)b * T * (5 * DL_D);
+    float* X = state + (size_t)b * T * (DL_STATE_ROWS * DL_D);
     float* TGT2 = X + (size_t)T * DL_D;
     float* QKV = TGT2 + (size_t)T * DL_D;
     const int lds = B * DL_D;
@@ -148,7 +141,7 @@
     const int nvalid = min(16, T - t0);
     const int lane = threadIdx.x & 63, wave = threadIdx.x >> 6, nw = DL_TILE_THREADS / 64;
     const int j = lane & 15, g = lane >> 4;
-    float* X = state + (size_t)b * T * (5 * DL_D);
+    float* X = state + (size_t)b * T * (DL_STATE_ROWS * DL_D);
     float* TGT2 = X + (size_t)T * DL_D;
     const float* QKV = TGT2 + (size_t)T * DL_D;
     DL_STAMP(16);
@@ -243,7 +236,7 @@
 }
 
 extern "C" size_t gf_decoder_token_state_bytes(int nq, int B) {
-    return (size_t)(nq > 0 ? nq : 0) * (B > 0 ? B : 0) * (5 * DL_D) * sizeof(float);
+    return (size_t)(nq > 0 ? nq : 0) * (B > 0 ? B : 0) * (DL_STATE_ROWS * DL_D) * sizeof(float);
 }
 
 extern "C" int gf_decoder_token_stage(const float* attn_out, const float* tgt_in, const float* query_pos, int nq, int B,
diff --git a/geoformer_amd/csrc/mask_head.hip b/geoformer_amd/csrc/mask_head.hip
--- a/geoformer_amd/csrc/mask_head.hip
+++ b/geoformer_amd/csrc/mask_head.hip
@@ -187,6 +187,10 @@
                                      const float* sqrt_max_geo, const float* w1, const float* b1, const float* w2,
                                      const float* b2, int ldp, int N, int nq, int E, int C, void* split_ws, float* out,
                                      void* stream);
+extern "C" int gf_mask_head_episodes_cfg(const float* feat, const float* coords, const float* geo, const float* qxyz,
+                                         const float* sqrt_max_geo, const float* w1, const float* b1, const float* w2,
+                                         const float* b2, int ldp, int N, int nq, int E, int C, void* split_ws,
+                                         int split_ready, float* out, void* stream);
 extern "C" size_t gf_mask_head_split_bytes(int N) { return (size_t)(N > 0 ? N : 0) * 16 * 3 * sizeof(unsigned short); }
 extern "C" int gf_mask_head(const float* feat, const float* coords, const float* geo, const float* qxyz,
                             const float* sqrt_max_geo, const float* w1, const float* b1, const float* w2,
@@ -204,6 +208,25 @@
                                      const float* sqrt_max_geo, const float* w1, const float* b1, const float* w2,
                                      const float* b2, int ldp, int N, int nq_scene, int E, int C, void* split_ws, float* out,
                                      void* stream) {
+    return gf_mask_head_episodes_cfg(feat, coords, geo, qxyz, sqrt_max_geo, w1, b1, w2, b2, ldp, N, nq_scene, E, C, split_ws,
+                                     0, out, stream);
+}
+
+extern "C" int gf_mask_head_split(const float* feat, int N, void* split_ws, void* stream) {
+    GF_CHECK_ARG(N >= 0 && (N == 0 || (feat && split_ws)), "gf_mask_head_split: bad arguments");
+    GF_CHECK_ARG(((uintptr_t)split_ws % 8) == 0, "gf_mask_head_split: split_ws must be 8-byte aligned");
+    if (N == 0) return GF_OK;
+    const int n16 = N * 16;
+    hipLaunchKernelGGL(k_mh_split, dim3(gf_div_up(n16, 256)), dim3(256), 0, (hipStream_t)stream, feat, n16,
+                       (unsigned short*)split_ws);
+    GF_CHECK_LAUNCH("gf_mask_head_split");
+    return GF_OK;
+}
+
+extern "C" int gf_mask_head_episodes_cfg(const float* feat, const float* coords, const float* geo, const float* qxyz,
+                                         const float* sqrt_max_geo, const float* w1, const float* b1, const float* w2,
+                                         const float* b2, int ldp, int N, int nq_scene, int E, int C, void* split_ws,
+                                         int split_ready, float* out, void* stream) {
     GF_CHECK_ARG(ldp >= 0, "gf_mask_head: negative parameter stride");
     GF_CHECK_ARG(C == 16, "gf_mask_head: only the 16-channel mask head (m=16) is implemented, got C=%d", C);
     GF_CHECK_ARG(N >= 0 && nq_scene >= 0 && E >= 1, "gf_mask_head: bad sizes");
@@ -220,10 +243,12 @@
     dim3 grid((unsigned)((waves + 3) / 4));
     hipStream_t st = (hipStream_t)stream;
     const unsigned short* fs = (const unsigned short*)split_ws;
+    GF_CHECK_ARG(fs || !split_ready, "gf_mask_head: split_ready without split_ws");
     if (fs) {
         GF_CHECK_ARG(((uintptr_t)fs % 8) == 0, "gf_mask_head: split_ws must be 8-byte aligned");
         const int n16 = N * 16;
-        hipLaunchKernelGGL(k_mh_split, dim3(gf_div_up(n16, 256)), dim3(256), 0, st, feat, n16, (unsigned short*)split_ws);
+        if (!split_ready)
+            hipLaunchKernelGGL(k_mh_split, dim3(gf_div_up(n16, 256)), dim3(256), 0, st, feat, n16, (unsigned short*)split_ws);
     }
 #define MH_LAUNCH(GEO_, SPLIT_)                                                                                          \
     do {                                                                                                                 \
diff --git a/geoformer_amd/csrc/proposal.hip b/geoformer_amd/csrc/proposal.hip
--- a/geoformer_amd/csrc/proposal.hip
+++ b/geoformer_amd/csrc/proposal.hip
@@ -218,6 +218,16 @@
     return GF_OK;
 }
 
+extern "C" int gf_relpos_gather(const float* geo, const int32_t* inds, int nq, int n, int nc, float* geo_ctx,
+                                float* row_max, void* stream) {
+    GF_CHECK_ARG(geo && inds && geo_ctx && row_max, "gf_relpos_gather: null argument");
+    GF_CHECK_ARG(nq >= 0 && n >= 1 && nc >= 1, "gf_relpos_gather: bad sizes");
+    if (nq == 0) return GF_OK;
+    hipLaunchKernelGGL(k_relpos_gather, dim3(nq), dim3(256), 0, (hipStream_t)stream, geo, inds, n, nc, geo_ctx, row_max);
+    GF_CHECK_LAUNCH("gf_relpos_gather");
+    return GF_OK;
+}
+
 __global__ __launch_bounds__(1024) void k_proposal_select(const int32_t* __restrict__ final_, const int32_t* __restrict__ cls_pred,
                                                           const float* __restrict__ scores, int nq,
                                                           int32_t* __restrict__ sel, long long* __restrict__ cls_out,
diff --git a/geoformer_amd/model/geoformer.py b/geoformer_amd/model/geoformer.py
--- a/geoformer_amd/model/geoformer.py
+++ b/geoformer_amd/model/geoformer.py
@@ -757,13 +757,14 @@
             for ev in pend.pop(_stream_key(), None) or ():
                 torch.cuda.current_stream().wait_event(ev)
 
-    def relative_position_embedding(self, context_locs, query_locs, pc_dims, geo_dists, pre_enc_inds):
+    def relative_position_embedding(self, context_locs, query_locs, pc_dims, geo_dists, pre_enc_inds, raw_max=False):
         B = context_locs.shape[0]
         self._join_side_stream()
         if context_locs.is_cuda and self.cfg.dec_dim == 64 and (not torch.is_grad_enabled()
                                                                  or os.environ.get("GF_FUSED_BWD", "1") != "0"):
             if B == 1 and pre_enc_inds.dtype == torch.int32:
-                g1, m1 = pointops.relpos_prepare(geo_dists[0].contiguous(), pre_enc_inds[0].contiguous())
+                g1, m1 = pointops.relpos_prepare(geo_dists[0].contiguous(), pre_enc_inds[0].contiguous(),
+                                                 raw_max=raw_max and not torch.is_grad_enabled())
                 geo, max_geo = g1.unsqueeze(0), m1.unsqueeze(0)
             elif B > 1 and pre_enc_inds.stride(0) == 0 and all(g is geo_dists[0] for g in geo_dists):
                 g1 = geo_dists[0][:, pre_enc_inds[0].long()]
@@ -795,8 +796,8 @@
             qpr = self._pointwise_chain("qproj", [self.query_projection], context_feats)
             if e2d is not None and qpr is not None:
                 ctx = pointops.pointwise_mlp(context_feats[0].contiguous(), e2d)
-                rel = LazyRelPos(lambda: self.relative_position_embedding(context_locs, query_locs, pc_dims, geo_dists,
-                                                                          pre_enc_inds))
+                rel = LazyRelPos(lambda **kw: self.relative_position_embedding(context_locs, query_locs, pc_dims,
+                                                                               geo_dists, pre_enc_inds, **kw))
                 hit = self._early().pop("qpos", None)
                 if hit is not None and hit[0].shape == query_locs.shape:
                     torch.cuda.current_stream().wait_event(hit[2])
@@ -866,9 +867,12 @@
         else:
             mx = torch.max(geo_dist, dim=1)[0]
             mx = torch.sqrt(torch.where(mx < 0, torch.max(mx), mx)).contiguous()
-        logits = pointops.mask_head_packed(mask_features.reshape(n_mask, self.output_dim).contiguous(),
-                                           coords_.contiguous(), geo_dist.contiguous(),
-                                           fps_sampling_coords.reshape(-1, 3).contiguous(), mx, params.contiguous())
+        feat = mask_features.reshape(n_mask, self.output_dim).contiguous()
+        hit = self.__dict__.get("_gf_mh_split", {}).pop(_stream_key(), None)
+        split_ws = hit[1] if hit is not None and hit[0] == (feat.data_ptr(), n_mask) else None
+        logits = pointops.mask_head_packed(feat, coords_.contiguous(), geo_dist.contiguous(),
+                                           fps_sampling_coords.reshape(-1, 3).contiguous(), mx, params.contiguous(),
+                                           split_ws=split_ws)
         return logits.reshape(1, num_insts, n_mask)
 
     def get_mask_prediction(self, geo_dists, param_kernels, mask_features, locs_float_, fps_sampling_locs,
@@ -1141,6 +1145,9 @@
             outputs["mask_predictions"] = None
             return outputs
 
+        caller_stream = torch.cuda.current_stream(locs_float_.device) if locs_float_.is_cuda else None
+        split_key = _stream_key() if locs_float_.is_cuda else None
+
         def sampling_independent(graphs_only=None):
             if graphs_only is True:
                 return knn_graphs(locs_float_, batch_offsets_, batch_size, neighbor=64, radius=0.05)
@@ -1151,6 +1158,15 @@
                 mf = self._mask_tower_rows(output_feats_)
                 if mf is None:
                     mf = self.mask_tower(output_feats_.unsqueeze(2).permute(2, 1, 0)).permute(2, 1, 0)
+            self.__dict__.get("_gf_mh_split", {}).pop(split_key, None)
+            if (mf.is_cuda and not training and not torch.is_grad_enabled() and batch_size == 1
+                    and self.output_dim == 16 and os.environ.get("GF_MASK_SPLIT_AHEAD", "1") != "0"):
+                feat = mf.reshape(mf.shape[0], self.output_dim)
+                if feat.is_contiguous():
+                    ws = pointops.mask_head_split(feat)
+                    if torch.cuda.current_stream(mf.device) != caller_stream:
+                        ws.record_stream(caller_stream)
+                    self.__dict__.setdefault("_gf_mh_split", {})[split_key] = ((feat.data_ptr(), feat.shape[0]), ws)
             sp = None
             if not training:
                 sp = F.softmax(semantic_scores_, dim=1)
@@ -1239,4 +1255,5 @@
                     knn_flags=[f for f in (knn_truncated(graphs),) if f is not None], segments=segments)
         if locs_float.is_cuda:
             self._early().clear()
+            self.__dict__.get("_gf_mh_split", {}).pop(_stream_key(), None)
         return outputs
diff --git a/geoformer_amd/model/layers.py b/geoformer_amd/model/layers.py
--- a/geoformer_amd/model/layers.py
+++ b/geoformer_amd/model/layers.py
@@ -388,9 +388,9 @@
     def __init__(self, fn):
         self.fn, self.value = fn, None
 
-    def get(self):
+    def get(self, **kw):
         if self.value is None:
-            self.value = self.fn()
+            self.value = self.fn(**kw)
         return self.value
 
 
@@ -502,7 +502,7 @@
             if p.dim() > 1:
                 nn.init.xavier_uniform_(p)
 
-    def _forward_fused(self, tgt, memory, query_pos, rp):
+    def _forward_fused(self, tgt, memory, query_pos, rp, state=None, qkv_alt=None, q1_out=None):
         from .. import pointops
 
         c = _decoder_fused_cache(self)
@@ -512,18 +512,28 @@
         ff = self.layers[0].linear1.out_features
         mem = memory.permute(1, 0, 2).reshape(1, B * nc, d)
         kk = torch.baddbmm(c["bs"], mem.expand(2 * L, B * nc, d), c["wt"])
-        state = pointops.decoder_token_state(nq, B, tgt.device)
+        if state is None:
+            state = pointops.decoder_token_state(nq, B, tgt.device)
         inter = torch.empty((L, nq, B, d), dtype=torch.float32, device=tgt.device)
-        q1 = torch.empty((B, nq, d), dtype=torch.float32, device=tgt.device)
+        q1 = torch.empty((B, nq, d), dtype=torch.float32, device=tgt.device) if q1_out is None else q1_out
         tgt_c, qp = tgt.contiguous(), query_pos.contiguous()
         pointops.decoder_token_stage(None, tgt_c, qp, nq, B, 4, ff, None, c["tables"][0][1], state, None, q1)
+        one_launch = pointops.decoder_fused_ok()
+        if one_launch and qkv_alt is None:
+            qkv_alt = pointops.decoder_fused_qkv(nq, B, tgt.device)
         if isinstance(rp, LazyRelPos):
-            rp = rp.get()
+            rp = rp.get(raw_max=True) if one_launch else rp.get()
         for l in range(L):
+            pre = c["tables"][l + 1][1] if l + 1 < L else None
+            K1, Kv = kk[2 * l].view(B, nc, d), kk[2 * l + 1].view(B, nc, d)
+            if one_launch:
+                pointops.decoder_layer_fused(rp.geo_ctx, rp.max_geo, rp.query_locs, rp.context_locs, rp.lo, rp.hi,
+                                             rp.gauss_B, q1, K1, Kv, c["packs"][l], 4, ff, qp,
+                                             c["tables"][l][1] if l > 0 else None, c["tables"][l][0], pre, state, qkv_alt,
+                                             l & 1, inter[l])
+                continue
             attn = pointops.decoder_cross_attn(rp.geo_ctx, rp.max_geo, rp.query_locs, rp.context_locs, rp.lo, rp.hi,
-                                               rp.gauss_B, q1, kk[2 * l].view(B, nc, d), kk[2 * l + 1].view(B, nc, d),
-                                               c["packs"][l], c["b2"][l])
-            pre = c["tables"][l + 1][1] if l + 1 < L else None
+                                               rp.gauss_B, q1, K1, Kv, c["packs"][l], c["b2"][l])
             pointops.decoder_token_stage(attn, None, qp, nq, B, 4, ff, c["tables"][l][0], pre, state, inter[l],
                                          q1 if pre is not None else None)
         return inter
diff --git a/geoformer_amd/pointops.py b/geoformer_amd/pointops.py
--- a/geoformer_amd/pointops.py
+++ b/geoformer_amd/pointops.py
@@ -397,6 +397,14 @@
     return scratch("mask_head_split", _lib.load().gf_mask_head_split_bytes(N) // 8 + 1, torch.int64, device)
 
 
+def mask_head_split(feat):
+    _f32c(feat, "feat")
+    N = feat.shape[0]
+    ws = torch.empty(_lib.load().gf_mask_head_split_bytes(N) // 8 + 1, dtype=torch.int64, device=feat.device)
+    check(_lib.load().gf_mask_head_split(ptr(feat), N, ptr(ws), stream_ptr()), "gf_mask_head_split")
+    return ws
+
+
 def mask_head(feat, coords, geo, qxyz, sqrt_max_geo, w1, b1, w2, b2, split=True):
     for t, name in ((feat, "feat"), (coords, "coords"), (qxyz, "qxyz"), (w1, "w1"), (b1, "b1"), (w2, "w2"), (b2, "b2")):
         _f32c(t, name)
@@ -409,11 +417,11 @@
     return out
 
 
-def mask_head_packed(feat, coords, geo, qxyz, sqrt_max_geo, params, split=True):
-    return mask_head_episodes(feat, coords, geo, qxyz, sqrt_max_geo, params.unsqueeze(0), split=split)[0]
-
-
-def mask_head_episodes(feat, coords, geo, qxyz, sqrt_max_geo, params, split=True):
+def mask_head_packed(feat, coords, geo, qxyz, sqrt_max_geo, params, split=True, split_ws=None):
+    return mask_head_episodes(feat, coords, geo, qxyz, sqrt_max_geo, params.unsqueeze(0), split=split, split_ws=split_ws)[0]
+
+
+def mask_head_episodes(feat, coords, geo, qxyz, sqrt_max_geo, params, split=True, split_ws=None):
     for t, name in ((feat, "feat"), (coords, "coords"), (qxyz, "qxyz"), (params, "params")):
         _f32c(t, name)
     N, C = feat.shape
@@ -423,10 +431,13 @@
     base = params.data_ptr()
     o_w2, o_b1, o_b2 = C * (C + 3), C * (C + 3) + C, C * (C + 3) + 2 * C
     out = torch.empty((E, nq, N), dtype=torch.float32, device=feat.device)
-    check(_lib.load().gf_mask_head_episodes(ptr(feat), ptr(coords), ptr(geo), ptr(qxyz), ptr(sqrt_max_geo), base,
-                                            base + 4 * o_b1, base + 4 * o_w2, base + 4 * o_b2, ld, N, nq, E, C,
-                                            ptr(_mask_head_split_ws(N, feat.device, split)), ptr(out), stream_ptr()),
-          "gf_mask_head_episodes")
+    ready = split_ws is not None
+    if ready and split_ws.numel() * 8 < _lib.load().gf_mask_head_split_bytes(N):
+        raise RuntimeError("mask_head_episodes: split_ws is smaller than gf_mask_head_split_bytes(N)")
+    check(_lib.load().gf_mask_head_episodes_cfg(ptr(feat), ptr(coords), ptr(geo), ptr(qxyz), ptr(sqrt_max_geo), base,
+                                                base + 4 * o_b1, base + 4 * o_w2, base + 4 * o_b2, ld, N, nq, E, C,
+                                                ptr(split_ws if ready else _mask_head_split_ws(N, feat.device, split)),
+                                                1 if ready else 0, ptr(out), stream_ptr()), "gf_mask_head_episodes")
     return out
 
 
@@ -721,6 +732,31 @@
           "gf_decoder_token_stage")
 
 
+def decoder_fused_qkv(nq, B, device):
+    return torch.empty(_lib.load().gf_decoder_layer_fused_qkv_bytes(nq, B) // 4, dtype=torch.float32, device=device)
+
+
+def decoder_fused_ok():
+    return bool(_lib.load().gf_decoder_layer_fused_ok(getattr(_launch_cfg, "cross_attn_waves", 16)))
+
+
+def decoder_layer_fused(geo_ctx, max_geo, qloc, cloc, lo, hi, gaussB, Q1, K1, Kv, wpack, nhead, ff, query_pos, pro, post,
+                        pre, state, qkv_alt, qkv_in, inter_out):
+    for t in (geo_ctx, max_geo, qloc, cloc, lo, hi, gaussB, Q1, K1, Kv, wpack, query_pos, state, qkv_alt, inter_out):
+        _f32c(t, "decoder_layer_fused argument")
+    B, nq, nc = geo_ctx.shape
+    if (Q1.shape != (B, nq, 64) or K1.shape != (B, nc, 64) or Kv.shape != (B, nc, 64) or max_geo.shape != (B, nq)
+            or query_pos.shape != (nq, B, 64) or inter_out.shape != (nq, B, 64)
+            or state.numel() * 4 < _lib.load().gf_decoder_token_state_bytes(nq, B)
+            or qkv_alt.numel() * 4 < _lib.load().gf_decoder_layer_fused_qkv_bytes(nq, B)):
+        raise RuntimeError("decoder_layer_fused: shapes do not match geo_ctx [B,nq,nc]")
+    check(_lib.load().gf_decoder_layer_fused(ptr(geo_ctx), ptr(max_geo), ptr(qloc), ptr(cloc), ptr(lo), ptr(hi),
+                                             ptr(gaussB), ptr(Q1), ptr(K1), ptr(Kv), ptr(wpack), B, nq, nc, 64, nhead, ff,
+                                             ptr(query_pos), pro, post, pre, ptr(state), ptr(qkv_alt), int(qkv_in),
+                                             ptr(inter_out),
+                                             stream_ptr()), "gf_decoder_layer_fused")
+
+
 def decoder_token_state(nq, B, device):
     return torch.empty(_lib.load().gf_decoder_token_state_bytes(nq, B) // 4, dtype=torch.float32, device=device)
 
@@ -779,14 +815,15 @@
     return out
 
 
-def relpos_prepare(geo, inds):
+def relpos_prepare(geo, inds, raw_max=False):
     _f32c(geo, "geo"); _i32c(inds, "inds")
     nq, n = geo.shape
     nc = inds.shape[0]
     geo_ctx = torch.empty((nq, nc), dtype=torch.float32, device=geo.device)
     max_geo = torch.empty(nq, dtype=torch.float32, device=geo.device)
-    check(_lib.load().gf_relpos_prepare(ptr(geo), ptr(inds), nq, n, nc, ptr(geo_ctx), ptr(max_geo), stream_ptr()),
-          "gf_relpos_prepare")
+    fn = _lib.load().gf_relpos_gather if raw_max else _lib.load().gf_relpos_prepare
+    check(fn(ptr(geo), ptr(inds), nq, n, nc, ptr(geo_ctx), ptr(max_geo), stream_ptr()),
+          "gf_relpos_gather" if raw_max else "gf_relpos_prepare")
     return geo_ctx, max_geo
 
 
diff --git a/include/geoformer_hip.h b/include/geoformer_hip.h
--- a/include/geoformer_hip.h
+++ b/include/geoformer_hip.h
@@ -248,6 +248,11 @@
 int gf_mask_head_episodes(const float* feat, const float* coords, const float* geo, const float* qxyz,
                           const float* sqrt_max_geo, const float* w1, const float* b1, const float* w2, const float* b2,
                           int ldp, int N, int nq, int E, int C, void* split_ws, float* out, void* stream);
+int gf_mask_head_split(const float* feat, int N, void* split_ws, void* stream);
+int gf_mask_head_episodes_cfg(const float* feat, const float* coords, const float* geo, const float* qxyz,
+                              const float* sqrt_max_geo, const float* w1, const float* b1, const float* w2,
+                              const float* b2, int ldp, int N, int nq, int E, int C, void* split_ws, int split_ready,
+                              float* out, void* stream);
 
 size_t gf_mask_head_bwd_scratch_floats(int N, int nq);
 int gf_mask_head_bwd(const float* feat, const float* coords, const float* geo, const float* qxyz,
@@ -321,6 +326,8 @@
 
 int gf_relpos_prepare(const float* geo, const int32_t* inds, int nq, int n, int nc, float* geo_ctx, float* max_geo,
                       void* stream);
+int gf_relpos_gather(const float* geo, const int32_t* inds, int nq, int n, int nc, float* geo_ctx, float* row_max,
+                     void* stream);
 
 int gf_proposal_select(const int32_t* final_, const int32_t* cls_pred, const float* scores, int nq, int32_t* sel,
                        long long* cls_out, float* scores_out, int32_t* d_count, void* stream);
@@ -422,6 +429,15 @@
                               const float* lo, const float* hi, const float* gaussB, const float* Q1, const float* K1,
                               const float* Kv, const float* Wpack, const float* b2, int B, int nq, int nc, int d,
                               float* out, float* stat_m, float* stat_l, int wg_waves, void* stream);
+
+size_t gf_decoder_layer_fused_qkv_bytes(int nq, int B);
+int gf_decoder_layer_fused(const float* geo_ctx, const float* max_geo, const float* qloc, const float* cloc,
+                           const float* lo, const float* hi, const float* gaussB, float* Q1, const float* K1,
+                           const float* Kv, const float* Wpack, int B, int nq, int nc, int d, int nhead, int ff,
+                           const float* query_pos, const float* const* pro_params, const float* const* post_params,
+                           const float* const* pre_params, void* state, void* qkv_alt, int qkv_in, float* inter_out,
+                           void* stream);
+int gf_decoder_layer_fused_ok(int wg_waves);
 
 size_t gf_decoder_cross_attn_bwd_scratch_floats(int B, int nq, int nc);
 int gf_decoder_cross_attn_bwd(const float* geo_ctx, const float* max_geo, const float* qloc, const float* cloc,
diff --git a/include/geoformer_hip_dev.h b/include/geoformer_hip_dev.h
--- a/include/geoformer_hip_dev.h
+++ b/include/geoformer_hip_dev.h
@@ -43,6 +43,8 @@
 
 int gf_dev_cross_attn_bf3(int on);
 
+int gf_dev_decoder_fused(int on);
+
 int gf_dev_bfs_qcap_max(int qcap);
 
 int gf_dev_panoptic_lds_bins(int bins);
```

After: 189.6. 15.8% lower.
